# qts8n/water-sandbox

Measured on AMD Instinct MI355X. Metric: simulation steps/sec @ N particles, higher is better.
Workload: dtype f32

## Files before the change

water-sandbox_amd/csrc/ws_api.cpp:

```cpp
#include <math.h>
#include <stdio.h>
#include <stdlib.h>
#include <string.h>

#include <algorithm>
#include <new>

#include "ws_internal.h"

namespace {

constexpr int kGridPad = 2;
constexpr uint64_t kMaxCells = 1ull << 29;

thread_local std::string g_create_error;

void slab_free(ws_handle *h);
void slab_drop_graphs(WsSlab *S);
ws_status slab_step(ws_handle *h);
ws_status slab_settle(ws_handle *h);
ws_status slab_read_by_id(ws_handle *h, int kind, void *out);
ws_status slab_gather_by_id(ws_handle *h, int kind);
ws_status slab_reset(ws_handle *h, const float *pos_xyz);
ws_status slab_write_particles(ws_handle *h, const ws_particle80 *in);
// ... 49 lines not shown
template <class T>
ws_status scratch_zeroed(ws_handle *h, WsScratch<T> &buf, size_t bytes, const char *what)
{
    const ws_status st = buf.grow(h, bytes, what);
    if (st) return st;
    HIP_TRY(h, hipMemsetAsync(buf.p, 0, bytes, h->stream));
    return WS_OK;
}

float powi_f32(float a, int b)
{
    float r = 1.0f;
    for (;;) {
        if (b & 1) r *= a;
        b /= 2;
        if (b == 0) break;
        a *= a;
    }
    return r;
}

float accept_threshold(float h)
{
    float t = h * h;
    while (sqrtf(t) > h) t = nextafterf(t, 0.0f);
    for (;;) {
        const float up = nextafterf(t, INFINITY);
        if (sqrtf(up) <= h)
            t = up;
        else
            break;
    }
    return t;
}

}

ws_status ws_alloc_failed(ws_handle *h, const char *what, hipError_t e)
{
    (void)hipGetLastError();
    return fail(h, e == hipErrorOutOfMemory ? WS_ERR_OUT_OF_MEMORY : WS_ERR_HIP, what, e);
}

namespace {

bool is_pow2(uint32_t n) { return n && !(n & (n - 1)); }

uint32_t ref_linear(int x, int y, int z)
{
    return (uint32_t)x * 15823u + (uint32_t)y * 9737333u + (uint32_t)z * 440817757u;
}

uint32_t ref_hash_delta(int x, int y, int z, uint32_t n) { return ref_linear(x, y, z) % n; }

ws_status validate_params(ws_handle *h, const ws_params *p)
{
    if (!p) return fail(h, WS_ERR_INVALID_ARG, "params is NULL");
    if (!(p->smoothing_radius > 0.0f) || !isfinite(p->smoothing_radius))
        return fail(h, WS_ERR_INVALID_ARG, "smoothing_radius must be finite and > 0");
    for (int c = 0; c < 3; c++) {
        if (!isfinite(p->ext_min[c]) || !isfinite(p->ext_max[c]) || p->ext_min[c] > p->ext_max[c])
            return fail(h, WS_ERR_INVALID_ARG, "container ext_min/ext_max must be finite with ext_min <= ext_max");
    }
    return WS_OK;
}

ws_status derive_dev(ws_handle *h, const ws_params &p, uint32_t n, WsDev *out)
{
    WsDev d{};
    d.dt = p.delta_time;
    d.damping = p.collision_damping;
    d.h = p.smoothing_radius;
    d.target_density = p.target_density;
    d.pressure_scalar = p.pressure_scalar;
    d.near_pressure_scalar = p.near_pressure_scalar;
    d.viscosity = p.viscosity_strength;
    ws_smoothing_kernel sk;
    ws_get_smoothing_kernel(&p, &sk);
    d.k_pow2 = sk.pow2;
    d.k_pow2_der = sk.pow2_der;
    d.k_pow3 = sk.pow3;
    d.k_pow3_der = sk.pow3_der;
    d.k_spikey = sk.spikey_pow3;
    for (int c = 0; c < 3; c++) {
        d.grav[c] = p.gravity[c];
        d.ext_min[c] = p.ext_min[c];
        d.ext_max[c] = p.ext_max[c];
    }
    d.d2_accept = accept_threshold(d.h);
    uint64_t cells = 1;
    for (int c = 0; c < 3; c++) {
        const double lo = floor((double)floorf(p.ext_min[c] / d.h)) - kGridPad;
        const double hi = floor((double)floorf(p.ext_max[c] / d.h)) + kGridPad;
        const double dim = hi - lo + 1.0;
        if (!(fabs(lo) < 8388608.0) || !(fabs(hi) < 8388608.0))
            return fail(h, WS_ERR_INVALID_ARG, "container / smoothing_radius out of range (more than 2^23 cells along an axis)");
        d.org[c] = (int32_t)lo;
        d.fdim[c] = d.dim[c] = (int32_t)dim;
        d.cm[c] = 1;
        cells *= (uint64_t)d.dim[c];
    }
    uint64_t budget = std::max<uint64_t>(16ull * n, 1ull << 24);
    if (const char *v = WS_DEV_ENV("WS_CELL_BUDGET")) budget = std::max<uint64_t>(strtoull(v, nullptr, 10), 64);
    budget = std::min<uint64_t>(budget, kMaxCells);
    for (int c = 2; c >= 0 && cells > budget; c--) {
        const uint64_t others = cells / (uint64_t)d.dim[c];
        uint64_t want = std::max<uint64_t>(budget / std::max<uint64_t>(others, 1), 1);
        uint64_t m = ((uint64_t)d.fdim[c] + want - 1) / want;
        const uint64_t m_max = c == 0 ? (uint64_t)d.fdim[c] : (uint64_t)d.fdim[c] / 3;
        m = std::min<uint64_t>(std::max<uint64_t>(m, 1), std::max<uint64_t>(m_max, 1));
        d.cm[c] = (int32_t)m;
        d.dim[c] = (int32_t)(((uint64_t)d.fdim[c] + m - 1) / m);
        cells = others * (uint64_t)d.dim[c];
    }
    d.coarse = (d.cm[0] != 1 || d.cm[1] != 1 || d.cm[2] != 1) ? 1u : 0u;
    if (cells > kMaxCells) return fail(h, WS_ERR_OUT_OF_MEMORY, "cell grid too large even with merged cells");
    d.ncells = (uint32_t)cells;
    d.guard = d.dim[1] * d.dim[2] + d.dim[2] + 1;
    d.n = n;
    d.base = 0;
    d.gdim_x = d.dim[0];
    d.xoff = 0;
    d.hash_n = n;
    h->sk = sk;
    *out = d;
    return WS_OK;
}

void free_grid(ws_handle *h)
{
    h->cells.release();
    h->starts.release();
    h->start = nullptr;
    h->grid_alloc_cells = 0;
}

ws_status alloc_grid(ws_handle *h)
{
    const WsDev &d = h->dev;
    if (h->steps > 0 && WS_DEV_ENV("WS_FAIL_REGRID")) return fail(h, WS_ERR_OUT_OF_MEMORY, "cell tables: allocation failure forced by WS_FAIL_REGRID");
    ws_status st = WS_OK;
    if (h->grid_alloc_cells < d.ncells) {
        free_grid(h);
        if ((st = h->cells.alloc(h, &h->count, (size_t)d.ncells * 4, "cell counts"))) return st;
        if ((st = h->cells.alloc(h, &h->cursor, (size_t)d.ncells * 4, "cell cursors"))) return st;
        h->grid_alloc_cells = d.ncells;
    }
    h->starts.release();
    h->start = nullptr;
    const size_t nstart = (size_t)d.ncells + 2 * (size_t)d.guard + 2;
    if ((st = h->starts.alloc(h, &h->start_alloc, (nstart + 4) * 4, "cell starts"))) return st;
    h->start = h->start_alloc + (4u - (uint32_t)d.guard % 4u) % 4u;
    if ((st = h->starts.alloc(h, &h->bsum, (size_t)wsk_scan_state_words(d.ncells) * 4, "cell scan state", true))) return st;
    HIP_TRY(h, hipMemsetAsync(h->start, 0, (size_t)d.guard * 4, h->stream));
    std::vector<uint32_t> tail((size_t)d.guard + 2, d.n);
    HIP_TRY(h, hipMemcpyAsync(h->start + d.guard + d.ncells, tail.data(), tail.size() * 4, hipMemcpyHostToDevice,
                              h->stream));
    HIP_TRY(h, hipStreamSynchronize(h->stream));
    HIP_TRY(h, hipMemsetAsync(h->count, 0, (size_t)d.ncells * 4, h->stream));
    return WS_OK;
}

ws_status upload_mult(ws_handle *h)
{
    uint8_t m[27];
    bool alias = false;
    const uint32_t n = h->dev.hash_n;
    for (int dx = -1; dx <= 1; dx++)
        for (int dy = -1; dy <= 1; dy++)
            for (int dz = -1; dz <= 1; dz++) {
                uint32_t cnt = 0;
                for (int ox = -1; ox <= 1; ox++)
                    for (int oy = -1; oy <= 1; oy++)
                        for (int oz = -1; oz <= 1; oz++) {
                            if (is_pow2(n)) {
                                if (ref_hash_delta(ox, oy, oz, n) == ref_hash_delta(dx, dy, dz, n)) cnt++;
                                continue;
                            }
                            if (ox == dx && oy == dy && oz == dz) {
                                cnt++;
                                continue;
                            }
                            const int64_t delta = (int64_t)ref_linear(ox, oy, oz) - (int64_t)ref_linear(dx, dy, dz);
                            for (int64_t k = -1; k <= 1; k++)
                                if ((delta + k * ((int64_t)1 << 32)) % (int64_t)n == 0) alias = true;
                        }
                if (cnt > 1) alias = true;
                m[(dx + 1) * 9 + (dy + 1) * 3 + (dz + 1)] = (uint8_t)(cnt ? cnt : 1);
            }
    h->alias = alias;
    if (!h->mult) {
        const ws_status st = h->fixed.alloc(h, &h->mult, 32, "stencil multiplicities");
        if (st) return st;
    }
    HIP_TRY(h, copy_now(h, h->mult, m, 27, hipMemcpyHostToDevice));
    return WS_OK;
}

void configure_kernels(ws_handle *h)
{
    if (const char *v = WS_DEV_ENV("WS_VARIANT")) h->variant = strcmp(v, "simple") == 0 ? WS_VARIANT_SIMPLE : WS_VARIANT_LISTED;
    h->ieee = (h->flags & WS_FLAG_IEEE_DIVISION) != 0;
}

ws_status ensure_stage(ws_handle *h, size_t bytes)
{
    const ws_status st = h->stage_mem.grow(h, bytes, "staging buffer");
    h->stage = h->stage_mem.p;
    return st;
}

#define WS_DEAD_CHECK(h)                                               \
    do {                                                               \
        if ((h)->dead) return fail((h), WS_ERR_HIP, (h)->err.c_str()); \
    } while (0)

#ifdef WS_WITH_REFCHECK
#include "ws_refcheck_host.inc"
#define WS_REF_DISPATCH(h, call)       \
    do {                               \
        if ((h)->refmode) return call; \
    } while (0)
#else
#define WS_REF_DISPATCH(h, call) ((void)0)
#endif

hipEvent_t get_event(ws_handle *h)
{
    if (!h->pool.empty()) {
        hipEvent_t e = h->pool.back();
        h->pool.pop_back();
        return e;
    }
    hipEvent_t e = nullptr;
    if (hipEventCreate(&e) != hipSuccess) return nullptr;
    return e;
}

struct Prof {
    ws_handle *h;
    bool on;
    WsEventPair p{};
    Prof(ws_handle *h_, uint32_t k) : h(h_), on((h_->flags & WS_FLAG_PROFILE) != 0 && ((h_->prof_mask >> k) & 1u))
    {
        if (!on) return;
        p.kernel = k;
        p.a = get_event(h);
        p.b = get_event(h);
        if (!p.a || !p.b || hipEventRecord(p.a, h->stream) != hipSuccess) {
            if (p.a) h->pool.push_back(p.a);
            if (p.b) h->pool.push_back(p.b);
            on = false;
        }
    }
    ~Prof()
    {
        if (!on) return;
        if (hipEventRecord(p.b, h->stream) == hipSuccess) {
            h->pending.push_back(p);
        } else {
            h->pool.push_back(p.a);
            h->pool.push_back(p.b);
        }
    }
};

struct ProfLaunch {
    ws_handle *h;
    bool on, taken = false;
    WsEventPair p{};
    ProfLaunch(ws_handle *h_, uint32_t k, bool counts = true)
        : h(h_), on((h_->flags & WS_FLAG_PROFILE) != 0 && ((h_->prof_mask >> k) & 1u))
    {
        if (!on) return;
        p.kernel = k;
        p.counts = counts;
        p.a = get_event(h);
        p.b = get_event(h);
        if (!p.a || !p.b) {
            if (p.a) h->pool.push_back(p.a);
            if (p.b) h->pool.push_back(p.b);
            on = false;
        }
    }
    const WsEventPair *events()
    {
        if (!on) return nullptr;
        taken = true;
        return &p;
    }
    ~ProfLaunch()
    {
        if (!on) return;
        if (taken) {
            h->pending.push_back(p);
        } else {
            h->pool.push_back(p.a);
            h->pool.push_back(p.b);
        }
    }
};

void drain_profile(ws_handle *h)
{
    for (auto &p : h->pending) {
        float ms = 0.f;
        if (hipEventElapsedTime(&ms, p.a, p.b) == hipSuccess) {
            h->prof_ms[p.kernel] += ms;
            h->prof_cnt[p.kernel] += p.counts ? 1 : 0;
        }
        h->pool.push_back(p.a);
        h->pool.push_back(p.b);
    }
    h->pending.clear();
}

void bound_pending(ws_handle *h)
{
    if (h->pending.size() < 4096) return;
    if (hipStreamSynchronize(h->stream) == hipSuccess) drain_profile(h);
}

#define WS_SCHED_MIN_PARTICLES (1u << 18)
#define WS_SCHED_END_PARTICLES (1u << 20)

void free_schedule(ws_handle *h)
{
    if (h->sched_stream) {
        hipStreamSynchronize(h->sched_stream);
        hipStreamDestroy(h->sched_stream);
    }
    if (h->ev_sched_in) hipEventDestroy(h->ev_sched_in);
    if (h->ev_sched_out) hipEventDestroy(h->ev_sched_out);
    h->sched.release();
    h->sched4[1].cost = nullptr;
    h->sched_stream = nullptr;
    h->ev_sched_in = h->ev_sched_out = nullptr;
    h->sched_on = false;
}

ws_status alloc_schedule(ws_handle *h)
{
    if (h->variant != WS_VARIANT_LISTED || h->slab) return WS_OK;
    uint32_t min_n = WS_SCHED_MIN_PARTICLES, max_n = WS_SCHED_END_PARTICLES - 1u;
    if (const char *v = WS_DEV_ENV("WS_TILE_SCHEDULE")) {
        min_n = 0;
        max_n = atoi(v) ? 0xFFFFFFFFu : 0u;
    }
    if (h->n > max_n || h->n < min_n) return WS_OK;
    if (const char *v = WS_DEV_ENV("WS_SCHED_CLASSES")) h->sched_classes = (uint32_t)atoi(v);
    if (const char *v = WS_DEV_ENV("WS_SCHED_GROUP")) h->sched_group = (uint32_t)atoi(v);
    h->sched_tiles4 = (h->n + wsk_density_tile() - 1u) / wsk_density_tile();
    h->sched_tiles5 = (h->n + wsk_force_tile(h->n) - 1u) / wsk_force_tile(h->n);
    const size_t t4 = (size_t)h->sched_tiles4 * 4, t5 = (size_t)h->sched_tiles5 * 4;
    WsGroup &G = h->sched;
    ws_status st = G.alloc(h, &h->sched4[0].cost, t4, "tile costs", true);
    h->sched4[1].cost = h->sched4[0].cost;
    for (int k = 0; k < 2 && !st; k++) {
        st = G.alloc(h, &h->sched4[k].split, 16 * 4, "tile schedule");
        if (!st) st = G.alloc(h, &h->sched4[k].perm, t4, "tile schedule");
        if (!st) st = G.alloc(h, &h->sched5[k].split, 16 * 4, "tile schedule");
        if (!st) st = G.alloc(h, &h->sched5[k].perm, t5, "tile schedule");
        if (!st) st = G.alloc(h, &h->sched5[k].cost, t5, "tile costs", true);
    }
    if (st) return st;
    HIP_TRY(h, hipStreamCreateWithFlags(&h->sched_stream, hipStreamNonBlocking));
    HIP_TRY(h, hipEventCreateWithFlags(&h->ev_sched_in, hipEventDisableTiming));
    HIP_TRY(h, hipEventCreateWithFlags(&h->ev_sched_out, hipEventDisableTiming));
    for (int k = 0; k < 2; k++)
        wsk_schedule(h->stream, h->sched4[k], h->sched_tiles4, h->sched5[k], h->sched5[k], h->sched_tiles5, h->sched_classes, h->sched_group,
                     wsk_force_tile(h->n));
    HIP_TRY(h, hipGetLastError());
    HIP_TRY(h, hipStreamSynchronize(h->stream));
    h->sched_parity = 0;
    h->sched_on = true;
    return WS_OK;
}

void enqueue_step(ws_handle *h)
{
    const WsDev &d = h->dev;
    hipStream_t s = h->stream;
    const bool sched = h->sched_on && !h->alias && h->variant == WS_VARIANT_LISTED && !(h->flags & WS_FLAG_GRAPH);
    const uint32_t par = h->sched_parity;
    {
        Prof p(h, WS_K_SCAN);
        wsk_scan(s, h->count, h->start + d.guard, nullptr, h->bsum, d.ncells, true, 0);
    }
    {
        Prof p(h, WS_K_SCATTER);
        wsk_place(s, d, h->cid_cur, h->cur.rank, h->start, h->slot_tmp);
    }
    {
        Prof p(h, WS_K_REORDER);
        wsk_reorder(s, d, h->slot_tmp, h->cid_cur, h->start, h->cur, h->srt, h->cid_srt, h->sxyz, h->pred_stale);
    }
    if (sched) hipStreamWaitEvent(s, h->ev_sched_out, 0);
    {
        ProfLaunch p(h, WS_K_DENSITY);
        wsk_density(s, d, h->start, h->cid_srt, h->srt, h->mult, h->alias, h->variant, h->ieee, h->stats, h->mask, h->sxyz,
                    p.events(), sched ? h->sched4[par] : WsSched{});
    }
    if (sched) {
        hipEventRecord(h->ev_sched_in, s);
        hipStreamWaitEvent(h->sched_stream, h->ev_sched_in, 0);
        wsk_schedule(h->sched_stream, h->sched4[par ^ 1u], h->sched_tiles4, h->sched5[par ^ 1u], h->sched5[par ^ 1u], h->sched_tiles5,
                     h->sched_classes, h->sched_group, wsk_force_tile(h->n));
        hipEventRecord(h->ev_sched_out, h->sched_stream);
        h->sched_parity = par ^ 1u;
    }
    {
        ProfLaunch p(h, WS_K_FORCE);
        wsk_force(s, d, h->start, h->cid_srt, h->srt, h->cur, h->accel, h->cid_cur, h->count, h->mult, h->alias,
                  h->variant, h->ieee, h->mask, false, p.events(), sched ? h->sched5[par] : WsSched{});
    }
    h->pred_stale = true;
    h->accel_stale = true;
}

void note_step_params(ws_handle *h)
{
    h->last_pressure = {h->dev.pressure_scalar, h->dev.target_density, h->dev.near_pressure_scalar};
}

void refresh_pred(ws_handle *h, const WsDev &d)
{
    if (!h->pred_stale) return;
    wsk_refresh_pred(h->stream, d, h->cur);
    h->pred_stale = false;
}

ws_status refresh_accel(ws_handle *h)
{
    if (!h->accel_stale) return WS_OK;
    WsDev d = h->dev;
    auto pass = [&](const WsDev &dd) {
        if (dd.n)
            wsk_force(h->stream, dd, h->start, h->cid_srt, h->srt, h->cur, h->accel, h->cid_cur, h->count, h->mult, h->alias,
                      h->variant, h->ieee, h->mask, true);
    };
    if (h->slab) {
        const WsSlab *S = h->slab;
        d.dyn = S->dyn;
        d.n = S->cap;
        if (S->last_split) {
            d.range_sel = WS_RANGE_EARLY;
            pass(d);
            d.range_sel = d.has_left && d.has_right ? WS_RANGE_LATE_BOTH : d.has_left ? WS_RANGE_LATE_LEFT : WS_RANGE_LATE_RIGHT;
            d.n = (uint32_t)std::min<uint64_t>(S->cap, 2ull * S->halo_cap);
            pass(d);
        } else {
            d.range_sel = WS_RANGE_ALL;
            pass(d);
        }
    } else {
        pass(d);
    }
    HIP_TRY(h, hipGetLastError());
    h->accel_stale = false;
    return WS_OK;
}

ws_status bin_current(ws_handle *h)
{
    refresh_pred(h, h->dev);
    HIP_TRY(h, hipMemsetAsync(h->count, 0, (size_t)h->dev.ncells * 4, h->stream));
    {
        Prof pr(h, WS_K_BIN);
        wsk_bin(h->stream, h->dev, h->cur, h->cid_cur, h->count);
    }
    HIP_TRY(h, hipGetLastError());
    return WS_OK;
}

ws_status upload_positions(ws_handle *h, const float *pos_xyz)
{
    const size_t bytes = (size_t)h->n * 12;
    ws_status st = ensure_stage(h, bytes);
    if (st) return st;
    HIP_TRY(h, hipMemcpyAsync(h->stage, pos_xyz, bytes, hipMemcpyHostToDevice, h->stream));
    wsk_upload_positions(h->stream, (const float *)h->stage, h->cur, h->n);
    HIP_TRY(h, hipGetLastError());
    h->pred_stale = false;
    h->accel_stale = false;
    st = bin_current(h);
    if (st) return st;
    HIP_TRY(h, hipStreamSynchronize(h->stream));
    h->steps = 0;
    h->last_pressure = {};
    return WS_OK;
}

void drop_graphs(ws_handle *h)
{
    if (h->graph_exec) hipGraphExecDestroy(h->graph_exec);
    h->graph_exec = nullptr;
    if (h->slab) slab_drop_graphs(h->slab);
}

ws_status alloc_particle_arrays(ws_handle *h, size_t slots, uint32_t mask_particles)
{
    const size_t n16 = (slots + 16) * 16, n4 = slots * 4;
    WsGroup &G = h->particles;
    ws_status st = G.alloc(h, &h->cur.pv, 2 * n16, "particle records");
    if (!st) st = G.alloc(h, &h->cur.pred, n16, "predicted positions");
    if (!st) st = G.alloc(h, &h->cur.rank, n4, "cell ranks");
    if (!st) st = G.alloc(h, &h->srt.pos, n16, "sorted positions");
    if (!st) st = G.alloc(h, &h->srt.pv, 2 * n16, "sorted records");
    for (float **plane : {&h->sxyz.x, &h->sxyz.y, &h->sxyz.z})
        if (!st) st = G.alloc(h, plane, n16 / 4, "sorted position planes", true);
    if (!st) st = G.alloc(h, &h->cid_cur, n4, "cell ids");
    if (!st) st = G.alloc(h, &h->cid_srt, n4, "sorted cell ids");
    if (!st) st = G.alloc(h, &h->accel, n16, "accelerations");
    if (!st) st = G.alloc(h, &h->slot_tmp, n4, "sort slots");
    if (!st && h->variant == WS_VARIANT_LISTED) {
        h->mask.stride = mask_particles;
        st = G.alloc(h, &h->mask.words, (size_t)wsk_mask_words() * mask_particles * 4, "accept masks");
    }
    return st;
}

void free_particle_arrays(ws_handle *h)
{
    drop_graphs(h);
    h->particles.release();
    h->mask.stride = 0;
}

void free_all(ws_handle *h)
{
    if (h->stream) hipStreamSynchronize(h->stream);
    if (h->copy_stream) {
        hipStreamSynchronize(h->copy_stream);
        hipStreamDestroy(h->copy_stream);
    }
    free_schedule(h);
    if (h->rb_gathered) hipEventDestroy(h->rb_gathered);
    if (h->rb_done) hipEventDestroy(h->rb_done);
    release_all(h->rb_stage, h->rb_host[0], h->rb_host[1]);
    drain_profile(h);
    for (auto e : h->pool) hipEventDestroy(e);
    free_grid(h);
    free_particle_arrays(h);
    release_all(h->fixed, h->stage_mem, h->force_cnt, h->solid_sums, h->v_keys, h->v_perm, h->v_tmp, h->v_count, h->v_cursor, h->v_start, h->v_bsum,
                h->v_off);
    for (auto &volume : h->volume) release_all(volume);
    release_all(h->attr);
    free_field(h);
#ifdef WS_WITH_REFCHECK
    ref_free(h);
#endif
    slab_free(h);
    if (h->done) hipEventDestroy(h->done);
    if (h->stream && h->own_stream) hipStreamDestroy(h->stream);
}

}

extern "C" {

uint32_t ws_abi_version(void) { return WS_ABI_VERSION; }

const char *ws_status_string(ws_status s)
{
    switch (s) {
        case WS_OK: return "ok";
        case WS_ERR_INVALID_ARG: return "invalid argument";
        case WS_ERR_NO_DEVICE: return "no usable gfx950 device";
        case WS_ERR_OUT_OF_MEMORY: return "out of device memory";
        case WS_ERR_HIP: return "HIP runtime error";
        case WS_ERR_COMM: return "RCCL communication error";
        case WS_ERR_UNSUPPORTED: return "unsupported";
        case WS_ERR_NOT_READY: return "not ready";
    }
    return "unknown status";
}

const char *ws_kernel_name(uint32_t k)
{
    static const char *names[WS_K_COUNT] = {"cell_scan", "cell_scatter", "reorder", "density", "force_integrate_bin",
                                            "bin"};
    return k < WS_K_COUNT ? names[k] : "?";
}

ws_status ws_default_params(ws_params *out)
{
    if (!out) return WS_ERR_INVALID_ARG;
    memset(out, 0, sizeof *out);
    out->delta_time = 1.0f / 60.0f;
    out->collision_damping = 0.95f;
    out->smoothing_radius = 0.25f;
    out->target_density = 10.0f;
    out->pressure_scalar = 22.0f;
    out->near_pressure_scalar = 2.0f;
    out->viscosity_strength = 0.1f;
    out->gravity[1] = -9.8f;
    const float position[3] = {0.f, 0.f, 0.f}, size[3] = {16.f, 9.f, 9.f};
    return ws_get_ext(position, size, 0.1f, out->ext_min, out->ext_max);
}

ws_status ws_get_smoothing_kernel(const ws_params *p, ws_smoothing_kernel *out)
{
    if (!p || !out) return WS_ERR_INVALID_ARG;
    const float PI = 3.14159265358979323846f;
    const float h = p->smoothing_radius;
    out->pow2 = 15.0f / (2.0f * PI * powi_f32(h, 5));
    out->pow2_der = 15.0f / (PI * powi_f32(h, 5));
    out->pow3 = 15.0f / (PI * powi_f32(h, 6));
    out->pow3_der = 45.0f / (PI * powi_f32(h, 6));
    out->spikey_pow3 = 315.0f / (64.0f * PI * powi_f32(h, 9));
    return WS_OK;
}

ws_status ws_cube_fluid(uint32_t ni, uint32_t nj, uint32_t nk, float r, float *out)
{
    if (!out) return WS_ERR_INVALID_ARG;
    const float ox = r - (float)ni * r, oy = r - (float)nj * r, oz = r - (float)nk * r;
    const float diam = r * 2.0f;
    size_t o = 0;
    for (uint32_t i = 0; i < ni; i++)
        for (uint32_t j = 0; j < nj; j++)
            for (uint32_t k = 0; k < nk; k++) {
                out[o++] = (float)i * diam + ox;
                out[o++] = (float)j * diam + oy;
                out[o++] = (float)k * diam + oz;
            }
    return WS_OK;
}

ws_status ws_get_ext(const float position[3], const float size[3], float padding, float ext_min[4], float ext_max[4])
{
    if (!position || !size || !ext_min || !ext_max) return WS_ERR_INVALID_ARG;
    for (int c = 0; c < 3; c++) {
        const float half = size[c] / 2.0f;
        ext_min[c] = (position[c] - half) + padding;
        ext_max[c] = (position[c] + half) - padding;
    }
    ext_min[3] = ext_max[3] = 0.0f;
    return WS_OK;
}

uint32_t ws_bit_sorter_stage_count(uint32_t data_length)
{
    uint32_t k = 0;
    uint64_t p = 1;
    while (p < data_length) {
        p <<= 1;
        k++;
    }
    return k * (k + 1) / 2;
}

ws_status ws_create(const ws_params *params, const float *pos_xyz, uint32_t n, const ws_device_cfg *cfg,
                    ws_handle **out)
{
    if (!out) return WS_ERR_INVALID_ARG;
    *out = nullptr;
    if (!pos_xyz || n == 0) return fail(nullptr, WS_ERR_INVALID_ARG, "pos_xyz is NULL or n == 0");
    if (n > WS_MAX_SLOTS - 16u) return fail(nullptr, WS_ERR_INVALID_ARG, "more than 2^27 particles on one device");
    ws_status st = validate_params(nullptr, params);
    if (st) return st;
    if (cfg && cfg->world_size > 1) return fail(nullptr, WS_ERR_UNSUPPORTED, "multi-GPU slabs are created with ws_slab_create");
#ifndef WS_WITH_REFCHECK
    if (cfg && (cfg->flags & WS_FLAG_REFERENCE_ORDER))
        return fail(nullptr, WS_ERR_UNSUPPORTED,
                    "WS_FLAG_REFERENCE_ORDER is a validation mode of the test-only build (tests/libwsfluid_refcheck.so)");
#endif

    int ndev = 0;
    if (hipGetDeviceCount(&ndev) != hipSuccess || ndev <= 0)
        return fail(nullptr, WS_ERR_NO_DEVICE, "no HIP device visible (this library has no CPU fallback)");
    const int device = cfg ? cfg->device : 0;
    if (device < 0 || device >= ndev) return fail(nullptr, WS_ERR_NO_DEVICE, "device index out of range");
    hipDeviceProp_t prop;
    if (hipGetDeviceProperties(&prop, device) != hipSuccess) return fail(nullptr, WS_ERR_NO_DEVICE, "hipGetDeviceProperties failed");
    if (strncmp(prop.gcnArchName, "gfx950", 6) != 0)
        return fail(nullptr, WS_ERR_NO_DEVICE, "device is not gfx950 (kernels are built for MI355X only)");

    ws_handle *h = new (std::nothrow) ws_handle();
    if (!h) return fail(nullptr, WS_ERR_OUT_OF_MEMORY, "host allocation failed");
    h->device = device;
    h->flags = cfg ? cfg->flags : 0;
    h->n = n;
    h->params = *params;
    configure_kernels(h);
    if (h->flags & WS_FLAG_GRAPH) h->flags &= ~(uint32_t)WS_FLAG_PROFILE;

    auto bail = [&](ws_status s) {
        g_create_error = h->err;
        free_all(h);
        delete h;
        return s;
    };

    CREATE_HIP(hipSetDevice(device));
    CREATE_HIP(hipStreamCreateWithFlags(&h->stream, hipStreamNonBlocking));
    CREATE_HIP(hipEventCreateWithFlags(&h->done, hipEventDisableTiming));
    CREATE_TRY(derive_dev(h, *params, n, &h->dev));
#ifdef WS_WITH_REFCHECK
    if (h->flags & WS_FLAG_REFERENCE_ORDER) {
        CREATE_TRY(ref_alloc(h));
        CREATE_TRY(ref_upload_positions(h, pos_xyz));
        *out = h;
        return WS_OK;
    }
#endif
    CREATE_TRY(alloc_particle_arrays(h, n, n));
    CREATE_TRY(h->fixed.alloc(h, &h->stats, 64, "device counters", true));
    CREATE_TRY(alloc_grid(h));
    CREATE_TRY(upload_mult(h));
    CREATE_TRY(upload_positions(h, pos_xyz));
    CREATE_TRY(alloc_schedule(h));
    *out = h;
    return WS_OK;
}

ws_status ws_destroy(ws_handle *h)
{
    if (!h) return WS_OK;
    hipSetDevice(h->device);
    free_all(h);
    delete h;
    return WS_OK;
}

const char *ws_last_error(ws_handle *h) { return h ? h->err.c_str() : g_create_error.c_str(); }
uint32_t ws_num_particles(ws_handle *h) { return h ? h->n : 0; }
uint64_t ws_steps_done(ws_handle *h) { return h ? h->steps : 0; }

ws_status ws_step(ws_handle *h)
{
    if (!h) return WS_ERR_INVALID_ARG;
    HIP_TRY(h, hipSetDevice(h->device));
    if (h->slab) return slab_step(h);
    WS_REF_DISPATCH(h, ref_step(h));
    if (h->dead) return fail(h, WS_ERR_HIP, h->err.c_str());
    hipStream_t s = h->stream;
    bound_pending(h);
    note_step_params(h);
    if ((h->flags & WS_FLAG_GRAPH) && !h->graph_failed && h->pred_stale) {
        if (!h->graph_exec) {
            hipGraph_t gr = nullptr;
            hipError_t e = hipStreamBeginCapture(s, hipStreamCaptureModeRelaxed);
            if (e == hipSuccess) {
                enqueue_step(h);
                e = hipStreamEndCapture(s, &gr);
                if (e == hipSuccess) e = hipGraphInstantiate(&h->graph_exec, gr, nullptr, nullptr, 0);
                if (gr) hipGraphDestroy(gr);
            }
            if (e != hipSuccess || !h->graph_exec) {
                (void)hipGetLastError();
                h->graph_failed = true;
                h->graph_exec = nullptr;
                h->err = std::string("WS_FLAG_GRAPH: capture failed (") + hipGetErrorName(e) + "), using direct launches";
            }
        }
        if (h->graph_exec) {
            HIP_TRY(h, hipGraphLaunch(h->graph_exec, s));
            h->pred_stale = true;
            h->accel_stale = true;
            h->graph_steps++;
            HIP_TRY(h, hipEventRecord(h->done, s));
            h->done_recorded = true;
            h->steps++;
            return WS_OK;
        }
    }
    enqueue_step(h);
    HIP_TRY(h, hipGetLastError());
    HIP_TRY(h, hipEventRecord(h->done, s));
    h->done_recorded = true;
    h->steps++;
    return WS_OK;
}

ws_status ws_ready(ws_handle *h, int *ready)
{
    if (!h || !ready) return WS_ERR_INVALID_ARG;
    if (!h->done_recorded) {
        *ready = 1;
        return WS_OK;
    }
    const hipError_t e = hipEventQuery(h->done);
    if (e == hipSuccess)
        *ready = 1;
    else if (e == hipErrorNotReady)
        *ready = 0;
    else
        return fail(h, WS_ERR_HIP, "hipEventQuery", e);
    return WS_OK;
}

ws_status ws_sync(ws_handle *h)
{
    if (!h) return WS_ERR_INVALID_ARG;
    WS_DEAD_CHECK(h);
    HIP_TRY(h, hipSetDevice(h->device));
    if (h->slab) {
        const ws_status st = slab_settle(h);
        drain_profile(h);
        return st;
    }
    HIP_TRY(h, hipStreamSynchronize(h->stream));
    drain_profile(h);
    return WS_OK;
}

ws_status ws_set_params(ws_handle *h, const ws_params *params)
{
    if (!h) return WS_ERR_INVALID_ARG;
    WS_DEAD_CHECK(h);
    ws_status st = validate_params(h, params);
    if (st) return st;
    HIP_TRY(h, hipSetDevice(h->device));
    WsDev nd;
    st = derive_dev(h, *params, h->slab ? h->slab->n_global : h->n, &nd);
    if (st) return st;
    const WsDev &od = h->dev;
    bool regrid = memcmp(nd.org, od.org, sizeof nd.org) || memcmp(nd.dim, od.dim, sizeof nd.dim) || nd.h != od.h;
    if (h->slab) {
        regrid = nd.h != od.h || nd.dim[1] != od.dim[1] || nd.dim[2] != od.dim[2] || nd.dim[0] != od.gdim_x ||
                 memcmp(nd.org, od.org, sizeof nd.org);
        nd.dim[0] = od.dim[0]; nd.gdim_x = od.gdim_x; nd.xoff = od.xoff; nd.ncells = od.ncells; nd.guard = od.guard;
        nd.base = od.base; nd.n = od.n; nd.hash_n = od.hash_n;
        nd.has_left = od.has_left; nd.has_right = od.has_right; nd.mig = od.mig;
        memcpy(nd.lidx, od.lidx, sizeof nd.lidx);
    }
    WS_REF_DISPATCH(h, ref_set_params(h, params, nd));
    if (h->slab && regrid) return slab_regrid(h, params, false);
    const bool accel_params_changed =
        nd.h != od.h || nd.target_density != od.target_density || nd.pressure_scalar != od.pressure_scalar ||
        nd.near_pressure_scalar != od.near_pressure_scalar || nd.viscosity != od.viscosity || nd.k_pow2_der != od.k_pow2_der ||
        nd.k_pow3_der != od.k_pow3_der || nd.k_spikey != od.k_spikey || nd.d2_accept != od.d2_accept;
    if (regrid || accel_params_changed) {
        st = refresh_accel(h);
        if (st) return st;
    }
    h->params = *params;
    if (!regrid) {
        if (memcmp(&h->dev, &nd, sizeof nd) != 0) {
            drop_graphs(h);
            if (h->slab) h->slab->limit_hold = 8;
        }
        h->dev = nd;
        return WS_OK;
    }
    drop_graphs(h);
    HIP_TRY(h, hipStreamSynchronize(h->stream));
    h->dev = nd;
    st = alloc_grid(h);
    if (!st) st = bin_current(h);
    if (st) {
        h->dead = true;
        h->err = "re-grid failed after the old cell tables were given up (" + h->err + "); the handle is unusable";
    }
    return st;
}

ws_status ws_read_positions(ws_handle *h, float *out_xyz)
{
    if (!h || (!out_xyz && !h->slab)) return WS_ERR_INVALID_ARG;
    WS_DEAD_CHECK(h);
    HIP_TRY(h, hipSetDevice(h->device));
    if (h->slab) return slab_read_by_id(h, WS_PACK_POS_H, out_xyz);
    WS_REF_DISPATCH(h, ref_read_positions(h, out_xyz));
    const size_t bytes = (size_t)h->n * 12;
    ws_status st = ensure_stage(h, bytes);
    if (st) return st;
    wsk_gather_positions(h->stream, h->cur, (float *)h->stage, h->n);
    HIP_TRY(h, hipGetLastError());
    HIP_TRY(h, hipMemcpyAsync(out_xyz, h->stage, bytes, hipMemcpyDeviceToHost, h->stream));
    HIP_TRY(h, hipStreamSynchronize(h->stream));
    drain_profile(h);
    return WS_OK;
}

ws_status ws_read_positions_begin(ws_handle *h, float *out_xyz)
{
    if (!h) return WS_ERR_INVALID_ARG;
    WS_DEAD_CHECK(h);
    WS_REF_DISPATCH(h, fail(h, WS_ERR_UNSUPPORTED, "no asynchronous readback in the reference-order validation mode"));
    if (h->rb_inflight) return fail(h, WS_ERR_INVALID_ARG, "a readback is already in flight (call ws_read_positions_end)");
    HIP_TRY(h, hipSetDevice(h->device));
    const size_t bytes = (size_t)(h->slab ? h->slab->n_global : h->n) * 12;
    if (!h->copy_stream) {
        int lo = 0, hi = 0;
        const char *pr = WS_DEV_ENV("WS_COPY_STREAM_PRIORITY");
        if (pr && strcmp(pr, "default") == 0) {
            HIP_TRY(h, hipStreamCreateWithFlags(&h->copy_stream, hipStreamNonBlocking));
        } else {
            HIP_TRY(h, hipDeviceGetStreamPriorityRange(&lo, &hi));
            HIP_TRY(h, hipStreamCreateWithPriority(&h->copy_stream, hipStreamNonBlocking, hi));
        }
        HIP_TRY(h, hipEventCreateWithFlags(&h->rb_gathered, hipEventDisableTiming));
        HIP_TRY(h, hipEventCreateWithFlags(&h->rb_done, hipEventDisableTiming));
    }
    const bool owned = out_xyz == nullptr;
    if (owned) {
        if (h->rb_host[1].bytes < bytes) {
            release_all(h->rb_host[0], h->rb_host[1]);
            h->rb_last = -1;
            for (auto &b : h->rb_host) {
                const ws_status st = b.alloc(h, bytes, "page-locked readback buffer");
                if (st) return st;
            }
        }
        h->rb_fill = h->rb_last == 0 ? 1 : 0;
        out_xyz = h->rb_host[h->rb_fill].p;
    }
    const float *src;
    if (h->slab) {
// ... 22 lines not shown
    if (!h->rb_inflight) return fail(h, WS_ERR_INVALID_ARG, "no readback in flight");
    HIP_TRY(h, hipSetDevice(h->device));
    HIP_TRY(h, hipEventSynchronize(h->rb_done));
    h->rb_inflight = false;
    if (h->rb_owned) h->rb_last = h->rb_fill;
    return WS_OK;
}

ws_status ws_read_positions_view(ws_handle *h, const float **out_xyz)
{
    if (!h || !out_xyz) return WS_ERR_INVALID_ARG;
    *out_xyz = nullptr;
    if (h->rb_last < 0) return fail(h, WS_ERR_INVALID_ARG, "no finished readback into the library's buffers (ws_read_positions_begin(h, NULL) / _end)");
    *out_xyz = h->rb_host[h->rb_last].p;
    return WS_OK;
}

ws_status ws_read_speeds(ws_handle *h, float *out_speed)
{
    if (!h || (!out_speed && !h->slab)) return WS_ERR_INVALID_ARG;
    WS_DEAD_CHECK(h);
    HIP_TRY(h, hipSetDevice(h->device));
    if (h->slab) return slab_read_by_id(h, WS_PACK_SPEED_H, out_speed);
    WS_REF_DISPATCH(h, ref_read_speeds(h, out_speed));
    const size_t bytes = (size_t)h->n * 4;
    ws_status st = ensure_stage(h, bytes);
    if (st) return st;
    wsk_gather_speeds(h->stream, h->cur, (float *)h->stage, h->n);
    HIP_TRY(h, hipGetLastError());
    HIP_TRY(h, hipMemcpyAsync(out_speed, h->stage, bytes, hipMemcpyDeviceToHost, h->stream));
    HIP_TRY(h, hipStreamSynchronize(h->stream));
    drain_profile(h);
    return WS_OK;
}

ws_status ws_read_velocities(ws_handle *h, float *out_xyz)
{
    if (!h || (!out_xyz && !h->slab)) return WS_ERR_INVALID_ARG;
    WS_DEAD_CHECK(h);
    if (h->flags & WS_FLAG_REFERENCE_ORDER) return fail(h, WS_ERR_UNSUPPORTED, "velocities: not in the reference-order validation mode");
    HIP_TRY(h, hipSetDevice(h->device));
    const uint32_t n = h->slab ? h->slab->n_global : h->n;
    const size_t bytes = (size_t)n * 12;
    if (h->slab) {
        ws_status st = slab_gather_by_id(h, WS_PACK_POSVEL_H);
        if (st) return st;
        if (out_xyz) {
            if ((st = ensure_stage(h, bytes))) return st;
            wsk_field_split(h->stream, reinterpret_cast<const float *>(h->slab->g_out.p), nullptr, (float *)h->stage, n);
            HIP_TRY(h, hipGetLastError());
            HIP_TRY(h, hipMemcpyAsync(out_xyz, h->stage, bytes, hipMemcpyDeviceToHost, h->stream));
        }
        HIP_TRY(h, hipStreamSynchronize(h->stream));
        return WS_OK;
    }
    ws_status st = ensure_stage(h, bytes);
    if (st) return st;
    wsk_gather_velocities(h->stream, h->cur, (float *)h->stage, n);
    HIP_TRY(h, hipGetLastError());
    HIP_TRY(h, hipMemcpyAsync(out_xyz, h->stage, bytes, hipMemcpyDeviceToHost, h->stream));
    HIP_TRY(h, hipStreamSynchronize(h->stream));
    drain_profile(h);
    return WS_OK;
}

ws_status ws_pin_host_buffer(ws_handle *h, void *ptr, uint64_t bytes)
{
    if (!h || !ptr || !bytes) return WS_ERR_INVALID_ARG;
    HIP_TRY(h, hipSetDevice(h->device));
    HIP_TRY(h, hipHostRegister(ptr, (size_t)bytes, hipHostRegisterDefault));
    return WS_OK;
}

ws_status ws_unpin_host_buffer(ws_handle *h, void *ptr)
{
    if (!h || !ptr) return WS_ERR_INVALID_ARG;
    HIP_TRY(h, hipSetDevice(h->device));
    HIP_TRY(h, hipHostUnregister(ptr));
    return WS_OK;
}

ws_status ws_read_particles(ws_handle *h, ws_particle80 *out)
{
    if (!h || (!out && !h->slab)) return WS_ERR_INVALID_ARG;
    WS_DEAD_CHECK(h);
    HIP_TRY(h, hipSetDevice(h->device));
    if (h->slab) return slab_read_by_id(h, WS_PACK_RECORD_H, out);
    WS_REF_DISPATCH(h, ref_read_particles(h, out));
    const size_t bytes = (size_t)h->n * sizeof(ws_particle80);
    ws_status st = ensure_stage(h, bytes);
    if (st) return st;
    refresh_pred(h, h->dev);
    st = refresh_accel(h);
    if (st) return st;
    wsk_gather_particles(h->stream, h->cur, h->srt, h->accel, h->steps > 0, h->last_pressure, (ws_particle80 *)h->stage, h->n);
    HIP_TRY(h, hipGetLastError());
    HIP_TRY(h, hipMemcpyAsync(out, h->stage, bytes, hipMemcpyDeviceToHost, h->stream));
    HIP_TRY(h, hipStreamSynchronize(h->stream));
    drain_profile(h);
    return WS_OK;
}

ws_status ws_reset(ws_handle *h, const float *pos_xyz)
{
    if (!h || !pos_xyz) return WS_ERR_INVALID_ARG;
    WS_DEAD_CHECK(h);
    HIP_TRY(h, hipSetDevice(h->device));
    if (h->attr.p) HIP_TRY(h, hipMemsetAsync(h->attr.p, 0, h->attr.bytes, h->stream));
    if (h->slab) return slab_reset(h, pos_xyz);
    WS_REF_DISPATCH(h, ref_upload_positions(h, pos_xyz));
    return upload_positions(h, pos_xyz);
}

ws_status ws_write_particles(ws_handle *h, const ws_particle80 *in)
{
    if (!h || !in) return WS_ERR_INVALID_ARG;
    WS_DEAD_CHECK(h);
    HIP_TRY(h, hipSetDevice(h->device));
    if (h->slab) return slab_write_particles(h, in);
    WS_REF_DISPATCH(h, ref_load(h, in, false));
    const size_t bytes = (size_t)h->n * sizeof(ws_particle80);
    ws_status st = ensure_stage(h, bytes);
    if (st) return st;
    HIP_TRY(h, hipMemcpyAsync(h->stage, in, bytes, hipMemcpyHostToDevice, h->stream));
    wsk_upload_particles(h->stream, (const ws_particle80 *)h->stage, h->cur, h->n);
    HIP_TRY(h, hipGetLastError());
    h->pred_stale = false;
    h->accel_stale = false;
    st = bin_current(h);
    if (st) return st;
    HIP_TRY(h, hipStreamSynchronize(h->stream));
    h->steps = 0;
    h->last_pressure = {};
    return WS_OK;
}

}

namespace {

template <class Call>
ws_status edit_fluid(ws_handle *h, Call &call)
{
    if (!h) return WS_ERR_INVALID_ARG;
    WS_DEAD_CHECK(h);
    if (h->flags & WS_FLAG_REFERENCE_ORDER)
        return fail(h, WS_ERR_UNSUPPORTED, (std::string(call.tag) + ": not in the reference-order validation mode").c_str());
    HIP_TRY(h, hipSetDevice(h->device));
    if (h->slab) return slab_edit_gathered(h, call);
    if (const char *why = call.refuse()) return fail(h, WS_ERR_INVALID_ARG, why);
    const ws_status st = call.prepare(h, nullptr);
    if (st) return st;
    HIP_TRY(h, hipMemsetAsync(h->count, 0, (size_t)h->dev.ncells * 4, h->stream));
    wsk_edit_current(h->stream, h->dev, h->cur, h->cid_cur, h->count, call.args);
    HIP_TRY(h, hipGetLastError());
    h->pred_stale = true;
    HIP_TRY(h, call.fetch(h));
    return WS_OK;
}

const char *forces_refusal(const ws_force *f, uint32_t k, float dt)
{
    if (!f) return "forces: f is NULL";
    if (k < 1u || k > WS_MAX_FORCES) return "forces: k outside 1 .. WS_MAX_FORCES";
    if (ws_bad_float(dt) || !(dt > 0.f)) return "forces: dt must be finite, > 0 and at most 1e15";
    for (uint32_t e = 0; e < k; e++) {
        if (f[e].kind > WS_FORCE_VORTEX) return "forces: unknown kind";
        if (f[e].reserved[0] || f[e].reserved[1]) return "forces: reserved words must be 0";
        for (int c = 0; c < 3; c++)
            if (ws_bad_float(f[e].centre[c]) || ws_bad_float(f[e].axis[c])) return "forces: centre and axis must be finite and at most 1e15 in magnitude";
        if (ws_bad_float(f[e].strength) || ws_bad_float(f[e].damping)) return "forces: strength and damping must be finite and at most 1e15 in magnitude";
        if (f[e].damping < 0.f) return "forces: damping must be >= 0";
        if (ws_bad_float(f[e].radius) || !(f[e].radius > 0.f)) return "forces: radius must be finite, > 0 and at most 1e15";
    }
    return nullptr;
}

struct ForcesCall {
    const ws_force *f;
    uint32_t k;
    float dt;
    uint32_t *out_affected;
    const char *tag = "forces", *things = "emitters";
    WsForceArgs args{};
    const char *refuse() const { return forces_refusal(f, k, dt); }
    ws_status prepare(ws_handle *h, const WsGathered *)
    {
        memcpy(args.fs.e, f, (size_t)k * sizeof(ws_force));
        args.k = k;
        args.dt = dt;
        if (!out_affected) return WS_OK;
        const ws_status st = scratch_zeroed(h, h->force_cnt, WS_MAX_FORCES * 4, "force counters");
        args.affected = h->force_cnt.p;
        return st;
    }
    template <class M>
    void mix(M m, bool valid) const
    {
        m(&k, 4);
        m(&dt, 4);
        if (valid) m(f, (size_t)k * sizeof(ws_force));
    }
    hipError_t fetch(ws_handle *h) const
    {
        return out_affected ? copy_now(h, out_affected, h->force_cnt.p, (size_t)k * 4, hipMemcpyDeviceToHost) : hipSuccess;
    }
};

}

extern "C" {

ws_status ws_apply_forces(ws_handle *h, const ws_force *f, uint32_t k, float dt, uint32_t *out_affected)
{
    ForcesCall call{f, k, dt, out_affected};
    return edit_fluid(h, call);
}

}

namespace {

struct CohesionCall {
    const ws_cohesion_params *p;
    float dt;
    uint32_t *out_affected;
    const char *tag = "cohesion", *things = "parameters";
    WsCohesionArgs args{};
    const char *refuse() const { return cohesion_refusal(p, dt); }
    uint32_t partial[WS_COHESION_SLOTS * WS_COHESION_SLOT_WORDS];
    ws_status prepare(ws_handle *h, const WsGathered *g)
    {
        ws_status st = cohesion_prepare(h, g, p, dt, &args);
        if (st || !out_affected) return st;
        st = scratch_zeroed(h, h->force_cnt, sizeof partial, "cohesion counters");
        args.affected = h->force_cnt.p;
        return st;
    }
    template <class M>
    void mix(M m, bool valid) const
    {
        m(&dt, 4);
        if (valid) m(p, sizeof *p);
    }
    hipError_t fetch(ws_handle *h)
    {
        if (!out_affected) return hipSuccess;
        const hipError_t e = copy_now(h, partial, h->force_cnt.p, sizeof partial, hipMemcpyDeviceToHost);
        if (e != hipSuccess) return e;
        uint32_t total = 0;
        for (uint32_t s = 0; s < WS_COHESION_SLOTS; s++) total += partial[s * WS_COHESION_SLOT_WORDS];
        *out_affected = total;
        return hipSuccess;
    }
};

}

extern "C" {

ws_status ws_apply_cohesion(ws_handle *h, const ws_cohesion_params *p, float dt, uint32_t *out_affected)
{
    CohesionCall call{p, dt, out_affected};
    return edit_fluid(h, call);
}

}

namespace {

const char *solids_refusal(const ws_solid *s, uint32_t k)
{
    if (!s) return "solids: s is NULL";
    if (k < 1u || k > WS_MAX_SOLIDS) return "solids: k outside 1 .. WS_MAX_SOLIDS";
    for (uint32_t e = 0; e < k; e++) {
        const ws_solid &o = s[e];
        if (o.kind > WS_SOLID_CAPSULE) return "solids: unknown kind";
        if (o.flags & ~WS_SOLID_HOLLOW) return "solids: unknown flag bits";
        if (o.reserved[0] || o.reserved[1]) return "solids: reserved words must be 0";
        for (int c = 0; c < 9; c++)
            if (ws_bad_float(o.rot[c])) return "solids: rot must be finite and at most 1e15 in magnitude";
        for (int c = 0; c < 3; c++)
            if (ws_bad_float(o.centre[c]) || ws_bad_float(o.size[c]) || ws_bad_float(o.velocity[c]) || ws_bad_float(o.angular_velocity[c]))
                return "solids: centre, size, velocity and angular_velocity must be finite and at most 1e15 in magnitude";
        if (ws_bad_float(o.restitution) || ws_bad_float(o.friction) || ws_bad_float(o.margin)) return "solids: restitution, friction and margin must be finite";
        const int used = o.kind == WS_SOLID_BOX ? 3 : 1;
        for (int c = 0; c < used; c++)
            if (!(o.size[c] > 0.f)) return "solids: a radius or half extent must be > 0";
        if (o.kind == WS_SOLID_CAPSULE && o.size[1] < 0.f) return "solids: a capsule's half length must be >= 0";
        if (o.restitution < 0.f || o.restitution > 1.f || o.friction < 0.f || o.friction > 1.f) return "solids: restitution and friction must lie in [0, 1]";
        if (o.margin < 0.f) return "solids: margin must be >= 0";
    }
    return nullptr;
}

double rot_sigma_min2(const float *rot)
{
    double G[3][3];
    for (int i = 0; i < 3; i++)
        for (int j = 0; j < 3; j++)
            G[i][j] = (double)rot[3 * i] * rot[3 * j] + (double)rot[3 * i + 1] * rot[3 * j + 1] + (double)rot[3 * i + 2] * rot[3 * j + 2];
    const double tr = G[0][0] + G[1][1] + G[2][2], mean = tr / 3.0;
    const double off = G[0][1] * G[0][1] + G[0][2] * G[0][2] + G[1][2] * G[1][2];
    double dev = 2.0 * off;
    for (int i = 0; i < 3; i++) dev += (G[i][i] - mean) * (G[i][i] - mean);
    const double pp = sqrt(dev / 6.0);
// ... 335 lines not shown
ws_status ws_read_stats(ws_handle *h, uint32_t out[16])
{
    if (!h || !out) return WS_ERR_INVALID_ARG;
    ws_status st = ws_sync(h);
    if (st) return st;
    HIP_TRY(h, copy_now(h, out, h->stats, 64, hipMemcpyDeviceToHost));
    for (int c = 0; c < 3; c++) out[1 + c] = (uint32_t)h->dev.cm[c];
    out[4] = (uint32_t)(h->slab ? h->slab->graph_steps : h->graph_steps);
    out[15] = (h->sched_on && !h->alias && !(h->flags & WS_FLAG_GRAPH)) ? 1u : 0u;
    if (h->slab) {
        uint32_t dyn[WS_DYN_WORDS];
        HIP_TRY(h, copy_now(h, dyn, h->slab->dyn, sizeof dyn, hipMemcpyDeviceToHost));
        out[5] = dyn[DY_PEAK_HALO];
        out[6] = h->slab->halo_cap;
        out[7] = dyn[DY_PEAK_MIG];
        out[8] = h->slab->mig_cap;
        out[9] = dyn[DY_PEAK_FAR];
        out[10] = h->slab->far_cap;
        out[11] = h->slab->mig_limit_next;
        out[12] = h->slab->halo_limit_next;
        out[13] = h->slab->far_limit_next;
        out[14] = h->slab->size_waits;
        if (h->slab->world == 1) {
            out[11] = out[12] = out[13] = 0;
        } else if (h->slab->exact_messages) {
            out[11] = h->slab->exact_now[0];
            out[12] = h->slab->exact_now[1];
            out[13] = h->slab->exact_now[2];
        }
    }
    return WS_OK;
}

ws_status ws_grid_dims(ws_handle *h, uint32_t dims[3])
{
    if (!h || !dims) return WS_ERR_INVALID_ARG;
    for (int c = 0; c < 3; c++) dims[c] = (uint32_t)h->dev.dim[c];
    return WS_OK;
}

}

#ifdef WS_DEV_HOOKS
namespace {

struct DevSchedArrays {
    WsScratch<uint32_t> cost4, cost5, split4, split5, perm4, perm5;
    void release() { release_all(cost4, cost5, split4, split5, perm4, perm5); }
};

ws_status dev_upload_costs(ws_handle *h, WsScratch<uint32_t> &buf, const uint32_t *cost, uint32_t nt)
{
    const ws_status st = buf.alloc(h, (size_t)nt * 4, "planted tile costs");
    if (st) return st;
    if (nt) HIP_TRY(h, hipMemcpyAsync(buf.p, cost, (size_t)nt * 4, hipMemcpyHostToDevice, h->stream));
    return WS_OK;
}

ws_status dev_schedule_outputs(ws_handle *h, WsScratch<uint32_t> &split, WsScratch<uint32_t> &perm, uint32_t nt)
{
    ws_status st = split.alloc(h, 16 * 4, "tile schedule");
    if (!st) st = perm.alloc(h, (size_t)nt * 4, "tile schedule");
    if (st) return st;
    HIP_TRY(h, hipMemsetAsync(split.p, 0xFF, 16 * 4, h->stream));
    if (nt) HIP_TRY(h, hipMemsetAsync(perm.p, 0xFF, (size_t)nt * 4, h->stream));
    return WS_OK;
}

ws_status dev_drain(ws_handle *h)
{
    HIP_TRY(h, hipStreamSynchronize(h->stream));
    if (h->sched_stream) HIP_TRY(h, hipStreamSynchronize(h->sched_stream));
    return WS_OK;
}

}

extern "C" {

ws_status ws_dev_schedule(ws_handle *h, const uint32_t *cost4, uint32_t nt4, const uint32_t *cost5, uint32_t nt5, uint32_t nclasses,
                          uint32_t group_particles, uint32_t tile5, uint32_t *split4, uint32_t *perm4, uint32_t *split5, uint32_t *perm5)
{
    if (!h || !split4 || !split5 || (nt4 && (!cost4 || !perm4)) || (nt5 && (!cost5 || !perm5)) || !tile5) return WS_ERR_INVALID_ARG;
    WS_DEAD_CHECK(h);
    HIP_TRY(h, hipSetDevice(h->device));
    DevSchedArrays a;
    const ws_status st = [&]() -> ws_status {
        ws_status s = dev_upload_costs(h, a.cost4, cost4, nt4);
        if (!s) s = dev_upload_costs(h, a.cost5, cost5, nt5);
        if (!s) s = dev_schedule_outputs(h, a.split4, a.perm4, nt4);
        if (!s) s = dev_schedule_outputs(h, a.split5, a.perm5, nt5);
        if (s) return s;
        WsSched s4, s5;
        s4.split = a.split4.p, s4.perm = a.perm4.p, s4.cost = a.cost4.p;
        s5.split = a.split5.p, s5.perm = a.perm5.p, s5.cost = a.cost5.p;
        wsk_schedule(h->stream, s4, nt4, s5, s5, nt5, nclasses, group_particles, tile5);
        HIP_TRY(h, hipGetLastError());
        HIP_TRY(h, hipMemcpyAsync(split4, a.split4.p, 9 * 4, hipMemcpyDeviceToHost, h->stream));
        HIP_TRY(h, hipMemcpyAsync(split5, a.split5.p, 9 * 4, hipMemcpyDeviceToHost, h->stream));
        if (nt4) HIP_TRY(h, hipMemcpyAsync(perm4, a.perm4.p, (size_t)nt4 * 4, hipMemcpyDeviceToHost, h->stream));
        if (nt5) HIP_TRY(h, hipMemcpyAsync(perm5, a.perm5.p, (size_t)nt5 * 4, hipMemcpyDeviceToHost, h->stream));
        HIP_TRY(h, hipStreamSynchronize(h->stream));
        return WS_OK;
    }();
    (void)hipStreamSynchronize(h->stream);
    a.release();
    return st;
}

ws_status ws_dev_plant_schedule(ws_handle *h, const uint32_t *cost4, const uint32_t *cost5)
{
    if (!h || !cost4 || !cost5) return WS_ERR_INVALID_ARG;
    WS_DEAD_CHECK(h);
    HIP_TRY(h, hipSetDevice(h->device));
    if (!h->sched_on) return fail(h, WS_ERR_INVALID_ARG, "ws_dev_plant_schedule: the handle has no tile schedule");
    DevSchedArrays a;
    const ws_status st = [&]() -> ws_status {
        ws_status s = dev_drain(h);
        if (!s) s = dev_upload_costs(h, a.cost4, cost4, h->sched_tiles4);
        if (!s) s = dev_upload_costs(h, a.cost5, cost5, h->sched_tiles5);
        if (s) return s;
        const uint32_t par = h->sched_parity;
        WsSched s4 = h->sched4[par], from5;
        s4.cost = a.cost4.p;
        from5.cost = a.cost5.p;
        wsk_schedule(h->stream, s4, h->sched_tiles4, h->sched5[par], from5, h->sched_tiles5, h->sched_classes, h->sched_group,
                     wsk_force_tile(h->n));
        HIP_TRY(h, hipGetLastError());
        HIP_TRY(h, hipMemsetAsync(h->sched4[par].cost, 0, (size_t)h->sched_tiles4 * 4, h->stream));
        HIP_TRY(h, hipMemsetAsync(h->sched5[par].cost, 0, (size_t)h->sched_tiles5 * 4, h->stream));
        HIP_TRY(h, hipStreamSynchronize(h->stream));
        return WS_OK;
    }();
    (void)hipStreamSynchronize(h->stream);
    a.release();
    return st;
}

ws_status ws_dev_read_tile_costs(ws_handle *h, uint32_t *cost4, uint32_t *cost5, uint32_t *ntiles)
{
    if (!h) return WS_ERR_INVALID_ARG;
    WS_DEAD_CHECK(h);
    HIP_TRY(h, hipSetDevice(h->device));
    if (!h->sched_on) return fail(h, WS_ERR_INVALID_ARG, "ws_dev_read_tile_costs: the handle has no tile schedule");
    const ws_status st = dev_drain(h);
    if (st) return st;
    if (ntiles) ntiles[0] = h->sched_tiles4, ntiles[1] = h->sched_tiles5;
    const uint32_t ran = h->sched_parity ^ 1u;
    if (cost4) HIP_TRY(h, copy_now(h, cost4, h->sched4[ran].cost, (size_t)h->sched_tiles4 * 4, hipMemcpyDeviceToHost));
    if (cost5) HIP_TRY(h, copy_now(h, cost5, h->sched5[ran].cost, (size_t)h->sched_tiles5 * 4, hipMemcpyDeviceToHost));
    return WS_OK;
}

}
#endif

#include "ws_field.inc"
#include "ws_slab.inc"
```

water-sandbox_amd/csrc/ws_internal.h:

```cpp
#pragma once

#include <hip/hip_runtime.h>
#include <math.h>
#include <stdint.h>

#include <string>
#include <vector>

#include "wsfluid.h"

#include "ws_devhooks.h"

struct WsMig {
    const uint32_t *cuts;
    uint32_t world, me;
    uint32_t *dyn;
    uint32_t *hole;
    uint32_t hole_cap;
    uint32_t *sendL, *sendR;
    uint32_t mig_cap;
    uint32_t *far;
    uint32_t far_cap;
};

// ... 95 lines not shown

struct WsSched {
    uint32_t *split = nullptr;
    uint32_t *perm = nullptr;
    uint32_t *cost = nullptr;
};

struct WsEventPair {
    uint32_t kernel;
    hipEvent_t a, b;
    bool counts = true;
};

inline bool ws_bad_float(float x) { return !isfinite(x) || fabsf(x) > 1e15f; }

ws_status ws_alloc_failed(ws_handle *h, const char *what, hipError_t e);

struct WsParked {
    std::vector<void *> list;
    void release()
    {
        for (void *q : list) (void)hipFree(q);
        list.clear();
    }
};

template <class... Owner>
void release_all(Owner &...o)
{
    (o.release(), ...);
}

template <class T, bool PINNED = false>
struct WsScratch {
    T *p = nullptr;
    size_t bytes = 0;
    ws_status alloc(ws_handle *h, size_t need, const char *what)
    {
        release();
        return fresh(h, need, what);
    }
    ws_status grow(ws_handle *h, size_t need, const char *what) { return bytes >= need ? WS_OK : alloc(h, need, what); }
    ws_status grow_parked(ws_handle *h, size_t need, size_t slack_div, WsParked *parked, const char *what)
    {
        if (bytes >= need) return WS_OK;
        T *const old = p;
        const size_t geometric = bytes + bytes / slack_div;
        const ws_status st = fresh(h, need > geometric ? need : geometric, what);
        if (!st && old) parked->list.push_back(old);
        return st;
    }
    void release()
    {
        if (p) (void)(PINNED ? hipHostFree(p) : hipFree(p));
        p = nullptr;
        bytes = 0;
    }

private:
    ws_status fresh(ws_handle *h, size_t want, const char *what)
    {
        void *q = nullptr;
        const size_t real = want > 4 ? want : 4;
        const hipError_t e = PINNED ? hipHostMalloc(&q, real, hipHostMallocDefault) : hipMalloc(&q, real);
        if (e != hipSuccess) return ws_alloc_failed(h, what, e);
        p = static_cast<T *>(q);
        bytes = want;
        return WS_OK;
    }
};

struct WsGroup {
    std::vector<void **> fields;
    template <class T>
    ws_status alloc(ws_handle *h, T **field, size_t bytes, const char *what, bool zero = false);
    void release()
    {
        for (void **f : fields) {
            (void)hipFree(*f);
            *f = nullptr;
        }
        fields.clear();
    }
};

struct WsField {
    uint32_t n = 0;
    WsScratch<float> xyz;
    WsScratch<uint32_t> keys, tmp, perm;
    WsScratch<float4> spos;
    uint32_t cells = 0;
    WsScratch<uint32_t> count, cursor, start, bsum;
    WsScratch<float> q, rho;
    WsScratch<float> grad;
    WsScratch<uint8_t> code;
    WsScratch<uint32_t> vbase, bcnt, bstart, bstate, tri;
    WsScratch<float> mxyz, mnrm;
    WsScratch<float> vxyz, vpos;
    WsScratch<float4> svel;
    WsScratch<float4> wnrm;
    WsScratch<float> wst, wout, wpt;
    WsScratch<uint32_t> wnb, wcnt, woff, wstate;
    WsScratch<float4> cnd, crec;
    WsScratch<float> cst;
    WsScratch<uint32_t> cnb;
    WsScratch<float4> sattr[2];
    WsScratch<float> srho;
    WsScratch<float4> aval;
    WsScratch<float> body;
    WsScratch<float> cxyz;
    WsScratch<float4> amf, smf;
    WsScratch<uint32_t> anb;
    WsScratch<float> rays, ray_t, ray_n;
};

struct WsVolumeDesc {
    const float *sdf;
    uint32_t dims[3];
    float origin[3];
    float spacing[3];
};

struct WsPressureParams {
    float pressure_scalar, target_density, near_pressure_scalar;
};

struct ws_handle {
    int device = 0;
    uint32_t flags = 0;
    uint32_t prof_mask = 0xFFFFFFFFu;
    uint32_t n = 0;
    uint64_t steps = 0;
    ws_params params{};
    ws_smoothing_kernel sk{};
    WsDev dev{};
    WsPressureParams last_pressure{};
    hipStream_t stream = nullptr;
    hipEvent_t done = nullptr;
    bool done_recorded = false;

    WsSoA cur{};
    WsSorted srt{};
    WsXYZ sxyz;
    uint32_t *cid_cur = nullptr;
    uint32_t *cid_srt = nullptr;
    int variant = WS_VARIANT_LISTED;
    float4 *accel = nullptr;
    uint32_t *slot_tmp = nullptr;
    uint32_t *count = nullptr;
    uint32_t *cursor = nullptr;
    uint32_t *start = nullptr;
    uint32_t *start_alloc = nullptr;
    uint32_t *bsum = nullptr;
    WsMask mask = {nullptr, 0};
    bool ieee = false;
    uint32_t *stats = nullptr;
    uint8_t *mult = nullptr;
    WsScratch<uint32_t> force_cnt;
    WsScratch<unsigned long long> solid_sums;
    WsScratch<float> volume[WS_MAX_VOLUMES];
    WsVolumeDesc volume_desc[WS_MAX_VOLUMES] = {};
    uint64_t volume_hash[WS_MAX_VOLUMES] = {};
    WsScratch<float4> attr;
    bool alias = false;
    size_t grid_alloc_cells = 0;
    WsGroup particles;
    WsGroup cells;
    WsGroup starts;
    WsGroup sched;
    WsGroup fixed;

    WsScratch<char> stage_mem;
    void *stage = nullptr;
    hipStream_t copy_stream = nullptr;
    hipEvent_t rb_gathered = nullptr, rb_done = nullptr;
    WsScratch<float> rb_stage;
    bool rb_inflight = false;
    WsScratch<float, true> rb_host[2];
    int rb_fill = 0, rb_last = -1;
    bool rb_owned = false;

    WsScratch<uint32_t> v_keys, v_perm, v_tmp, v_count, v_cursor, v_start, v_bsum, v_off;

    WsField field;

    std::vector<WsEventPair> pending;
    std::vector<hipEvent_t> pool;
    double prof_ms[WS_K_COUNT] = {0};
    uint64_t prof_cnt[WS_K_COUNT] = {0};

#ifdef WS_WITH_REFCHECK
    bool refmode = false;
    WsRef ref;
#endif

    WsSched sched4[2], sched5[2];
    uint32_t sched_tiles4 = 0, sched_tiles5 = 0;
    bool sched_on = false;
    uint32_t sched_classes = 8, sched_group = 64;
    uint32_t sched_parity = 0;
    hipStream_t sched_stream = nullptr;
    hipEvent_t ev_sched_in = nullptr, ev_sched_out = nullptr;

    hipGraphExec_t graph_exec = nullptr;
    bool graph_failed = false;
    uint64_t graph_steps = 0;

    bool accel_stale = false;
    bool pred_stale = false;
    struct WsSlab *slab = nullptr;
    bool own_stream = true;
    bool dead = false;

    std::string err;
};

template <class T>
ws_status WsGroup::alloc(ws_handle *h, T **field, size_t bytes, const char *what, bool zero)
{
    void *q = nullptr;
    hipError_t e = hipMalloc(&q, bytes);
    if (e != hipSuccess) return ws_alloc_failed(h, what, e);
    *field = static_cast<T *>(q);
    fields.push_back(reinterpret_cast<void **>(field));
    if (zero && (e = hipMemsetAsync(q, 0, bytes, h->stream)) != hipSuccess) return ws_alloc_failed(h, what, e);
    return WS_OK;
}

struct WsGraphEntry {
    uint32_t n_bound = 0, mig_cur = 0, mig_next = 0, halo = 0, far_cur = 0, far_next = 0;
    hipGraphExec_t exec = nullptr;
};
struct WsSlab {
    ws_transport tr{};
    uint32_t rank = 0, world = 1;
    uint32_t n_global = 0;
    uint32_t cap = 0;
    uint32_t halo_cap = 0;
    uint32_t mig_cap = 0;
    uint32_t far_cap = 0;
    uint32_t hole_cap = 0;
    uint32_t max_arrivals = 0;
    uint32_t mig_limit_cur = 0;
    uint32_t mig_limit_next = 0;
    uint32_t far_limit_cur = 0, far_limit_next = 0, want_far = 0;
    uint32_t halo_limit = 0, halo_limit_next = 0;
    uint32_t want_mig = 0, want_halo = 0;
    uint32_t want_ring[3][8] = {};
    uint64_t arrivals_hist[4] = {0, 0, 0, 0};
    uint32_t floor_mig = 4096, floor_far = 256, floor_halo = 8192;
    bool exact_messages = false;
    uint32_t *xs_send[2] = {nullptr, nullptr}, *xs_all[2] = {nullptr, nullptr};
    WsScratch<uint32_t, true> xs_host[2];
    hipEvent_t ev_sizes[2] = {nullptr, nullptr};
    uint32_t *far_pack = nullptr;
    uint32_t exact_now[3] = {0, 0, 0};
    uint32_t size_waits = 0;
    uint32_t limit_hold = 0;
    bool fixed_messages = false;
    uint32_t mode_word = 0;
    std::vector<uint32_t> cuts;
    uint32_t *cuts_dev = nullptr;
    uint32_t *dyn = nullptr;
    WsMig *mig_dev = nullptr;
    uint32_t *hole = nullptr, *tgt = nullptr, *src = nullptr;
    uint32_t *mig_sendL = nullptr, *mig_sendR = nullptr, *mig_recvL = nullptr, *mig_recvR = nullptr;
    uint32_t *far_send = nullptr, *far_all = nullptr;
    uint32_t *halo_sendL = nullptr, *halo_sendR = nullptr, *halo_recvL = nullptr, *halo_recvR = nullptr;
    bool binned = false;
    uint32_t *status_dev = nullptr;
    WsScratch<uint32_t, true> status_host;
    hipEvent_t ev_status[4] = {nullptr, nullptr, nullptr, nullptr};
    uint32_t n_known = 0;
    uint64_t n_known_step = 0;
    uint64_t t0 = 0;
    uint32_t cfg_ghost_capacity = 0;
    WsScratch<uint32_t> cnt_send, cnt_all;
    WsScratch<uint32_t> g_send, g_all, g_out;
    WsScratch<uint32_t> hist;
    WsScratch<uint32_t> agree_send, agree_all;
    WsParked retired;
    WsGroup fixed;
    WsGroup geometry;
    std::vector<uint32_t> counts;
    std::vector<uint32_t> caps;
    uint64_t left_base = 0, arrived_base = 0, far_base = 0;
    bool balanced = false;
    uint32_t failed = 0;
    bool comm_failed = false;
    hipStream_t comm = nullptr, copy = nullptr;
    hipEvent_t ev_sorted = nullptr, ev_halo_a = nullptr, ev_k4_late = nullptr, ev_halo_b = nullptr, ev_filled = nullptr;
    bool overlap = true;
    bool last_split = false;
    std::vector<struct WsGraphEntry> graphs;
    bool graph_failed = false;
    bool capturing = false;
    uint64_t graph_steps = 0;
    hipEvent_t ev_copied = nullptr;
    uint64_t migrated_out = 0;
};

extern "C" void ws_rccl_transport_bind_stream(const ws_transport *t, void *stream);

void wsk_upload_positions(hipStream_t s, const float *xyz_dev, WsSoA cur, uint32_t n);
void wsk_upload_particles(hipStream_t s, const ws_particle80 *in_dev, WsSoA cur, uint32_t n);
void wsk_bin(hipStream_t s, const WsDev &d, WsSoA cur, uint32_t *cid, uint32_t *count);
void wsk_place(hipStream_t s, const WsDev &d, const uint32_t *cid, const uint32_t *rank, const uint32_t *start, uint32_t *slot_tmp);
void wsk_scan(hipStream_t s, uint32_t *count, uint32_t *start_body, uint32_t *cursor, uint32_t *state, uint32_t nitems,
              bool zero_count, uint32_t base);
uint32_t wsk_scan_state_words(uint32_t nitems);
void wsk_scatter(hipStream_t s, const uint32_t *keys, uint32_t *cursor, uint32_t *slot_tmp, uint32_t n, const uint32_t *n_dev);
void wsk_reorder(hipStream_t s, const WsDev &d, const uint32_t *slot_tmp, const uint32_t *cid_cur, const uint32_t *start, WsSoA cur,
                 WsSorted srt, uint32_t *cid_srt, WsXYZ sxyz, bool recompute_pred);
void wsk_refresh_pred(hipStream_t s, const WsDev &d, WsSoA cur);
struct WsForceSet {
    ws_force e[WS_MAX_FORCES];
};
struct WsForceArgs {
    WsForceSet fs;
    uint32_t k;
    float dt;
    uint32_t *affected;
    bool outputs() const { return affected != nullptr; }
};
#define WS_SOLID_WORDS 7u
struct WsSolidSet {
    ws_solid e[WS_MAX_SOLIDS];
    float reach2[WS_MAX_SOLIDS];
};
struct WsSolidArgs {
    WsSolidSet ss;
    uint32_t k;
    unsigned long long *sums;
    bool outputs() const { return sums != nullptr; }
};
struct WsVolumeSet {
    WsVolumeDesc vol[WS_MAX_VOLUMES];
    ws_volume_pose e[WS_MAX_VOLUME_POSES];
    float reach2[WS_MAX_VOLUME_POSES];
};
struct WsVolumeArgs {
    WsVolumeSet vs;
    uint32_t k;
    unsigned long long *sums;
    bool outputs() const { return sums != nullptr; }
};
static_assert(WS_MAX_VOLUME_POSES == WS_MAX_SOLIDS, "the poses' sums are the solids' accumulator rows");
#define WS_COHESION_SLOTS 64u
#define WS_COHESION_SLOT_WORDS 16u
struct WsCohesionArgs {
    const float4 *dvc;
    uint32_t *affected;
    uint32_t n;
    bool outputs() const { return affected != nullptr; }
};
struct WsGathered {
    const uint32_t *recs, *cnt;
    uint32_t world, max_n;
    size_t stride_words;
};
template <class Args>
void wsk_edit_current(hipStream_t s, const WsDev &d, WsSoA cur, uint32_t *cid, uint32_t *count, const Args &a);
template <class Args>
void wsk_edit_records(hipStream_t s, const WsDev &d, uint32_t *all, const uint32_t *cnt, uint32_t world, uint32_t max_n,
                      size_t stride_words, const Args &a);
void wsk_density(hipStream_t s, const WsDev &d, const uint32_t *start, const uint32_t *cid_srt, WsSorted srt,
                 const uint8_t *mult, bool alias, int variant, bool ieee, uint32_t *stats, WsMask mask, WsXYZ sxyz,
                 const WsEventPair *ev = nullptr, WsSched sched = WsSched{});
uint32_t wsk_density_tile(void);
uint32_t wsk_force_tile(uint32_t n);
uint32_t wsk_sched_grid(uint32_t ntiles);
void wsk_schedule(hipStream_t s, WsSched s4, uint32_t ntiles4, WsSched s5, WsSched s5_costs, uint32_t ntiles5, uint32_t nclasses,
                  uint32_t group_particles, uint32_t tile5);
uint32_t wsk_mask_words(void);
void wsk_force(hipStream_t s, const WsDev &d, const uint32_t *start, const uint32_t *cid_srt, WsSorted srt, WsSoA out,
               float4 *accel, uint32_t *cid_out, uint32_t *count, const uint8_t *mult, bool alias, int variant, bool ieee,
               WsMask mask, bool accel_only, const WsEventPair *ev = nullptr, WsSched sched = WsSched{});
void wsk_gather_positions(hipStream_t s, WsSoA cur, float *out_xyz, uint32_t n);
void wsk_gather_speeds(hipStream_t s, WsSoA cur, float *out, uint32_t n);
void wsk_gather_velocities(hipStream_t s, WsSoA cur, float *out_xyz, uint32_t n);
void wsk_gather_particles(hipStream_t s, WsSoA cur, WsSorted srt, const float4 *accel, bool have_step,
                          const WsPressureParams &pp, ws_particle80 *out, uint32_t n);
void wsk_view_keys(hipStream_t s, const WsDev &d, WsSorted srt, uint32_t *keys_by_id, uint32_t *count);
void wsk_view_count(hipStream_t s, const uint32_t *keys, uint32_t *count, uint32_t n);
void wsk_view_fix(hipStream_t s, const uint32_t *tmp, const uint32_t *keys, const uint32_t *start,
                  uint32_t *perm, uint32_t n);
void wsk_view_offsets(hipStream_t s, const uint32_t *start, uint32_t *off, uint32_t n);
void wsk_iota(hipStream_t s, uint32_t *p, uint32_t n);
void wsk_set_words4(hipStream_t s, uint32_t *p, uint32_t a, uint32_t b, uint32_t c, uint32_t d);
void wsk_field_keys(hipStream_t s, const WsDev &d, const float *xyz, uint32_t *keys, uint32_t n);
void wsk_field_gather(hipStream_t s, const uint32_t *perm, const float *xyz, float4 *spos, uint32_t n);
void wsk_field_sample(hipStream_t s, const WsDev &d, const uint32_t *start, const float4 *spos, const float4 *smf, bool ieee,
                      bool grad_on, const float *xyz, uint32_t m, const float *grid6, const uint32_t *dims, bool bricks,
                      float *rho, float *grad);
void wsk_field_split(hipStream_t s, const float *pv, float *pos, float *vel, uint32_t n);
void wsk_field_gather_vel(hipStream_t s, const uint32_t *perm, const float *vxyz, float4 *svel, uint32_t n);
void wsk_velocity_sample(hipStream_t s, const WsDev &d, const uint32_t *start, const float4 *spos, const float4 *svel, bool ieee,
                         const float *xyz, uint32_t m, const float *grid6, const uint32_t *dims, bool bricks, float *vel,
                         float *rho);
void wsk_advect(hipStream_t s, const WsDev &d, const uint32_t *start, const float4 *spos, const float4 *svel, bool ieee,
                float *pts, uint32_t m, float dt, uint32_t substeps, float *vel, float *rho);
struct WsWhiteEmit {
    float tt0, tt1, tc0, tc1, te0, te1, kt, kc, align, dt, radius, l0, l1;
    uint32_t maxpp, seed;
};
struct WsWhiteStep {
    float dt;
    uint32_t spray_max, bubble_min;
    float buoyancy, drag;
};
void wsk_whitewater_stage(hipStream_t s, const WsDev &d, const uint32_t *start, const float4 *spos, const float4 *svel,
                          float4 *snrm, float *trapped, float *crest, float *align, float *energy, float *normal, uint32_t *nb,
                          uint32_t n);
void wsk_whitewater_count(hipStream_t s, const WsWhiteEmit &e, const float *vxyz, const float *trapped, const float *crest,
                          const float *align, const float *energy, uint32_t *cnt, uint32_t n);
void wsk_whitewater_spawn(hipStream_t s, const WsWhiteEmit &e, const float *pxyz, const float *vxyz, const uint32_t *cnt,
                          const uint32_t *off, float *out_xyz, float *out_vel, float *out_life, uint32_t *out_src, uint32_t n);
void wsk_whitewater_step(hipStream_t s, const WsDev &d, const uint32_t *start, const float4 *spos, const float4 *svel, bool ieee,
                         const WsWhiteStep &sp, float *pts, float *vel, float *life, uint8_t *cls, uint32_t m);
struct WsCohesion {
    float cohesion, curvature, xsph, rho0, dt, kc, h664;
};
void wsk_cohesion_stage(hipStream_t s, const WsDev &d, const uint32_t *start, const float4 *spos, const float4 *svel,
                        float4 *snd, const WsCohesion &k, float4 *dvc, float4 *nrho, uint32_t n);
void wsk_cohesion_unpack(hipStream_t s, const float4 *dvc, const float4 *nrho, float *normal, float *rho, float *dv, uint32_t *nb,
                         uint32_t n);
void wsk_state_split(hipStream_t s, const uint32_t *all, const uint32_t *cnt, uint32_t world, uint32_t max_n, size_t stride_words,
                     uint32_t n_global, float *pos, float *vel);
struct WsBrushSet {
    ws_brush e[WS_MAX_BRUSHES];
};
struct WsBrushArgs {
    WsBrushSet bs;
    uint32_t k;
    uint32_t *painted;
};
void wsk_attr_paint(hipStream_t s, const WsBrushArgs &a, const float *xyz, float4 *attr, uint32_t n);
void wsk_attr_gather(hipStream_t s, const float4 *spos, const float4 *attr, float4 *sa, uint32_t n);
void wsk_attr_scatter(hipStream_t s, const float4 *spos, const float4 *sa, float4 *attr, uint32_t n);
void wsk_attr_density(hipStream_t s, const WsDev &d, const uint32_t *start, const float4 *spos, float *srho, uint32_t n);
void wsk_attr_diffuse(hipStream_t s, const WsDev &d, const uint32_t *start, const float4 *spos, const float *srho, const float4 *sa,
                      const float *r4, float4 *out, uint32_t *affected, uint32_t n);
void wsk_attr_sample(hipStream_t s, const WsDev &d, const uint32_t *start, const float4 *spos, const float4 *sa, bool ieee,
                     const float *xyz, uint32_t m, const float *grid6, const uint32_t *dims, bool bricks, float4 *value, float *rho);
struct WsBodyParams {
    float fluid_density, drag, rho0;
};
uint32_t wsk_body_chunk(void);
void wsk_body_forces(hipStream_t s, const WsDev &d, const uint32_t *start, const float4 *spos, const float4 *svel, bool ieee,
                     const WsBodyParams &bp, const uint32_t *chunks, uint32_t nchunks, const uint32_t *cstart, uint32_t nb,
                     const float *xyz, const float *vel, const float *vol, const float *centre, float *part, float *sforce,
                     float *sfrac, float *force, float *torque, float *volume, uint32_t *wet);
struct WsAnisoParams {
    float lambda, kr, kn;
    uint32_t neps;
};
void wsk_aniso(hipStream_t s, const WsDev &d, const uint32_t *start, const float4 *spos, WsAnisoParams ap, float *cxyz,
               float4 *mf, uint32_t *nb, uint32_t n);
void wsk_aniso_gather(hipStream_t s, const uint32_t *perm, const float *cxyz, const float4 *mf, float4 *srec, float4 *smf,
                      uint32_t n);
void wsk_ray_cast(hipStream_t s, const WsDev &d, const uint32_t *start, const float4 *spos, const float4 *smf,
                  bool ieee, const ws_ray_params &r, const float *origin, const float *dir, uint32_t m,
                  const ws_camera *cam, const uint32_t *size, float *out_t, float *out_n);
uint32_t wsk_iso_blocks(const uint32_t *dims);
void wsk_iso_totals(hipStream_t s, const uint32_t *v_total, const uint32_t *t_total, uint32_t *out);
void wsk_iso_count(hipStream_t s, const float *rho, const float *grid6, const uint32_t *dims, float iso, uint8_t *code,
                   uint32_t *vcnt, uint32_t *tcnt);
void wsk_iso_mesh(hipStream_t s, const float *rho, const float *grad, const float *grid6, const uint32_t *dims, float iso,
                  const uint8_t *code, const uint32_t *vstart, const uint32_t *tstart, uint32_t *vbase, float *xyz,
                  float *nrm, uint32_t *tri);
void wsk_migrate_mark(hipStream_t s, const WsDev &d, WsSoA cur, uint32_t *cid_cur, uint32_t *count);
void wsk_migrate_fill(hipStream_t s, const WsDev &d, uint32_t world, uint32_t me, uint32_t cap, uint32_t *dyn,
                      const uint32_t *hole, const uint32_t *recvL, const uint32_t *recvR, uint32_t mig_cap,
                      const uint32_t *far_all, uint32_t far_cap, uint32_t *tgt, uint32_t *src, WsSoA cur, uint32_t *cid_cur,
                      uint32_t *count, uint32_t *status_ring, uint32_t status_slots, uint32_t hole_cap, uint32_t *sendL,
                      uint32_t *sendR, uint32_t *far_send, uint32_t far_next, uint64_t leave_bound);
void wsk_far_seal(hipStream_t s, uint32_t world, uint32_t far_cur, uint32_t *far_send, uint32_t *dyn);
void wsk_sizes(hipStream_t s, const uint32_t *a, const uint32_t *b, const uint32_t *c, const uint32_t *dyn, uint32_t *out);
void wsk_far_pack(hipStream_t s, uint32_t world, uint32_t far_cap, uint32_t far_n, const uint32_t *src, uint32_t *dst);
void wsk_halo_pack(hipStream_t s, const WsDev &d, const uint32_t *start, WsSorted srt, uint32_t *dyn, uint32_t rowy,
                   uint32_t halo_cap, uint32_t *sendL, uint32_t *sendR, bool densities);
void wsk_halo_unpack(hipStream_t s, const WsDev &d, uint32_t *start, WsSorted srt, WsXYZ sxyz, uint32_t *dyn, uint32_t rowy,
                     uint32_t nxl, uint32_t ghost_cap, const uint32_t *recvL, const uint32_t *recvR, bool densities);
void wsk_gather_slab(hipStream_t s, const WsDev &d, WsSoA cur, WsSorted srt, const float4 *accel, bool have_step,
                     const WsPressureParams &pp, ws_particle80 *out, uint32_t *ids);
void wsk_upload_positions_ids(hipStream_t s, const float *xyz_dev, const uint32_t *ids_dev, WsSoA cur, uint32_t n);
enum { WS_PACK_POS_H = 0, WS_PACK_SPEED_H = 1, WS_PACK_RECORD_H = 2, WS_PACK_STATE_H = 3, WS_PACK_KEY_H = 4, WS_PACK_POSVEL_H = 5 };
uint32_t wsk_pack_words(int kind);
void wsk_slab_pack(hipStream_t s, const WsDev &d, int kind, WsSoA cur, WsSorted srt, const float4 *accel, bool have_step,
                   const WsPressureParams &pp, uint32_t *out);
void wsk_slab_unpack_by_id(hipStream_t s, const uint32_t *all, const uint32_t *cnt, uint32_t world, uint32_t max_n,
                           size_t stride_words, uint32_t pw, uint32_t n_global, uint32_t *out);
void wsk_slab_layer_hist(hipStream_t s, const WsDev &d, const uint32_t *all, const uint32_t *cnt, uint32_t world, uint32_t max_n,
                         size_t stride_words, uint32_t *hist);
void wsk_slab_select(hipStream_t s, const WsDev &d, int src, const uint32_t *cuts, uint32_t world, uint32_t me,
                     const void *chunk, uint32_t id0, uint32_t m, const uint32_t *cnt, size_t stride_words, WsSoA cur,
                     uint32_t cap, uint32_t *dyn);
```

water-sandbox_amd/csrc/ws_kernels.hip:

```cpp
#include <stdlib.h>

#include <algorithm>
#include <type_traits>

#include "ws_internal.h"

#include <hip/hip_ext.h>


#pragma clang fp contract(off)

#define WS_BLOCK 256
#define WS_SCAN_ITEMS_SMALL 32
#define WS_SCAN_ITEMS_LARGE 64
#define WS_SCAN_LARGE_FROM (1u << 21)
#define WS_SCAN_TILE_MIN (WS_BLOCK * WS_SCAN_ITEMS_SMALL)

static inline uint32_t cdiv(uint32_t a, uint32_t b) { return (a + b - 1) / b; }

__device__ __forceinline__ uint32_t xcd_tile(uint32_t b, uint32_t nt, bool reverse = false)
{
    const uint32_t xcd = b & 7u, q = nt >> 3, r = nt & 7u;
    const uint32_t first = xcd < r ? xcd * (q + 1u) : r * (q + 1u) + (xcd - r) * q, mine = q + (xcd < r ? 1u : 0u);
    const uint32_t j = b >> 3;
    return first + (reverse ? mine - 1u - j : j);
}


__device__ __forceinline__ int grid_layer_x(const WsDev &d, float x)
{
    const float fx = floorf(x / d.h) - (float)d.org[0];
    int gxg = (int)fminf(fmaxf(fx, 0.0f), (float)(d.fdim[0] - 1));
    if (d.coarse) gxg /= d.cm[0];
    return gxg;
}

__device__ __forceinline__ uint32_t grid_cell(const WsDev &d, float x, float y, float z)
{
    const float fy = floorf(y / d.h) - (float)d.org[1];
    const float fz = floorf(z / d.h) - (float)d.org[2];
    const int gxg = grid_layer_x(d, x);
    int gy = (int)fminf(fmaxf(fy, 0.0f), (float)(d.fdim[1] - 1));
    int gz = (int)fminf(fmaxf(fz, 0.0f), (float)(d.fdim[2] - 1));
    if (d.coarse) {
        gy /= d.cm[1];
        gz /= d.cm[2];
    }
    const int gx = min(max(gxg - d.xoff, 0), d.dim[0] - 1);
    return (uint32_t)((gx * d.dim[1] + gy) * d.dim[2] + gz);
}

__device__ __forceinline__ uint32_t ref_hash_key(const WsDev &d, float x, float y, float z)
{
    const uint32_t cx = (uint32_t)(int32_t)floorf(x / d.h);
    const uint32_t cy = (uint32_t)(int32_t)floorf(y / d.h);
    const uint32_t cz = (uint32_t)(int32_t)floorf(z / d.h);
    return (cx * 15823u + cy * 9737333u + cz * 440817757u) % d.hash_n;
}

__device__ __forceinline__ uint32_t ws_n(const WsDev &d) { return d.dyn ? d.dyn[DY_N] : d.n; }

struct WsSpan {
    uint32_t lo, len, split, jump;
};
__device__ __forceinline__ WsSpan ws_span(const WsDev &d, const uint32_t *__restrict__ start)
{
    WsSpan sp = {d.base, d.n, 0xFFFFFFFFu, 0u};
    if (!d.dyn) return sp;
    const uint32_t n = d.dyn[DY_N], end = d.base + n;
    sp.len = n;
    if (d.range_sel == WS_RANGE_ALL) return sp;
    const uint32_t a = d.has_left ? start[d.lidx[1]] : d.base;
    const uint32_t b = d.has_right ? start[d.lidx[2]] : end;
    if (d.range_sel == WS_RANGE_EARLY) {
        sp.lo = a;
        sp.len = b - a;
    } else if (d.range_sel == WS_RANGE_LATE_LEFT) {
        sp.len = a - d.base;
    } else if (d.range_sel == WS_RANGE_LATE_RIGHT) {
        sp.lo = b;
        sp.len = end - b;
    } else {
        sp.split = a - d.base;
        sp.jump = b - a;
        sp.len = (a - d.base) + (end - b);
    }
    return sp;
}
__device__ __forceinline__ uint32_t span_at(const WsSpan &sp, uint32_t v) { return sp.lo + v + (v >= sp.split ? sp.jump : 0u); }

struct WsCut {
    uint32_t lo, hi;
    bool on;
};
__device__ __forceinline__ WsCut ws_cut(const WsDev &d)
{
    WsCut c = {0u, 0xFFFFFFFFu, false};
    if (d.dyn && d.range_sel == WS_RANGE_EARLY) {
        c.lo = d.base;
        c.hi = d.base + d.dyn[DY_N];
        c.on = true;
    }
    return c;
}
template <bool CUT>
__device__ __forceinline__ void cut_run_t(const WsDev &d, uint32_t &b, uint32_t &e)
{
    if constexpr (CUT) {
        const uint32_t lo = d.base, hi = d.base + d.dyn[DY_N];
        b = min(max(b, lo), hi);
        e = min(max(e, lo), hi);
    }
}
__device__ __forceinline__ void cut_run(const WsCut &c, uint32_t &b, uint32_t &e)
{
    if (c.on) {
        b = min(max(b, c.lo), c.hi);
        e = min(max(e, c.lo), c.hi);
    }
}


__global__ void __launch_bounds__(WS_BLOCK) k_upload_positions(const float *__restrict__ xyz, WsSoA cur,
                                                               uint32_t n)
{
    const uint32_t i = blockIdx.x * WS_BLOCK + threadIdx.x;
    if (i >= n) return;
    const float x = xyz[3 * (size_t)i], y = xyz[3 * (size_t)i + 1], z = xyz[3 * (size_t)i + 2];
    cur.pos(i) = make_float4(x, y, z, __uint_as_float(i));
    cur.vel(i) = make_float4(0.f, 0.f, 0.f, 0.f);
    cur.pred[i] = make_float4(x, y, z, 0.f);
}

__global__ void __launch_bounds__(WS_BLOCK) k_upload_particles(const ws_particle80 *__restrict__ in, WsSoA cur,
                                                               uint32_t n)
{
    const uint32_t i = blockIdx.x * WS_BLOCK + threadIdx.x;
    if (i >= n) return;
    const float4 *rec = reinterpret_cast<const float4 *>(in + i);
    const float4 p = rec[0], v = rec[2], q = rec[4];
    cur.pos(i) = make_float4(p.x, p.y, p.z, __uint_as_float(i));
    cur.vel(i) = make_float4(v.x, v.y, v.z, 0.f);
    cur.pred[i] = make_float4(q.x, q.y, q.z, 0.f);
}

void wsk_upload_positions(hipStream_t s, const float *xyz_dev, WsSoA cur, uint32_t n)
{
    hipLaunchKernelGGL(k_upload_positions, dim3(cdiv(n, WS_BLOCK)), dim3(WS_BLOCK), 0, s, xyz_dev, cur, n);
}
void wsk_upload_particles(hipStream_t s, const ws_particle80 *in_dev, WsSoA cur, uint32_t n)
{
    hipLaunchKernelGGL(k_upload_particles, dim3(cdiv(n, WS_BLOCK)), dim3(WS_BLOCK), 0, s, in_dev, cur, n);
}

#define WS_DEAD 0xFFFFFFFFu

__global__ void __launch_bounds__(WS_BLOCK) k_bin(WsDev d, WsSoA cur, uint32_t *__restrict__ cid, uint32_t *__restrict__ count)
{
    const uint32_t i = blockIdx.x * WS_BLOCK + threadIdx.x;
    if (i >= ws_n(d)) return;
    const float4 p = cur.pred[i];
    const uint32_t c = grid_cell(d, p.x, p.y, p.z);
    cid[i] = c;
    cur.vel(i).w = __uint_as_float(c);
    const uint32_t r = atomicAdd(&count[c], 1u);
    if (cur.rank) cur.rank[i] = r;
}

void wsk_bin(hipStream_t s, const WsDev &d, WsSoA cur, uint32_t *cid, uint32_t *count)
{
    hipLaunchKernelGGL(k_bin, dim3(cdiv(d.n, WS_BLOCK)), dim3(WS_BLOCK), 0, s, d, cur, cid, count);
}

__device__ __forceinline__ uint32_t wave_incl_scan(uint32_t v)
{
    const int lane = threadIdx.x & 63;
#pragma unroll
    for (int o = 1; o < 64; o <<= 1) {
        const uint32_t t = __shfl_up(v, o, 64);
        if (lane >= o) v += t;
    }
    return v;
}

__device__ __forceinline__ uint32_t wave_run_atomic_inc(uint32_t *__restrict__ table, uint32_t key, bool active)
{
    const int lane = threadIdx.x & 63;
    const unsigned long long act = __ballot(active);
    const uint32_t prev = __shfl_up(key, 1, 64);
    const bool prev_active = lane > 0 && ((act >> (lane - 1)) & 1ull);
    const bool head = active && (!prev_active || key != prev);
    const unsigned long long heads = __ballot(head);
    if (!active) return 0u;
    const unsigned long long upto = heads & ((lane == 63) ? ~0ull : ((2ull << lane) - 1ull));
    const int hl = 63 - __builtin_clzll(upto);
    const unsigned long long above = (hl == 63) ? 0ull : (~((2ull << hl) - 1ull));
    const unsigned long long stop = (heads | ~act) & above;
    const int end = stop ? __builtin_ctzll(stop) : 64;
    uint32_t base = 0;
    if (lane == hl) base = atomicAdd(&table[key], (uint32_t)(end - hl));
    base = __shfl(base, hl, 64);
    return base + (uint32_t)(lane - hl);
}

template <bool ZERO, int WS_SCAN_ITEMS>
__global__ void __launch_bounds__(WS_BLOCK) k_scan(uint32_t *__restrict__ count, uint32_t nitems,
                                                   uint32_t *__restrict__ state, uint32_t *__restrict__ start,
                                                   uint32_t *__restrict__ cursor, uint32_t start_offset, uint32_t ntiles)
{
    __shared__ uint32_t s_tile, s_epoch, s_prefix;
    if (threadIdx.x == 0) {
        const unsigned long long ticket = atomicAdd(reinterpret_cast<unsigned long long *>(state), 1ull);
        s_tile = (uint32_t)(ticket % ntiles);
        s_epoch = (uint32_t)(ticket / ntiles) + 1u;
    }
    __syncthreads();
    const uint32_t tile = s_tile, epoch = s_epoch;
    constexpr int Q = WS_SCAN_ITEMS / 4;
    constexpr uint32_t WS_SCAN_TILE = WS_BLOCK * WS_SCAN_ITEMS;
    const uint32_t tbase = tile * WS_SCAN_TILE;
    uint4 v[Q];
    uint32_t excl[Q], total = 0;
#pragma unroll
    for (int q = 0; q < Q; q++) {
        const uint32_t at = tbase + (q * WS_BLOCK + threadIdx.x) * 4u;
        if (at + 4u <= nitems) {
            v[q] = *reinterpret_cast<const uint4 *>(count + at);
        } else {
            v[q].x = at < nitems ? count[at] : 0u;
            v[q].y = at + 1u < nitems ? count[at + 1u] : 0u;
            v[q].z = at + 2u < nitems ? count[at + 2u] : 0u;
            v[q].w = 0u;
        }
    }
    {
        __shared__ uint32_t wsum[Q][WS_BLOCK / 64];
        const int lane = threadIdx.x & 63, wave = threadIdx.x >> 6;
#pragma unroll
        for (int q = 0; q < Q; q++) {
            excl[q] = wave_incl_scan(v[q].x + v[q].y + v[q].z + v[q].w);
            if (lane == 63) wsum[q][wave] = excl[q];
        }
        __syncthreads();
#pragma unroll
        for (int q = 0; q < Q; q++) {
            uint32_t base = 0, tot = 0;
#pragma unroll
            for (int w = 0; w < WS_BLOCK / 64; w++) {
                const uint32_t sw = wsum[q][w];
                if (w < wave) base += sw;
                tot += sw;
            }
            excl[q] = total + base + excl[q] - (v[q].x + v[q].y + v[q].z + v[q].w);
            total += tot;
        }
    }
    if (threadIdx.x < 64) {
        unsigned long long *desc = reinterpret_cast<unsigned long long *>(state + 2);
        const uint32_t e30 = epoch & 0x3FFFFFFFu;
        const unsigned long long tag = (unsigned long long)(e30 << 2) << 32;
        const int lane = (int)threadIdx.x;
        uint32_t prefix = 0;
        if (tile != 0u) {
            if (lane == 0)
                __hip_atomic_store(&desc[tile], tag | (1ull << 32) | total, __ATOMIC_RELAXED, __HIP_MEMORY_SCOPE_AGENT);
            for (int32_t newest = (int32_t)tile - 1;;) {
                const int32_t p = newest - lane;
                const unsigned long long dsc =
                    p >= 0 ? __hip_atomic_load(&desc[p], __ATOMIC_RELAXED, __HIP_MEMORY_SCOPE_AGENT) : (tag | (2ull << 32));
                const uint32_t hi = (uint32_t)(dsc >> 32);
                const bool ready = (hi >> 2) == e30 && (hi & 3u) != 0u;
                const unsigned long long inclusive = __ballot(ready && (hi & 3u) == 2u);
                const int stop = inclusive ? __ffsll((long long)inclusive) - 1 : 63;
                const unsigned long long needed = stop == 63 ? ~0ull : (2ull << stop) - 1ull;
                if (__ballot(!ready) & needed) {
                    __builtin_amdgcn_s_sleep(1);
                    continue;
                }
                uint32_t v = lane <= stop ? (uint32_t)dsc : 0u;
#pragma unroll
                for (int sh = 32; sh >= 1; sh >>= 1) v += __shfl_xor(v, sh, 64);
                prefix += v;
                if (inclusive) break;
                newest -= 64;
            }
        }
        if (lane == 0) {
            __hip_atomic_store(&desc[tile], tag | (2ull << 32) | (prefix + total), __ATOMIC_RELAXED, __HIP_MEMORY_SCOPE_AGENT);
            s_prefix = prefix;
        }
    }
    __syncthreads();
    const uint32_t carry = s_prefix + start_offset;
#pragma unroll
    for (int q = 0; q < Q; q++) {
        const uint32_t at = tbase + (q * WS_BLOCK + threadIdx.x) * 4u;
        uint4 r;
        r.x = carry + excl[q];
        r.y = r.x + v[q].x;
        r.z = r.y + v[q].y;
        r.w = r.z + v[q].z;
        if (at + 4u <= nitems) {
            *reinterpret_cast<uint4 *>(start + at) = r;
            if (cursor) *reinterpret_cast<uint4 *>(cursor + at) = r;
            if (ZERO) *reinterpret_cast<uint4 *>(count + at) = make_uint4(0u, 0u, 0u, 0u);
        } else {
            const uint32_t rr[3] = {r.x, r.y, r.z};
            for (uint32_t k = 0; k < 3u && at + k < nitems; k++) {
                start[at + k] = rr[k];
                if (cursor) cursor[at + k] = rr[k];
                if (ZERO) count[at + k] = 0u;
            }
        }
    }
}

uint32_t wsk_scan_state_words(uint32_t nitems) { return 2u + 2u * cdiv(nitems, WS_SCAN_TILE_MIN); }

void wsk_scan(hipStream_t s, uint32_t *count, uint32_t *start_body, uint32_t *cursor, uint32_t *state, uint32_t nitems,
              bool zero_count, uint32_t base)
{
    const bool large = nitems >= WS_SCAN_LARGE_FROM;
    const uint32_t ntiles = cdiv(nitems, WS_BLOCK * (large ? WS_SCAN_ITEMS_LARGE : WS_SCAN_ITEMS_SMALL));
#define WS_SCAN_LAUNCH(Z, I) \
    hipLaunchKernelGGL((k_scan<Z, I>), dim3(ntiles), dim3(WS_BLOCK), 0, s, count, nitems, state, start_body, cursor, base, ntiles)
    if (zero_count) {
        if (large) WS_SCAN_LAUNCH(true, WS_SCAN_ITEMS_LARGE);
        else WS_SCAN_LAUNCH(true, WS_SCAN_ITEMS_SMALL);
    } else {
        if (large) WS_SCAN_LAUNCH(false, WS_SCAN_ITEMS_LARGE);
        else WS_SCAN_LAUNCH(false, WS_SCAN_ITEMS_SMALL);
    }
#undef WS_SCAN_LAUNCH
}

__global__ void __launch_bounds__(WS_BLOCK) k_scatter(const uint32_t *__restrict__ keys, uint32_t *__restrict__ cursor,
                                                      uint32_t *__restrict__ slot_tmp, uint32_t n,
                                                      const uint32_t *__restrict__ n_dev)
{
    const uint32_t i = blockIdx.x * WS_BLOCK + threadIdx.x;
    bool active = i < (n_dev ? *n_dev : n);
    if (active && keys[i] == WS_DEAD) active = false;
    const uint32_t slot = wave_run_atomic_inc(cursor, active ? keys[i] : 0u, active);
    if (active) slot_tmp[slot] = i;
}

__global__ void __launch_bounds__(WS_BLOCK) k_place(WsDev d, const uint32_t *__restrict__ cid,
                                                    const uint32_t *__restrict__ rank,
                                                    const uint32_t *__restrict__ start, uint32_t *__restrict__ slot_tmp)
{
    const uint32_t i = blockIdx.x * WS_BLOCK + threadIdx.x;
    if (i >= ws_n(d)) return;
    const uint32_t c = cid[i];
    if (c == WS_DEAD) return;
    slot_tmp[start[d.guard + c] + rank[i]] = i;
}

void wsk_place(hipStream_t s, const WsDev &d, const uint32_t *cid, const uint32_t *rank, const uint32_t *start, uint32_t *slot_tmp)
{
    hipLaunchKernelGGL(k_place, dim3(cdiv(d.n, WS_BLOCK)), dim3(WS_BLOCK), 0, s, d, cid, rank, start, slot_tmp);
}

void wsk_scatter(hipStream_t s, const uint32_t *keys, uint32_t *cursor, uint32_t *slot_tmp, uint32_t n, const uint32_t *n_dev)
{
    hipLaunchKernelGGL(k_scatter, dim3(cdiv(n, WS_BLOCK)), dim3(WS_BLOCK), 0, s, keys, cursor, slot_tmp, n, n_dev);
}

#define WS_LOOKAHEAD 0.02f
typedef uint32_t nd_u4u __attribute__((ext_vector_type(4), aligned(4)));
#ifndef WS_REORDER_BLOCK
#define WS_REORDER_BLOCK 512
#endif
template <bool RECOMPUTE_PRED>
__global__ void __launch_bounds__(WS_REORDER_BLOCK) k_reorder(WsDev d, const uint32_t *__restrict__ slot_tmp,
                                                      const uint32_t *__restrict__ cid_cur,
                                                      const uint32_t *__restrict__ start, WsSoA cur, WsSorted srt,
                                                      uint32_t *__restrict__ cid_srt, WsXYZ sxyz)
{
    __shared__ uint32_t s_id[WS_REORDER_BLOCK];
    const uint32_t blk = d.dyn ? blockIdx.x : xcd_tile(blockIdx.x, gridDim.x);
    const uint32_t k = blk * WS_REORDER_BLOCK + threadIdx.x;
    const uint32_t s = d.base + k, s0 = d.base + blk * WS_REORDER_BLOCK;
    bool active = k < ws_n(d);
    uint32_t i = 0, c = WS_DEAD;
    float4 p = make_float4(0.f, 0.f, 0.f, __uint_as_float(0xFFFFFFFFu)), v = p;
    if (active) {
        i = slot_tmp[s];
        p = cur.pos(i);
        v = cur.vel(i);
        c = __float_as_uint(v.w);
        v.w = 0.f;
        active = c != WS_DEAD;
        if (!active) p.w = __uint_as_float(0xFFFFFFFFu);
    }
    const uint32_t id = __float_as_uint(p.w);
    s_id[threadIdx.x] = id;
    __syncthreads();
    if (!active) return;
    const uint32_t b = start[d.guard + c], e = start[d.guard + c + 1];
    uint32_t rank = 0;
    for (uint32_t t = b; t < e; t++) {
        const uint32_t o = t - s0;
        const uint32_t other = o < (uint32_t)WS_REORDER_BLOCK ? s_id[o] : __float_as_uint(cur.pos(slot_tmp[t]).w);
        rank += other < id ? 1u : 0u;
    }
    const uint32_t dst = b + rank;
    float4 q;
    if constexpr (RECOMPUTE_PRED)
        q = make_float4(p.x + v.x * WS_LOOKAHEAD, p.y + v.y * WS_LOOKAHEAD, p.z + v.z * WS_LOOKAHEAD, 0.f);
    else
        q = cur.pred[i];
    srt.pos[dst] = p;
    srt.vel(dst) = v;
    srt.pred(dst) = q;
    sxyz.x[dst] = q.x;
    sxyz.y[dst] = q.y;
    sxyz.z[dst] = q.z;
    cid_srt[dst] = c;
}

void wsk_reorder(hipStream_t s, const WsDev &d, const uint32_t *slot_tmp, const uint32_t *cid_cur, const uint32_t *start, WsSoA cur,
                 WsSorted srt, uint32_t *cid_srt, WsXYZ sxyz, bool recompute_pred)
{
    if (recompute_pred)
        hipLaunchKernelGGL(k_reorder<true>, dim3(cdiv(d.n, WS_REORDER_BLOCK)), dim3(WS_REORDER_BLOCK), 0, s, d, slot_tmp, cid_cur, start, cur, srt,
                           cid_srt, sxyz);
    else
        hipLaunchKernelGGL(k_reorder<false>, dim3(cdiv(d.n, WS_REORDER_BLOCK)), dim3(WS_REORDER_BLOCK), 0, s, d, slot_tmp, cid_cur, start, cur, srt,
                           cid_srt, sxyz);
}

__global__ void __launch_bounds__(WS_BLOCK) k_refresh_pred(WsDev d, WsSoA cur)
{
    const uint32_t k = blockIdx.x * WS_BLOCK + threadIdx.x;
    if (k >= ws_n(d)) return;
    const uint32_t i = d.base + k;
    const float4 p = cur.pos(i), v = cur.vel(i);
    cur.pred[i] = make_float4(p.x + v.x * WS_LOOKAHEAD, p.y + v.y * WS_LOOKAHEAD, p.z + v.z * WS_LOOKAHEAD, 0.f);
}

void wsk_refresh_pred(hipStream_t s, const WsDev &d, WsSoA cur)
{
    if (d.n) hipLaunchKernelGGL(k_refresh_pred, dim3(cdiv(d.n, WS_BLOCK)), dim3(WS_BLOCK), 0, s, d, cur);
}

template <bool COUNTS>
__device__ __forceinline__ bool forces_eval(const WsForceSet &fs, uint32_t k, float dt, bool active, const float4 &p, float4 &v,
                                            uint32_t *__restrict__ affected)
{
    float ax = 0.f, ay = 0.f, az = 0.f;
    bool hit = false;
    for (uint32_t e = 0; e < k; e++) {
        const ws_force &f = fs.e[e];
        const float qx = p.x - f.centre[0], qy = p.y - f.centre[1], qz = p.z - f.centre[2];
        const float dst = sqrtf(qx * qx + qy * qy + qz * qz);
        const bool in = active && dst < f.radius;
        if constexpr (COUNTS) {
            const uint32_t c = (uint32_t)__popcll(__ballot(in));
            if (c && (threadIdx.x & 63u) == 0u) atomicAdd(&affected[e], c);
        }
        if (!in) continue;
        hit = true;
        const float w = 1.f - dst / f.radius, s = f.strength * w;
        if (f.kind == WS_FORCE_RADIAL) {
            if (dst > 0.f) {
                ax = ax - (qx / dst) * s;
                ay = ay - (qy / dst) * s;
                az = az - (qz / dst) * s;
            }
        } else if (f.kind == WS_FORCE_JET) {
            ax = ax + f.axis[0] * s;
            ay = ay + f.axis[1] * s;
            az = az + f.axis[2] * s;
        } else {
            const float tx = f.axis[1] * qz - f.axis[2] * qy;
            const float ty = f.axis[2] * qx - f.axis[0] * qz;
            const float tz = f.axis[0] * qy - f.axis[1] * qx;
            ax = ax + tx * s;
            ay = ay + ty * s;
            az = az + tz * s;
        }
        const float g = f.damping * w;
        ax = ax - v.x * g;
        ay = ay - v.y * g;
        az = az - v.z * g;
    }
    if (hit) {
        v.x = v.x + dt * ax;
        v.y = v.y + dt * ay;
        v.z = v.z + dt * az;
    }
    return hit;
}

__device__ __forceinline__ long long solids_fixed(float x)
{
    return llrintf(fminf(fmaxf(x, -2147483648.f), 2147483648.f) * 16777216.f);
}

__device__ __forceinline__ long long wave_sum_i64(long long x)
{
#pragma unroll
    for (int o = 32; o > 0; o >>= 1) x += __shfl_xor(x, o, 64);
    return x;
}

template <bool REACT>
__device__ __forceinline__ bool contact_respond(bool hit, float s, float nx, float ny, float nz, float margin, const float *centre,
                                                const float *V, const float *W, float restitution, float friction, float4 &p,
                                                float4 &v, unsigned long long *a)
{
    bool kicked = false;
    float dvx = 0.f, dvy = 0.f, dvz = 0.f, rx = 0.f, ry = 0.f, rz = 0.f;
// ... 405 lines not shown
            }
    return cnt;
}


template <bool IEEE>
__device__ __forceinline__ float ws_sqrt(float x)
{
    if constexpr (IEEE) return sqrtf(x);
    else return __builtin_amdgcn_sqrtf(x);
}

template <bool IEEE>
struct WsDivisor {
    float v;
    __device__ __forceinline__ explicit WsDivisor(float den) : v(IEEE ? den : __builtin_amdgcn_rcpf(den)) {}
    __device__ __forceinline__ float operator()(float num) const { return IEEE ? num / v : num * v; }
};

template <bool IEEE>
__device__ __forceinline__ void density_pair(const WsDev &d, float d2, float &density, float &near_density,
                                             uint32_t mult)
{
    const float dst = ws_sqrt<IEEE>(d2);
    const float w = sk_density(d, dst), wn = sk_near(d, dst);
    for (uint32_t r = 0; r < mult; r++) {
        density += w;
        near_density += wn;
    }
}

struct ForceAcc {
    float pfx, pfy, pfz, vfx, vfy, vfz;
};

template <bool IEEE>
__device__ __forceinline__ void force_pair(const WsDev &d, float ex, float ey, float ez, float d2, float nrho_x,
                                           float nrho_y, float4 nvel, float4 vel, float pressure, float near_pressure,
                                           ForceAcc &a, uint32_t mult)
{
    const float dst = ws_sqrt<IEEE>(d2);
    const float npress = d.pressure_scalar * (nrho_x - d.target_density);
    const float nnear = d.near_pressure_scalar * nrho_y;
    const float slope = sk_der(d, dst);
    const float shared = (pressure + npress) / 2.f;
    const float slope_near = sk_der_near(d, dst);
    const float shared_near = (near_pressure + nnear) / 2.f;
    if constexpr (IEEE) {
        const WsDivisor<IEEE> by_dst(dst), by_rho(nrho_x), by_near_rho(nrho_y);
        if (dst > 0.f) {
            ex = by_dst(ex);
            ey = by_dst(ey);
            ez = by_dst(ez);
        } else {
            ex = 0.f;
            ey = 1.f;
            ez = 0.f;
        }
        const float ax = by_rho(ex * shared * slope), ay = by_rho(ey * shared * slope), az = by_rho(ez * shared * slope);
        const float bx = by_near_rho(ex * shared_near * slope_near), by = by_near_rho(ey * shared_near * slope_near),
                    bz = by_near_rho(ez * shared_near * slope_near);
        const float visc = sk_visc(d, dst);
        const float wx = (nvel.x - vel.x) * visc, wy = (nvel.y - vel.y) * visc, wz = (nvel.z - vel.z) * visc;
        for (uint32_t r = 0; r < mult; r++) {
            a.pfx += ax; a.pfy += ay; a.pfz += az;
            a.pfx += bx; a.pfy += by; a.pfz += bz;
            a.vfx += wx; a.vfy += wy; a.vfz += wz;
        }
    } else {
        const float sa = shared * slope * __builtin_amdgcn_rcpf(nrho_x);
        const float sb = shared_near * slope_near * __builtin_amdgcn_rcpf(nrho_y);
        const float f = sa + sb;
        const float g = f * __builtin_amdgcn_rcpf(dst);
        const bool apart = dst > 0.f;
        const float fx = apart ? ex * g : 0.f, fy = apart ? ey * g : f, fz = apart ? ez * g : 0.f;
        const float hv = d.h * d.h - d2;
        const float visc = hv * hv * hv * d.k_spikey;
        const float wx = (nvel.x - vel.x) * visc, wy = (nvel.y - vel.y) * visc, wz = (nvel.z - vel.z) * visc;
        for (uint32_t r = 0; r < mult; r++) {
            a.pfx += fx; a.pfy += fy; a.pfz += fz;
            a.vfx += wx; a.vfy += wy; a.vfz += wz;
        }
    }
}

__device__ __forceinline__ void density_store(float density, float near_density, uint32_t i, WsSorted srt)
{
    density = density + 0.00001f;
    near_density = near_density + 0.00001f;
    srt.pred(i).w = density;
    srt.vel(i).w = near_density;
}


#define WS_HDR_WORDS 8u
#define WS_MIG_REC_WORDS 8u

__device__ __forceinline__ void migrate_out(const WsDev &d, const WsMig &m, uint32_t i, float4 pos, float4 vel, float4 pred)
{
    const uint32_t gxg = (uint32_t)grid_layer_x(d, pred.x);
    uint32_t dest = 0;
    while (dest + 1 < m.world && gxg >= m.cuts[dest + 1]) dest++;
    const uint32_t hs = atomicAdd(&m.dyn[DY_NHOLE], 1u);
    if (hs < m.hole_cap) m.hole[hs] = i;
    uint32_t *msg;
    uint32_t cap;
    const uint32_t mig_cap = d.mig_limit ? min(d.mig_limit, m.mig_cap) : m.mig_cap;
    if (dest + 1u == m.me) {
        msg = m.sendL; cap = mig_cap;
    } else if (dest == m.me + 1u) {
        msg = m.sendR; cap = mig_cap;
    } else {
        cap = d.far_limit ? min(d.far_limit, m.far_cap) : m.far_cap;
        msg = m.far + (size_t)min(dest, m.world - 1u) * (WS_HDR_WORDS + (size_t)cap * WS_MIG_REC_WORDS);
        atomicAdd(&m.dyn[DY_FAR], 1u);
    }
    const uint32_t slot = atomicAdd(&msg[0], 1u);
    if (slot >= cap || dest == m.me) {
        atomicOr(&m.dyn[DY_ERR], WS_DYN_ERR_MIGRATION);
        return;
    }
    float4 *rec = reinterpret_cast<float4 *>(msg + WS_HDR_WORDS) + 2 * (size_t)slot;
    rec[0] = pos;
    rec[1] = vel;
}

struct WsNewRecord {
    float px, py, pz, pw, vx, vy, vz, vw;
    int have;
};

__device__ __forceinline__ void store_records(const WsDev &d, WsSoA out, uint32_t i, const WsNewRecord &r)
{
    const int lane = threadIdx.x & 63;
    const bool odd = (lane & 1) != 0;
    const int nhave = __popcll(__ballot(r.have != 0));
    const uint32_t i0 = (uint32_t)__builtin_amdgcn_readfirstlane((int)i);
    auto from = [](int byte_addr, float v) { return __int_as_float(__builtin_amdgcn_ds_bpermute(byte_addr, __float_as_int(v))); };
#pragma unroll
    for (int h = 0; h < 2; h++) {
        const int src = 32 * h + (lane >> 1), a = src << 2;
        const uint32_t si = d.dyn ? (uint32_t)__builtin_amdgcn_ds_bpermute(a, (int)i) : i0 + (uint32_t)src;
        const float px = from(a, r.px), py = from(a, r.py), pz = from(a, r.pz), pw = from(a, r.pw);
        const float vx = from(a, r.vx), vy = from(a, r.vy), vz = from(a, r.vz), vw = from(a, r.vw);
        const float4 w = make_float4(odd ? vx : px, odd ? vy : py, odd ? vz : pz, odd ? vw : pw);
        if (src < nhave) out.pv[2 * (size_t)si + (odd ? 1u : 0u)] = w;
    }
}

template <bool ACCEL_ONLY>
__device__ __forceinline__ void force_integrate_bin(const WsDev &d, const ForceAcc &a, float rho_x, float4 vel, uint32_t i,
                                                    const float4 *__restrict__ pos, WsSoA out, float4 *__restrict__ accel,
                                                    uint32_t *__restrict__ cid_out, uint32_t *__restrict__ count,
                                                    WsNewRecord &rec)
{
    const float accx = a.pfx / rho_x + a.vfx * d.viscosity;
    const float accy = a.pfy / rho_x + a.vfy * d.viscosity;
    const float accz = a.pfz / rho_x + a.vfz * d.viscosity;
    if constexpr (ACCEL_ONLY) {
        accel[i] = make_float4(accx, accy, accz, 0.f);
        return;
    }

    const float4 p0 = pos[i];
    float vx = vel.x + (d.grav[0] + accx) * d.dt;
    float vy = vel.y + (d.grav[1] + accy) * d.dt;
    float vz = vel.z + (d.grav[2] + accz) * d.dt;
    float px = p0.x + vx * d.dt;
    float py = p0.y + vy * d.dt;
    float pz = p0.z + vz * d.dt;
    const float nd = -1.f * d.damping;
    if (px < d.ext_min[0]) { vx *= nd; px = d.ext_min[0]; } else if (px > d.ext_max[0]) { vx *= nd; px = d.ext_max[0]; }
    if (py < d.ext_min[1]) { vy *= nd; py = d.ext_min[1]; } else if (py > d.ext_max[1]) { vy *= nd; py = d.ext_max[1]; }
    if (pz < d.ext_min[2]) { vz *= nd; pz = d.ext_min[2]; } else if (pz > d.ext_max[2]) { vz *= nd; pz = d.ext_max[2]; }
    const float qx = px + vx * WS_LOOKAHEAD, qy = py + vy * WS_LOOKAHEAD, qz = pz + vz * WS_LOOKAHEAD;

    const uint32_t nc = grid_cell(d, qx, qy, qz);
    bool stays = true;
    if (d.mig) {
        const uint32_t rowy = (uint32_t)(d.dim[1] * d.dim[2]);
        stays = nc >= rowy && nc < (uint32_t)(d.dim[0] - 1) * rowy;
    }
    const uint32_t cell = stays ? nc : WS_DEAD;
    cid_out[i] = cell;
    rec.px = px; rec.py = py; rec.pz = pz; rec.pw = p0.w;
    rec.vx = vx; rec.vy = vy; rec.vz = vz; rec.vw = __uint_as_float(cell);
    rec.have = 1;
    const uint32_t r = wave_run_atomic_inc(count, nc, stays);
    if (out.rank) out.rank[i] = r;
    if (!stays) migrate_out(d, *d.mig, i, make_float4(px, py, pz, p0.w), make_float4(vx, vy, vz, 0.f), make_float4(qx, qy, qz, 0.f));
}

template <bool ALIAS, bool IEEE, int CUTMODE = 2>
__device__ __forceinline__ void density_sweep_simple(const WsDev &d, const uint32_t *__restrict__ start, WsSorted srt,
                                                     const uint8_t *__restrict__ mult, float4 o, int c, float &density,
                                                     float &near_density)
{
    const int rowz = d.dim[2], rowy = d.dim[1] * d.dim[2];
    WsCut cut = {0u, 0xFFFFFFFFu, false};
    if constexpr (CUTMODE == 2) cut = ws_cut(d);
    for (int dx = -1; dx <= 1; dx++) {
        for (int dy = -1; dy <= 1; dy++) {
            const int cc = d.guard + c + dx * rowy + dy * rowz;
            uint32_t b = start[cc - 1], e = start[cc + 2];
            if constexpr (CUTMODE == 2) cut_run(cut, b, e);
            else cut_run_t<CUTMODE == 1>(d, b, e);
            for (uint32_t j = b; j < e; j++) {
                const float4 q = srt.pred(j);
                const float ex = q.x - o.x, ey = q.y - o.y, ez = q.z - o.z;
                const float d2 = ex * ex + ey * ey + ez * ez;
                if (d2 > d.d2_accept) continue;
                density_pair<IEEE>(d, d2, density, near_density, ALIAS ? alias_mult(d, mult, o, q) : 1u);
            }
        }
    }
}

template <bool ALIAS, bool IEEE, int CUTMODE = 2>
__device__ __forceinline__ void force_sweep_simple(const WsDev &d, const uint32_t *__restrict__ start, WsSorted srt,
                                                   const uint8_t *__restrict__ mult, uint32_t i, float4 o, float4 vel, int c,
                                                   float pressure, float near_pressure, ForceAcc &acc)
{
    const int rowz = d.dim[2], rowy = d.dim[1] * d.dim[2];
    WsCut cut = {0u, 0xFFFFFFFFu, false};
    if constexpr (CUTMODE == 2) cut = ws_cut(d);
    for (int dx = -1; dx <= 1; dx++) {
        for (int dy = -1; dy <= 1; dy++) {
            const int cc = d.guard + c + dx * rowy + dy * rowz;
            uint32_t b = start[cc - 1], e = start[cc + 2];
            if constexpr (CUTMODE == 2) cut_run(cut, b, e);
            else cut_run_t<CUTMODE == 1>(d, b, e);
            for (uint32_t j = b; j < e; j++) {
                if (j == i) continue;
                const float4 q = srt.pred(j);
                const float ex = q.x - o.x, ey = q.y - o.y, ez = q.z - o.z;
                const float d2 = ex * ex + ey * ey + ez * ez;
                if (d2 > d.d2_accept) continue;
                const float4 nvel = srt.vel(j);
                force_pair<IEEE>(d, ex, ey, ez, d2, q.w, nvel.w, nvel, vel, pressure, near_pressure, acc,
                                 ALIAS ? alias_mult(d, mult, o, q) : 1u);
            }
        }
    }
}

template <bool ALIAS, bool IEEE>
__global__ void __launch_bounds__(WS_BLOCK) k_density_simple(WsDev d, const uint32_t *__restrict__ start,
                                                             const uint32_t *__restrict__ cid_srt, WsSorted srt,
                                                             const uint8_t *__restrict__ mult)
{
    const WsSpan sp = ws_span(d, start);
    const uint32_t v = blockIdx.x * WS_BLOCK + threadIdx.x;
    if (v >= sp.len) return;
    const uint32_t i = span_at(sp, v);
    float density = 0.f, near_density = 0.f;
    density_sweep_simple<ALIAS, IEEE>(d, start, srt, mult, srt.pred(i), (int)cid_srt[i], density, near_density);
    density_store(density, near_density, i, srt);
}

template <bool ALIAS, bool IEEE, bool ACCEL_ONLY>
__global__ void __launch_bounds__(WS_BLOCK) k_force_simple(WsDev d, const uint32_t *__restrict__ start,
                                                           const uint32_t *__restrict__ cid_srt, WsSorted srt, WsSoA out,
                                                           float4 *__restrict__ accel, uint32_t *__restrict__ cid_out,
                                                           uint32_t *__restrict__ count, const uint8_t *__restrict__ mult)
{
    const WsSpan sp = ws_span(d, start);
    const uint32_t v = blockIdx.x * WS_BLOCK + threadIdx.x;
    if (sp.len == 0u || (blockIdx.x * WS_BLOCK + (threadIdx.x & ~63u)) >= sp.len) return;
    const bool valid = v < sp.len;
    const uint32_t i = span_at(sp, valid ? v : sp.len - 1u);
    const float4 o = srt.pred(i);
    const float4 vel = srt.vel(i);
    WsNewRecord rec = {0.f, 0.f, 0.f, 0.f, 0.f, 0.f, 0.f, 0.f, 0};
    if (valid) {
        const float pressure = d.pressure_scalar * (o.w - d.target_density);
        const float near_pressure = d.near_pressure_scalar * vel.w;
        ForceAcc acc = {0.f, 0.f, 0.f, 0.f, 0.f, 0.f};
        force_sweep_simple<ALIAS, IEEE>(d, start, srt, mult, i, o, vel, (int)cid_srt[i], pressure, near_pressure, acc);
        force_integrate_bin<ACCEL_ONLY>(d, acc, o.w, vel, i, srt.pos, out, accel, cid_out, count, rec);
    }
    if constexpr (!ACCEL_ONLY) store_records(d, out, i, rec);
}

#ifndef ND_P
#define ND_P 64
#endif
#ifndef ND_K
#define ND_K 16
#endif
#define ND_ROWS (ND_K + 3)
#ifndef ND_MASK_WORDS
#define ND_MASK_WORDS 64
#endif


typedef float nd_f4 __attribute__((ext_vector_type(4)));
typedef float nd_f4u __attribute__((ext_vector_type(4), aligned(4)));

__device__ __forceinline__ void run_bounds(const uint32_t *__restrict__ start, int cc, uint32_t &b, uint32_t &e)
{
    const nd_u4u v = *reinterpret_cast<const nd_u4u *>(start + (cc - 1));
    b = v[0];
    e = v[3];
}

__device__ __forceinline__ uint64_t nd_lanes_lt(uint32_t a, uint32_t b) { return __ballot(a < b); }
__device__ __forceinline__ uint64_t nd_lanes_ge(uint32_t a, uint32_t b) { return __ballot(a >= b); }

template <int U, bool TEST>
__device__ __forceinline__ void nd_mark(float d2, float d2_accept, uint32_t left, uint32_t &at, uint32_t &bits)
{
    const bool acc = (!(TEST && U > 0) || left > 4u * U) && !(d2 > d2_accept);
    *reinterpret_cast<__attribute__((address_space(3))) float *>(at) = d2;
    at += acc ? 4u * ND_P : 0u;
    bits = (U ? bits : 0u) | (acc ? 1u : 0u) << U;
}

template <class Phase2, class Note>
__device__ __forceinline__ void nd_run_planar(const WsDev &d, float4 o, uint32_t j, uint32_t e, uint32_t &at, const uint32_t at0,
                                              WsXYZ p, Phase2 &&phase2, Note &&note)
{
    static_assert(4u * ND_P == 256u, "the fill level is read as (at - at0) >> 8");
    uint32_t off = j * 4u;
    const uint32_t end = e > j ? e * 4u : off;
    auto trip = [&]() {
        const nd_f4 X = *reinterpret_cast<const nd_f4u *>(reinterpret_cast<const char *>(p.x) + off);
        const nd_f4 Y = *reinterpret_cast<const nd_f4u *>(reinterpret_cast<const char *>(p.y) + off);
        const nd_f4 Z = *reinterpret_cast<const nd_f4u *>(reinterpret_cast<const char *>(p.z) + off);
        __builtin_amdgcn_sched_barrier(0);
        float d2[4];
#pragma unroll
        for (int u = 0; u < 4; u++) {
            const float ex = X[u] - o.x, ey = Y[u] - o.y, ez = Z[u] - o.z;
            d2[u] = ex * ex + ey * ey + ez * ez;
        }
        const uint32_t left = end - off;
        uint32_t bits;
        nd_mark<0, true>(d2[0], d.d2_accept, left, at, bits);
        nd_mark<1, true>(d2[1], d.d2_accept, left, at, bits);
        nd_mark<2, true>(d2[2], d.d2_accept, left, at, bits);
        nd_mark<3, true>(d2[3], d.d2_accept, left, at, bits);
        note(min(4u, left >> 2), bits);
        off += 16u;
    };
    if (!(nd_lanes_lt(off, end) & nd_lanes_lt((uint32_t)ND_K, ((at - at0) >> 8) + ((end - off) >> 2)))) {
        while (off < end) trip();
        return;
    }
    const uint32_t full = at0 + 4u * ND_P * ND_K;
    for (;;) {
        const uint64_t more = nd_lanes_lt(off, end);
        if (more & nd_lanes_ge(at, full)) {
            phase2((at - at0) >> 8);
            at = at0;
        }
        if (!more) break;
        if (off < end) {
            do trip();
            while (off < end && !nd_lanes_ge(at, full));
        }
    }
}

template <bool IEEE, bool CUT>
__device__ __forceinline__ void nd_tile(const WsDev &d, const uint32_t *__restrict__ start, const uint32_t *__restrict__ cid_srt,
                                        WsSorted srt, WsXYZ sxyz, WsMask mask, uint32_t *__restrict__ stats, float *list,
                                        const uint32_t iv, const bool valid, const uint32_t tid)
{
    const uint32_t i = iv;
    const float4 o = make_float4(sxyz.x[iv], sxyz.y[iv], sxyz.z[iv], 0.f);
    const int c = (int)cid_srt[iv];
    const int rowz = d.dim[2], rowy = d.dim[1] * d.dim[2];
    float density = 0.f, near_density = 0.f;
    uint32_t acc32 = 0;
    uint32_t posb = 0u - 32u, word = 0;
    uint32_t *mrow = mask.words + (iv - d.base);
    auto phase2 = [&](uint32_t cnt) {
        uint32_t k = 0;
        for (; k + 2u <= cnt; k += 2u) {
            const float a = list[k * ND_P + tid], b = list[(k + 1u) * ND_P + tid];
            density_pair<IEEE>(d, a, density, near_density, 1u);
            density_pair<IEEE>(d, b, density, near_density, 1u);
        }
        if (k < cnt) density_pair<IEEE>(d, list[k * ND_P + tid], density, near_density, 1u);
    };
    auto note = [&](uint32_t nvalid, uint32_t bits) {
        acc32 |= bits << (posb & 31u);
        uint32_t over;
        if (__builtin_expect(__builtin_add_overflow(posb, nvalid, &over), 0)) {
            if (word < ND_MASK_WORDS) {
                *mrow = acc32;
                mrow += mask.stride;
            }
            acc32 = bits >> (nvalid - over);
            word++;
            over -= 32u;
        }
        posb = over;
    };
    const uint32_t at0 = (uint32_t)(uintptr_t)(__attribute__((address_space(3))) float *)list + 4u * tid;
    uint32_t at = at0;
    for (int p = 0; p < 3; p++) {
        const int cc = d.guard + c + (p - 1) * rowy;
        uint32_t b0, b1, b2, e0, e1, e2;
        run_bounds(start, cc - rowz, b0, e0);
        run_bounds(start, cc, b1, e1);
        run_bounds(start, cc + rowz, b2, e2);
        cut_run_t<CUT>(d, b0, e0);
        cut_run_t<CUT>(d, b1, e1);
        cut_run_t<CUT>(d, b2, e2);
        if (!valid) {
            e0 = b0;
            e1 = b1;
            e2 = b2;
        }
        nd_run_planar(d, o, b0, e0, at, at0, sxyz, phase2, note);
        nd_run_planar(d, o, b1, e1, at, at0, sxyz, phase2, note);
        nd_run_planar(d, o, b2, e2, at, at0, sxyz, phase2, note);
    }
    phase2((at - at0) >> 8);
    if (valid) {
        const uint32_t pos = posb + 32u;
        if (pos && word < ND_MASK_WORDS) *mrow = acc32;
        if (32u * word + pos > 32u * ND_MASK_WORDS) atomicAdd(&stats[0], 1u);
        density_store(density, near_density, i, srt);
    }
}

template <bool IEEE, bool CUT, bool SCHED>
__global__ void __launch_bounds__(ND_P) k_density_listed(WsDev d, const uint32_t *__restrict__ start,
                                                         const uint32_t *__restrict__ cid_srt, WsSorted srt, WsXYZ sxyz,
                                                         WsMask mask, uint32_t *__restrict__ stats, WsSched sched)
{
    __shared__ float list[ND_ROWS * ND_P];
    if constexpr (SCHED) {
        const unsigned long long t0 = wall_clock64();
        const uint32_t x = blockIdx.x & 7u, j = blockIdx.x >> 3;
        const uint32_t s0 = sched.split[x], s1 = sched.split[x + 1];
        if (j >= s1 - s0) return;
        const uint32_t tile = sched.perm[s0 + j];
        const uint32_t v = tile * ND_P + threadIdx.x;
        const bool valid = v < d.n;
        nd_tile<IEEE, CUT>(d, start, cid_srt, srt, sxyz, mask, stats, list, d.base + (valid ? v : d.n - 1u), valid, threadIdx.x);
        if (threadIdx.x == 0) sched.cost[tile] = (uint32_t)min(wall_clock64() - t0, 0xFFFFFFull) + 1u;
    } else {
        const WsSpan sp = ws_span(d, start);
        const uint32_t ntiles = (sp.len + ND_P - 1u) / ND_P;
        if (blockIdx.x >= ntiles) return;
        const uint32_t v = xcd_tile(blockIdx.x, ntiles, true) * ND_P + threadIdx.x;
        const bool valid = v < sp.len;
        nd_tile<IEEE, CUT>(d, start, cid_srt, srt, sxyz, mask, stats, list, span_at(sp, valid ? v : sp.len - 1u), valid, threadIdx.x);
    }
}

#ifndef NF_WORDSYNC_MAX
#define NF_WORDSYNC_MAX 6
#endif
#ifndef NF_WORDSYNC_MAX_BIG
#define NF_WORDSYNC_MAX_BIG 12
#endif
#ifndef NF_WORDSYNC_BIG_TILES
#define NF_WORDSYNC_BIG_TILES 16384
#endif
#ifndef NF_WORDSYNC_MAX_TINY
#define NF_WORDSYNC_MAX_TINY 4
#endif
#ifndef NF_WORDSYNC_TINY_TILES
#define NF_WORDSYNC_TINY_TILES 2048
#endif
#ifndef NF_WORDSYNC_MAX_IEEE
#define NF_WORDSYNC_MAX_IEEE 4
#endif
#ifndef NF_P
#define NF_P 128
#endif
#ifndef NF_P_SMALL
#define NF_P_SMALL 64
#endif
#ifndef NF_SMALL_BELOW
#define NF_SMALL_BELOW (1u << 19)
#endif

template <bool IEEE, bool ACCEL_ONLY, bool CUT, int P>
__device__ __forceinline__ void nf_tile(const WsDev &d, const uint32_t *__restrict__ start, const uint32_t *__restrict__ cid_srt,
                                        WsSorted srt, WsSoA out, float4 *__restrict__ accel, uint32_t *__restrict__ cid_out,
                                        uint32_t *__restrict__ count, WsMask mask, uint32_t *t_end, uint32_t *t_delta,
                                        const uint32_t iv, const bool valid, const uint32_t tid, const uint32_t wordsync_max)
{
    const uint32_t i = iv;
    const float4 o = srt.pred(iv);
    const float4 vel = srt.vel(iv);
    const float pressure = d.pressure_scalar * (o.w - d.target_density);
    const float near_pressure = d.near_pressure_scalar * vel.w;
    ForceAcc acc = {0.f, 0.f, 0.f, 0.f, 0.f, 0.f};
    const int c = (int)cid_srt[iv];
    uint32_t total = 0;
    {
        const int rowz = d.dim[2], rowy = d.dim[1] * d.dim[2];
#pragma unroll
        for (int p = 0; p < 3; p++) {
            uint32_t b[3], e[3];
#pragma unroll
            for (int q = 0; q < 3; q++) {
                const int cc = d.guard + c + (p - 1) * rowy + (q - 1) * rowz;
                b[q] = start[cc - 1];
                e[q] = start[cc + 2];
                cut_run_t<CUT>(d, b[q], e[q]);
            }
#pragma unroll
            for (int q = 0; q < 3; q++) {
                const int r = 3 * p + q;
                t_delta[r * P + tid] = b[q] - total;
                total += e[q] - b[q];
                t_end[r * P + tid] = total;
            }
        }
        t_end[9 * P + tid] = 0xFFFFFFFFu;
        if (!valid) total = 0;
    }
    const bool over = total > 32u * ND_MASK_WORDS;
    const bool any_over = __ballot(over) != 0ull;
    if (!over) {
        const uint32_t *mrow = mask.words + (iv - d.base);
        const uint32_t nwords = (total + 31u) >> 5;
        uint32_t run = 0, end_r = t_end[tid], delta_r = t_delta[tid];
        const uint32_t self_s = i - t_delta[4 * P + tid];
      if (!any_over && !__ballot(nwords > wordsync_max)) {
        uint32_t wn0 = nwords ? mrow[0] : 0u, wn1 = nwords > 1u ? mrow[mask.stride] : 0u;
        bool pend = false;
        float4 q_p = o, nvel_p = vel;
        for (uint32_t w = 0; __ballot(w < nwords); w += 2u) {
            unsigned long long bits = (w < nwords ? (unsigned long long)wn0 : 0ull) | (w + 1u < nwords ? (unsigned long long)wn1 << 32 : 0ull);
            if ((w >> 1) == (self_s >> 6)) bits &= ~(1ull << (self_s & 63u));
            wn0 = w + 2u < nwords ? mrow[(size_t)(w + 2u) * mask.stride] : 0u;
            wn1 = w + 3u < nwords ? mrow[(size_t)(w + 3u) * mask.stride] : 0u;
            const uint32_t wbase = w << 5;
            while (__ballot(bits != 0ull)) {
                const bool has = bits != 0ull;
                float4 q_n = q_p, nvel_n = nvel_p;
                if (has) {
                    const uint32_t sc = wbase + (uint32_t)__ffsll((long long)bits) - 1u;
                    bits &= bits - 1ull;
                    while (sc >= end_r) {
                        run++;
                        end_r = t_end[run * P + tid];
                        delta_r = t_delta[min(run, 8u) * P + tid];
                    }
                    const uint32_t j = sc + delta_r;
                    q_n = srt.pred_near(j);
                    nvel_n = srt.vel_near(j);
                }
                if (pend) {
                    const float ex = q_p.x - o.x, ey = q_p.y - o.y, ez = q_p.z - o.z;
                    force_pair<IEEE>(d, ex, ey, ez, ex * ex + ey * ey + ez * ez, q_p.w, nvel_p.w, nvel_p, vel, pressure,
                                     near_pressure, acc, 1u);
                }
                pend = has;
                q_p = q_n;
                nvel_p = nvel_n;
            }
        }
        if (pend) {
            const float ex = q_p.x - o.x, ey = q_p.y - o.y, ez = q_p.z - o.z;
            force_pair<IEEE>(d, ex, ey, ez, ex * ex + ey * ey + ez * ez, q_p.w, nvel_p.w, nvel_p, vel, pressure, near_pressure,
                             acc, 1u);
        }
      } else {
        uint32_t rest = 0, wbase = 0, widx = 0;
        uint32_t wnext = nwords ? mrow[0] : 0u;
        const uint32_t *mnext = mrow;
        auto next = [&](uint32_t &j) -> bool {
            while (rest == 0u) {
                if (widx >= nwords) return false;
                rest = wnext;
                wbase = widx << 5;
                if (widx == (self_s >> 5)) rest &= ~(1u << (self_s & 31u));
                widx++;
                mnext += mask.stride;
                wnext = widx < nwords ? *mnext : 0u;
            }
            const uint32_t sc = wbase + (uint32_t)__ffs((int)rest) - 1u;
            rest &= rest - 1u;
            while (sc >= end_r) {
                run++;
                end_r = t_end[run * P + tid];
                delta_r = t_delta[min(run, 8u) * P + tid];
            }
            j = sc + delta_r;
            return true;
        };
        uint32_t j1 = iv, j2 = iv;
        bool have0 = next(j1);
        float4 q_next = srt.pred_near(j1), nvel_next = srt.vel_near(j1);
        bool have1 = have0 && next(j2);
        while (have0) {
            const float4 q = q_next, nvel = nvel_next;
            q_next = srt.pred_near(j2);
            nvel_next = srt.vel_near(j2);
            have0 = have1;
            have1 = have1 && next(j2);
            const float ex = q.x - o.x, ey = q.y - o.y, ez = q.z - o.z;
            force_pair<IEEE>(d, ex, ey, ez, ex * ex + ey * ey + ez * ez, q.w, nvel.w, nvel, vel, pressure, near_pressure,
                             acc, 1u);
        }
      }
    } else if (valid) {
        force_sweep_simple<false, IEEE, CUT ? 1 : 0>(d, start, srt, nullptr, i, o, vel, c, pressure, near_pressure, acc);
    }
    WsNewRecord rec = {0.f, 0.f, 0.f, 0.f, 0.f, 0.f, 0.f, 0.f, 0};
    if (valid) force_integrate_bin<ACCEL_ONLY>(d, acc, o.w, vel, i, srt.pos, out, accel, cid_out, count, rec);
    if constexpr (!ACCEL_ONLY) store_records(d, out, i, rec);
}

template <bool IEEE, bool ACCEL_ONLY, bool CUT, bool SCHED, int P>
__global__ void __launch_bounds__(P) k_force_listed(WsDev d, const uint32_t *__restrict__ start,
                                                       const uint32_t *__restrict__ cid_srt, WsSorted srt, WsSoA out,
                                                       float4 *__restrict__ accel, uint32_t *__restrict__ cid_out,
                                                       uint32_t *__restrict__ count, WsMask mask, WsSched sched)
{
    __shared__ uint32_t t_end[10 * P];
    __shared__ uint32_t t_delta[9 * P];
    if constexpr (SCHED) {
        const unsigned long long t0 = wall_clock64();
        const uint32_t x = blockIdx.x & 7u, j = blockIdx.x >> 3;
        const uint32_t s0 = sched.split[x], s1 = sched.split[x + 1];
        if (j >= s1 - s0) return;
        const uint32_t tile = sched.perm[s0 + j];
        const uint32_t v = tile * P + threadIdx.x;
        const bool valid = v < d.n;
        nf_tile<IEEE, ACCEL_ONLY, CUT, P>(d, start, cid_srt, srt, out, accel, cid_out, count, mask, t_end, t_delta,
                                       d.base + (valid ? v : d.n - 1u), valid, threadIdx.x, (uint32_t)(IEEE ? NF_WORDSYNC_MAX_IEEE : NF_WORDSYNC_MAX));
        __syncthreads();
        if (threadIdx.x == 0) sched.cost[tile] = (uint32_t)min(wall_clock64() - t0, 0xFFFFFFull) + 1u;
    } else {
        const WsSpan sp = ws_span(d, start);
        const uint32_t ntiles = (sp.len + P - 1u) / P;
        if (blockIdx.x >= ntiles) return;
        const uint32_t v = xcd_tile(blockIdx.x, ntiles) * P + threadIdx.x;
        const bool valid = v < sp.len;
        nf_tile<IEEE, ACCEL_ONLY, CUT, P>(d, start, cid_srt, srt, out, accel, cid_out, count, mask, t_end, t_delta,
                                       span_at(sp, valid ? v : sp.len - 1u), valid, threadIdx.x,
                                       IEEE ? (uint32_t)NF_WORDSYNC_MAX_IEEE : ntiles >= (uint32_t)NF_WORDSYNC_BIG_TILES ? (uint32_t)NF_WORDSYNC_MAX_BIG
                                                                     : ntiles >= (uint32_t)NF_WORDSYNC_TINY_TILES ? (uint32_t)NF_WORDSYNC_MAX : (uint32_t)NF_WORDSYNC_MAX_TINY);
    }
}

uint32_t wsk_mask_words(void) { return ND_MASK_WORDS; }

#define WS_LAUNCH(kernel, grid, block, s, ev, ...)                                                          \
    do {                                                                                                    \
        if (ev) hipExtLaunchKernelGGL(kernel, grid, block, 0, s, (ev)->a, (ev)->b, 0, __VA_ARGS__);         \
        else hipLaunchKernelGGL(kernel, grid, block, 0, s, __VA_ARGS__);                                    \
    } while (0)

uint32_t wsk_sched_grid(uint32_t ntiles) { return 8u * (ntiles / 8u + ntiles / 16u + 2u); }
uint32_t wsk_density_tile(void) { return ND_P; }
uint32_t wsk_force_tile(uint32_t n) { return n < (uint32_t)NF_SMALL_BELOW ? (uint32_t)NF_P_SMALL : (uint32_t)NF_P; }

template <bool IEEE>
static void launch_density(hipStream_t s, const WsDev &d, const uint32_t *start, const uint32_t *cid_srt, WsSorted srt,
                           const uint8_t *mult, bool alias, int variant, uint32_t *stats, WsMask mask, WsXYZ sxyz,
                           const WsEventPair *ev, WsSched sched)
{
    if (alias)
        WS_LAUNCH((k_density_simple<true, IEEE>), dim3(cdiv(d.n, WS_BLOCK)), dim3(WS_BLOCK), s, ev, d, start, cid_srt, srt, mult);
    else if (variant == WS_VARIANT_SIMPLE)
        WS_LAUNCH((k_density_simple<false, IEEE>), dim3(cdiv(d.n, WS_BLOCK)), dim3(WS_BLOCK), s, ev, d, start, cid_srt, srt, mult);
    else if (d.dyn && d.range_sel == WS_RANGE_EARLY)
        WS_LAUNCH((k_density_listed<IEEE, true, false>), dim3(cdiv(d.n, ND_P)), dim3(ND_P), s, ev, d, start, cid_srt, srt, sxyz, mask, stats, sched);
    else if (sched.perm && !d.dyn)
        WS_LAUNCH((k_density_listed<IEEE, false, true>), dim3(wsk_sched_grid(cdiv(d.n, ND_P))), dim3(ND_P), s, ev, d, start, cid_srt, srt, sxyz, mask, stats, sched);
    else
        WS_LAUNCH((k_density_listed<IEEE, false, false>), dim3(cdiv(d.n, ND_P)), dim3(ND_P), s, ev, d, start, cid_srt, srt, sxyz, mask, stats, sched);
}

template <bool IEEE, bool ACCEL_ONLY, int P>
static void launch_force_listed(hipStream_t s, const WsDev &d, const uint32_t *start, const uint32_t *cid_srt, WsSorted srt, WsSoA out,
                                float4 *accel, uint32_t *cid_out, uint32_t *count, WsMask mask, const WsEventPair *ev, WsSched sched)
{
    if (d.dyn && d.range_sel == WS_RANGE_EARLY)
        WS_LAUNCH((k_force_listed<IEEE, ACCEL_ONLY, true, false, P>), dim3(cdiv(d.n, P)), dim3(P), s, ev, d, start, cid_srt, srt, out,
                  accel, cid_out, count, mask, sched);
    else if (sched.perm && !d.dyn)
        WS_LAUNCH((k_force_listed<IEEE, ACCEL_ONLY, false, true, P>), dim3(wsk_sched_grid(cdiv(d.n, P))), dim3(P), s, ev, d, start, cid_srt, srt, out,
                  accel, cid_out, count, mask, sched);
    else
        WS_LAUNCH((k_force_listed<IEEE, ACCEL_ONLY, false, false, P>), dim3(cdiv(d.n, P)), dim3(P), s, ev, d, start, cid_srt, srt, out,
                  accel, cid_out, count, mask, sched);
}

template <bool IEEE, bool ACCEL_ONLY>
static void launch_force(hipStream_t s, const WsDev &d, const uint32_t *start, const uint32_t *cid_srt, WsSorted srt,
                         WsSoA out, float4 *accel, uint32_t *cid_out, uint32_t *count, const uint8_t *mult, bool alias,
                         int variant, WsMask mask, const WsEventPair *ev, WsSched sched)
{
    if (alias)
        WS_LAUNCH((k_force_simple<true, IEEE, ACCEL_ONLY>), dim3(cdiv(d.n, WS_BLOCK)), dim3(WS_BLOCK), s, ev, d, start, cid_srt,
                  srt, out, accel, cid_out, count, mult);
    else if (variant == WS_VARIANT_SIMPLE)
        WS_LAUNCH((k_force_simple<false, IEEE, ACCEL_ONLY>), dim3(cdiv(d.n, WS_BLOCK)), dim3(WS_BLOCK), s, ev, d, start, cid_srt,
                  srt, out, accel, cid_out, count, mult);
    else if (wsk_force_tile(d.n) == (uint32_t)NF_P_SMALL)
        launch_force_listed<IEEE, ACCEL_ONLY, NF_P_SMALL>(s, d, start, cid_srt, srt, out, accel, cid_out, count, mask, ev, sched);
    else
        launch_force_listed<IEEE, ACCEL_ONLY, NF_P>(s, d, start, cid_srt, srt, out, accel, cid_out, count, mask, ev, sched);
}

void wsk_density(hipStream_t s, const WsDev &d, const uint32_t *start, const uint32_t *cid_srt, WsSorted srt,
                 const uint8_t *mult, bool alias, int variant, bool ieee, uint32_t *stats, WsMask mask, WsXYZ sxyz,
                 const WsEventPair *ev, WsSched sched)
{
    if (ieee) launch_density<true>(s, d, start, cid_srt, srt, mult, alias, variant, stats, mask, sxyz, ev, sched);
    else launch_density<false>(s, d, start, cid_srt, srt, mult, alias, variant, stats, mask, sxyz, ev, sched);
}

void wsk_force(hipStream_t s, const WsDev &d, const uint32_t *start, const uint32_t *cid_srt, WsSorted srt, WsSoA out,
               float4 *accel, uint32_t *cid_out, uint32_t *count, const uint8_t *mult, bool alias, int variant, bool ieee,
               WsMask mask, bool accel_only, const WsEventPair *ev, WsSched sched)
{
    if (accel_only) {
        if (ieee) launch_force<true, true>(s, d, start, cid_srt, srt, out, accel, cid_out, count, mult, alias, variant, mask, ev, sched);
        else launch_force<false, true>(s, d, start, cid_srt, srt, out, accel, cid_out, count, mult, alias, variant, mask, ev, sched);
    } else {
        if (ieee) launch_force<true, false>(s, d, start, cid_srt, srt, out, accel, cid_out, count, mult, alias, variant, mask, ev, sched);
        else launch_force<false, false>(s, d, start, cid_srt, srt, out, accel, cid_out, count, mult, alias, variant, mask, ev, sched);
    }
}

#define WS_SCHED_BLOCK 1024
#define WS_SCHED_CLASSES 8

__device__ __forceinline__ uint32_t block_excl_scan_1024(uint32_t v, uint32_t *s_w, uint32_t &total)
{
    const int lane = threadIdx.x & 63, wave = threadIdx.x >> 6;
    const uint32_t incl = wave_incl_scan(v);
    __syncthreads();
    if (lane == 63) s_w[wave] = incl;
    __syncthreads();
    uint32_t base = 0, tot = 0;
#pragma unroll
    for (int w = 0; w < WS_SCHED_BLOCK / 64; w++) {
        const uint32_t x = s_w[w];
        if (w < wave) base += x;
        tot += x;
    }
    total = tot;
    return base + incl - v;
}

__global__ void __launch_bounds__(WS_SCHED_BLOCK) k_schedule(WsSched s4, uint32_t nt4, WsSched s5, uint32_t nt5, uint32_t nclasses,
                                                             uint32_t group_particles, uint32_t tile5)
{
    __shared__ uint32_t s_w[WS_SCHED_BLOCK / 64];
    __shared__ uint32_t s_cut[9];
    __shared__ uint32_t s_max;
    const bool second = blockIdx.x >= 8u;
    const WsSched sc = second ? s5 : s4;
    const uint32_t T = second ? nt5 : nt4, x = blockIdx.x & 7u, tid = threadIdx.x;
    if (T == 0u) return;
    const uint32_t G = max(group_particles / (second ? tile5 : (uint32_t)ND_P), 1u);
    const uint32_t per = (T + WS_SCHED_BLOCK - 1u) / WS_SCHED_BLOCK;
    const uint32_t a = min(tid * per, T), b = min(a + per, T);
    uint32_t known = 0, sum = 0;
    for (uint32_t t = a; t < b; t++) {
        const uint32_t c = sc.cost[t];
        known += c ? 1u : 0u;
        sum += c;
    }
    uint32_t tot_known, tot_sum;
    block_excl_scan_1024(known, s_w, tot_known);
    block_excl_scan_1024(sum >> 10, s_w, tot_sum);
    const uint32_t fill = tot_known ? (uint32_t)min(max(((unsigned long long)tot_sum << 10) / tot_known, 1ull), 0xFFFFFFull) : 1u;
    unsigned long long mine = 0;
    for (uint32_t t = a; t < b; t++) {
        const uint32_t c = sc.cost[t];
        mine += c ? c : fill;
    }
    const uint32_t shift = 10u;
    const uint32_t mine_s = (uint32_t)(mine >> shift);
    uint32_t total_s;
    const uint32_t before_s = block_excl_scan_1024(mine_s, s_w, total_s);
    if (tid < 9u) s_cut[tid] = tid == 8u ? T : 0u;
    __syncthreads();
    if (total_s >= 8u) {
        for (uint32_t k = 1; k < 8u; k++) {
            const unsigned long long target = (unsigned long long)total_s * k / 8u;
            if (target >= before_s && target < (unsigned long long)before_s + mine_s) {
                unsigned long long run = (unsigned long long)before_s << shift;
                const unsigned long long want = target << shift;
                uint32_t t = a;
                for (; t < b; t++) {
                    const uint32_t c = sc.cost[t];
                    run += c ? c : fill;
                    if (run > want) break;
                }
                s_cut[k] = min(t + 1u, T);
            }
        }
    } else if (tid == 0u) {
        for (uint32_t k = 1; k < 8u; k++) s_cut[k] = (uint32_t)((unsigned long long)T * k / 8u);
    }
    __syncthreads();
    if (tid == 0u) {
        const uint32_t nmax = T / 8u + T / 16u + 1u, nmin = T / 16u;
        uint32_t prev = 0;
        for (uint32_t k = 1; k < 8u; k++) {
            const uint32_t left = 8u - k;
            uint32_t lo = prev + nmin, hi = prev + nmax;
            lo = max(lo, T > left * nmax ? T - left * nmax : 0u);
            hi = min(hi, T - min(T, left * nmin));
            uint32_t c = s_cut[k];
            c = min(max(c, lo), max(hi, lo));
            c = min(c, T);
            s_cut[k] = c;
            prev = c;
        }
        s_cut[0] = 0u;
        s_cut[8] = T;
        s_max = 0u;
    }
    __syncthreads();
    if (x == 0u && tid < 9u) sc.split[tid] = s_cut[tid];
    const uint32_t r0 = s_cut[x], r1 = s_cut[x + 1u], n = r1 - r0;
    if (n == 0u) return;
    const uint32_t g0 = r0 / G, g1 = (r1 + G - 1u) / G, ng = g1 - g0;
    const uint32_t gper = (ng + WS_SCHED_BLOCK - 1u) / WS_SCHED_BLOCK;
    const uint32_t ga = g0 + min(tid * gper, ng), gb = min(ga + gper, g1);
    auto group_cost = [&](uint32_t g) {
        const uint32_t ta = max(g * G, r0), tb = min((g + 1u) * G, r1);
        unsigned long long sumc = 0;
        for (uint32_t t = ta; t < tb; t++) {
            const uint32_t c = sc.cost[t];
            sumc += c ? c : fill;
        }
        return tb > ta ? (uint32_t)(sumc / (tb - ta)) : 0u;
    };
    uint32_t mx = 0;
    for (uint32_t g = ga; g < gb; g++) mx = max(mx, group_cost(g));
#pragma unroll
    for (int sh = 32; sh >= 1; sh >>= 1) mx = max(mx, (uint32_t)__shfl_xor((int)mx, sh, 64));
    if ((tid & 63u) == 0u) atomicMax(&s_max, mx);
    __syncthreads();
    const uint32_t cmax = s_max + 1u;
    auto cls_of = [&](uint32_t v) {
        return (uint32_t)(((unsigned long long)(cmax - 1u - min(v, cmax - 1u)) * nclasses) / cmax);
    };
    uint32_t cnt[WS_SCHED_CLASSES];
#pragma unroll
    for (int k = 0; k < WS_SCHED_CLASSES; k++) cnt[k] = 0u;
    for (uint32_t g = ga; g < gb; g++) {
        const uint32_t k = cls_of(group_cost(g));
        const uint32_t m = min((g + 1u) * G, r1) - max(g * G, r0);
#pragma unroll
        for (int q = 0; q < WS_SCHED_CLASSES; q++) cnt[q] += (k == (uint32_t)q) ? m : 0u;
    }
    uint32_t off[WS_SCHED_CLASSES], cbase = 0;
#pragma unroll
    for (int k = 0; k < WS_SCHED_CLASSES; k++) {
        uint32_t tot;
        off[k] = cbase + block_excl_scan_1024(cnt[k], s_w, tot);
        cbase += tot;
    }
    for (uint32_t g = ga; g < gb; g++) {
        const uint32_t k = cls_of(group_cost(g));
        const uint32_t ta = max(g * G, r0), tb = min((g + 1u) * G, r1);
        uint32_t dst = 0;
#pragma unroll
        for (int q = 0; q < WS_SCHED_CLASSES; q++)
            if (k == (uint32_t)q) {
                dst = off[q];
                off[q] += tb - ta;
            }
        for (uint32_t t = ta; t < tb; t++) sc.perm[r0 + dst + (t - ta)] = t;
    }
}

void wsk_schedule(hipStream_t s, WsSched s4, uint32_t ntiles4, WsSched s5, WsSched s5_costs, uint32_t ntiles5, uint32_t nclasses,
                  uint32_t group_particles, uint32_t tile5)
// ... 2549 lines not shown
```

Before: 793.2.

## Accumulate per-tile cell-count sums during binning to skip scan lookback

The binning and force kernels now add per-tile particle counts into a small tile-sum table with wave-aggregated atomics. The next step's cell-count scan can then build each tile's prefix from these precomputed sums instead of running the decoupled lookback chain. The place kernel takes the table, presumably to reset or consume it. This removes the serial lookback latency from the scan. In exchange it adds atomics to the bin and force kernels, extra validity bookkeeping, and a second graph instance.

```diff
diff --git a/water-sandbox_amd/csrc/ws_api.cpp b/water-sandbox_amd/csrc/ws_api.cpp
--- a/water-sandbox_amd/csrc/ws_api.cpp
+++ b/water-sandbox_amd/csrc/ws_api.cpp
@@ -225,6 +225,13 @@
     if ((st = h->starts.alloc(h, &h->start_alloc, (nstart + 4) * 4, "cell starts"))) return st;
     h->start = h->start_alloc + (4u - (uint32_t)d.guard % 4u) % 4u;
     if ((st = h->starts.alloc(h, &h->bsum, (size_t)wsk_scan_state_words(d.ncells) * 4, "cell scan state", true))) return st;
+    h->tile_sums_valid = false;
+    h->tile_count = 0;
+    if (!h->slab && wsk_scan_sums_pays(d.ncells)) {
+        h->tile_count = wsk_scan_tiles(d.ncells);
+        h->tile_shift = wsk_scan_tile_shift(d.ncells);
+        if ((st = h->starts.alloc(h, &h->tile_sum, (size_t)h->tile_count * 4, "scan tile sums", true))) return st;
+    }
     HIP_TRY(h, hipMemsetAsync(h->start, 0, (size_t)d.guard * 4, h->stream));
     std::vector<uint32_t> tail((size_t)d.guard + 2, d.n);
     HIP_TRY(h, hipMemcpyAsync(h->start + d.guard + d.ncells, tail.data(), tail.size() * 4, hipMemcpyHostToDevice,
@@ -450,20 +457,32 @@
     return WS_OK;
 }
 
+bool scan_with_tile_sums(const ws_handle *h) { return h->tile_sum && h->tile_sums_valid && !h->scan_lookback_only; }
+
 void enqueue_step(ws_handle *h)
 {
     const WsDev &d = h->dev;
     hipStream_t s = h->stream;
     const bool sched = h->sched_on && !h->alias && h->variant == WS_VARIANT_LISTED && !(h->flags & WS_FLAG_GRAPH);
     const uint32_t par = h->sched_parity;
+    const WsTileSums ts = {h->tile_sum, h->tile_shift};
     {
         Prof p(h, WS_K_SCAN);
-        wsk_scan(s, h->count, h->start + d.guard, nullptr, h->bsum, d.ncells, true, 0);
+        if (scan_with_tile_sums(h)) {
+            wsk_scan_sums(s, h->count, h->start + d.guard, h->tile_sum, d.ncells, 0);
+            h->last_scan = 2;
+        } else {
+            wsk_scan(s, h->count, h->start + d.guard, nullptr, h->bsum, d.ncells, true, 0);
+            h->last_scan = 1;
+        }
     }
     {
         Prof p(h, WS_K_SCATTER);
-        wsk_place(s, d, h->cid_cur, h->cur.rank, h->start, h->slot_tmp);
-    }
+        wsk_place(s, d, h->cid_cur, h->cur.rank, h->start, h->slot_tmp, h->tile_sum, h->tile_count);
+    }
+#ifdef WS_DEV_HOOKS
+    if (h->tile_snap.p && h->tile_snap.bytes >= (size_t)h->tile_count * 4) hipMemcpyAsync(h->tile_snap.p, h->tile_sum, (size_t)h->tile_count * 4, hipMemcpyDeviceToDevice, s);
+#endif
     {
         Prof p(h, WS_K_REORDER);
         wsk_reorder(s, d, h->slot_tmp, h->cid_cur, h->start, h->cur, h->srt, h->cid_srt, h->sxyz, h->pred_stale);
@@ -485,8 +504,9 @@
     {
         ProfLaunch p(h, WS_K_FORCE);
         wsk_force(s, d, h->start, h->cid_srt, h->srt, h->cur, h->accel, h->cid_cur, h->count, h->mult, h->alias,
-                  h->variant, h->ieee, h->mask, false, p.events(), sched ? h->sched5[par] : WsSched{});
-    }
+                  h->variant, h->ieee, h->mask, false, p.events(), sched ? h->sched5[par] : WsSched{}, ts);
+    }
+    h->tile_sums_valid = true;
     h->pred_stale = true;
     h->accel_stale = true;
 }
@@ -538,11 +558,13 @@
 {
     refresh_pred(h, h->dev);
     HIP_TRY(h, hipMemsetAsync(h->count, 0, (size_t)h->dev.ncells * 4, h->stream));
+    if (h->tile_sum) HIP_TRY(h, hipMemsetAsync(h->tile_sum, 0, (size_t)h->tile_count * 4, h->stream));
     {
         Prof pr(h, WS_K_BIN);
-        wsk_bin(h->stream, h->dev, h->cur, h->cid_cur, h->count);
+        wsk_bin(h->stream, h->dev, h->cur, h->cid_cur, h->count, WsTileSums{h->tile_sum, h->tile_shift});
     }
     HIP_TRY(h, hipGetLastError());
+    h->tile_sums_valid = h->tile_sum != nullptr;
     return WS_OK;
 }
 
@@ -566,8 +588,10 @@
 
 void drop_graphs(ws_handle *h)
 {
-    if (h->graph_exec) hipGraphExecDestroy(h->graph_exec);
-    h->graph_exec = nullptr;
+    for (hipGraphExec_t &g : h->graph_exec) {
+        if (g) hipGraphExecDestroy(g);
+        g = nullptr;
+    }
     if (h->slab) slab_drop_graphs(h->slab);
 }
 
@@ -615,7 +639,7 @@
     for (auto e : h->pool) hipEventDestroy(e);
     free_grid(h);
     free_particle_arrays(h);
-    release_all(h->fixed, h->stage_mem, h->force_cnt, h->solid_sums, h->v_keys, h->v_perm, h->v_tmp, h->v_count, h->v_cursor, h->v_start, h->v_bsum,
+    release_all(h->fixed, h->stage_mem, h->tile_snap, h->force_cnt, h->solid_sums, h->v_keys, h->v_perm, h->v_tmp, h->v_count, h->v_cursor, h->v_start, h->v_bsum,
                 h->v_off);
     for (auto &volume : h->volume) release_all(volume);
     release_all(h->attr);
@@ -812,24 +836,28 @@
     bound_pending(h);
     note_step_params(h);
     if ((h->flags & WS_FLAG_GRAPH) && !h->graph_failed && h->pred_stale) {
-        if (!h->graph_exec) {
+        const bool sums = scan_with_tile_sums(h);
+        hipGraphExec_t &exec = h->graph_exec[sums ? 1 : 0];
+        if (!exec) {
             hipGraph_t gr = nullptr;
             hipError_t e = hipStreamBeginCapture(s, hipStreamCaptureModeRelaxed);
             if (e == hipSuccess) {
                 enqueue_step(h);
                 e = hipStreamEndCapture(s, &gr);
-                if (e == hipSuccess) e = hipGraphInstantiate(&h->graph_exec, gr, nullptr, nullptr, 0);
+                if (e == hipSuccess) e = hipGraphInstantiate(&exec, gr, nullptr, nullptr, 0);
                 if (gr) hipGraphDestroy(gr);
             }
-            if (e != hipSuccess || !h->graph_exec) {
+            if (e != hipSuccess || !exec) {
                 (void)hipGetLastError();
                 h->graph_failed = true;
-                h->graph_exec = nullptr;
+                exec = nullptr;
                 h->err = std::string("WS_FLAG_GRAPH: capture failed (") + hipGetErrorName(e) + "), using direct launches";
             }
         }
-        if (h->graph_exec) {
-            HIP_TRY(h, hipGraphLaunch(h->graph_exec, s));
+        if (exec) {
+            HIP_TRY(h, hipGraphLaunch(exec, s));
+            h->last_scan = sums ? 2 : 1;
+            h->tile_sums_valid = true;
             h->pred_stale = true;
             h->accel_stale = true;
             h->graph_steps++;
@@ -1158,6 +1186,7 @@
     const ws_status st = call.prepare(h, nullptr);
     if (st) return st;
     HIP_TRY(h, hipMemsetAsync(h->count, 0, (size_t)h->dev.ncells * 4, h->stream));
+    h->tile_sums_valid = false;
     wsk_edit_current(h->stream, h->dev, h->cur, h->cid_cur, h->count, call.args);
     HIP_TRY(h, hipGetLastError());
     h->pred_stale = true;
@@ -1799,6 +1828,39 @@
     return WS_OK;
 }
 
+ws_status ws_dev_scan_lookback(ws_handle *h, int on)
+{
+    if (!h) return WS_ERR_INVALID_ARG;
+    HIP_TRY(h, hipSetDevice(h->device));
+    h->scan_lookback_only = on != 0;
+    drop_graphs(h);
+    return WS_OK;
+}
+
+ws_status ws_dev_read_tile_sums(ws_handle *h, uint32_t *now, uint32_t *after_place, uint32_t *info)
+{
+    if (!h) return WS_ERR_INVALID_ARG;
+    WS_DEAD_CHECK(h);
+    HIP_TRY(h, hipSetDevice(h->device));
+    if (!h->tile_sum) return fail(h, WS_ERR_INVALID_ARG, "ws_dev_read_tile_sums: the handle has no tile table");
+    const ws_status st = dev_drain(h);
+    if (st) return st;
+    const size_t bytes = (size_t)h->tile_count * 4;
+    if (info) info[0] = h->tile_count, info[1] = h->tile_shift, info[2] = h->last_scan, info[3] = h->tile_sums_valid ? 1u : 0u;
+    if (now) HIP_TRY(h, copy_now(h, now, h->tile_sum, bytes, hipMemcpyDeviceToHost));
+    if (after_place) {
+        if (h->tile_snap.bytes < bytes) {
+            const ws_status sa = h->tile_snap.alloc(h, bytes, "tile table snapshot");
+            if (sa) return sa;
+            HIP_TRY(h, hipMemsetAsync(h->tile_snap.p, 0xFF, bytes, h->stream));
+            drop_graphs(h);
+        }
+        HIP_TRY(h, copy_now(h, after_place, h->tile_snap.p, bytes, hipMemcpyDeviceToHost));
+        HIP_TRY(h, hipMemsetAsync(h->tile_snap.p, 0xFF, bytes, h->stream));
+    }
+    return WS_OK;
+}
+
 }
 #endif
 
diff --git a/water-sandbox_amd/csrc/ws_internal.h b/water-sandbox_amd/csrc/ws_internal.h
--- a/water-sandbox_amd/csrc/ws_internal.h
+++ b/water-sandbox_amd/csrc/ws_internal.h
@@ -271,6 +271,12 @@
     uint32_t *start = nullptr;
     uint32_t *start_alloc = nullptr;
     uint32_t *bsum = nullptr;
+    uint32_t *tile_sum = nullptr;
+    uint32_t tile_count = 0, tile_shift = 0;
+    bool tile_sums_valid = false;
+    bool scan_lookback_only = false;
+    uint32_t last_scan = 0;
+    WsScratch<uint32_t> tile_snap;
     WsMask mask = {nullptr, 0};
     bool ieee = false;
     uint32_t *stats = nullptr;
@@ -321,7 +327,7 @@
     hipStream_t sched_stream = nullptr;
     hipEvent_t ev_sched_in = nullptr, ev_sched_out = nullptr;
 
-    hipGraphExec_t graph_exec = nullptr;
+    hipGraphExec_t graph_exec[2] = {nullptr, nullptr};
     bool graph_failed = false;
     uint64_t graph_steps = 0;
 
@@ -423,11 +429,20 @@
 
 void wsk_upload_positions(hipStream_t s, const float *xyz_dev, WsSoA cur, uint32_t n);
 void wsk_upload_particles(hipStream_t s, const ws_particle80 *in_dev, WsSoA cur, uint32_t n);
-void wsk_bin(hipStream_t s, const WsDev &d, WsSoA cur, uint32_t *cid, uint32_t *count);
-void wsk_place(hipStream_t s, const WsDev &d, const uint32_t *cid, const uint32_t *rank, const uint32_t *start, uint32_t *slot_tmp);
+struct WsTileSums {
+    uint32_t *sum = nullptr;
+    uint32_t shift = 0;
+};
+void wsk_bin(hipStream_t s, const WsDev &d, WsSoA cur, uint32_t *cid, uint32_t *count, WsTileSums ts = WsTileSums{});
+void wsk_place(hipStream_t s, const WsDev &d, const uint32_t *cid, const uint32_t *rank, const uint32_t *start, uint32_t *slot_tmp,
+               uint32_t *tile_sum = nullptr, uint32_t ntiles = 0);
 void wsk_scan(hipStream_t s, uint32_t *count, uint32_t *start_body, uint32_t *cursor, uint32_t *state, uint32_t nitems,
               bool zero_count, uint32_t base);
 uint32_t wsk_scan_state_words(uint32_t nitems);
+void wsk_scan_sums(hipStream_t s, uint32_t *count, uint32_t *start_body, const uint32_t *tile_sum, uint32_t nitems, uint32_t base);
+bool wsk_scan_sums_pays(uint32_t nitems);
+uint32_t wsk_scan_tiles(uint32_t nitems);
+uint32_t wsk_scan_tile_shift(uint32_t nitems);
 void wsk_scatter(hipStream_t s, const uint32_t *keys, uint32_t *cursor, uint32_t *slot_tmp, uint32_t n, const uint32_t *n_dev);
 void wsk_reorder(hipStream_t s, const WsDev &d, const uint32_t *slot_tmp, const uint32_t *cid_cur, const uint32_t *start, WsSoA cur,
                  WsSorted srt, uint32_t *cid_srt, WsXYZ sxyz, bool recompute_pred);
@@ -494,7 +509,8 @@
 uint32_t wsk_mask_words(void);
 void wsk_force(hipStream_t s, const WsDev &d, const uint32_t *start, const uint32_t *cid_srt, WsSorted srt, WsSoA out,
                float4 *accel, uint32_t *cid_out, uint32_t *count, const uint8_t *mult, bool alias, int variant, bool ieee,
-               WsMask mask, bool accel_only, const WsEventPair *ev = nullptr, WsSched sched = WsSched{});
+               WsMask mask, bool accel_only, const WsEventPair *ev = nullptr, WsSched sched = WsSched{},
+               WsTileSums ts = WsTileSums{});
 void wsk_gather_positions(hipStream_t s, WsSoA cur, float *out_xyz, uint32_t n);
 void wsk_gather_speeds(hipStream_t s, WsSoA cur, float *out, uint32_t n);
 void wsk_gather_velocities(hipStream_t s, WsSoA cur, float *out_xyz, uint32_t n);
diff --git a/water-sandbox_amd/csrc/ws_kernels.hip b/water-sandbox_amd/csrc/ws_kernels.hip
--- a/water-sandbox_amd/csrc/ws_kernels.hip
+++ b/water-sandbox_amd/csrc/ws_kernels.hip
@@ -155,7 +155,22 @@
 
 #define WS_DEAD 0xFFFFFFFFu
 
-__global__ void __launch_bounds__(WS_BLOCK) k_bin(WsDev d, WsSoA cur, uint32_t *__restrict__ cid, uint32_t *__restrict__ count)
+__device__ __forceinline__ void wave_tile_sum_add(const WsTileSums &ts, uint32_t cell)
+{
+    if (!ts.sum) return;
+    const uint32_t tile = cell >> ts.shift;
+    for (;;) {
+        const uint32_t t = (uint32_t)__builtin_amdgcn_readfirstlane((int)tile);
+        const unsigned long long same = __ballot(tile == t);
+        if (tile == t) {
+            if ((int)(threadIdx.x & 63u) == __builtin_ctzll(same)) atomicAdd(&ts.sum[t], (uint32_t)__builtin_popcountll(same));
+            break;
+        }
+    }
+}
+
+__global__ void __launch_bounds__(WS_BLOCK) k_bin(WsDev d, WsSoA cur, uint32_t *__restrict__ cid, uint32_t *__restrict__ count,
+                                                  WsTileSums ts)
 {
     const uint32_t i = blockIdx.x * WS_BLOCK + threadIdx.x;
     if (i >= ws_n(d)) return;
@@ -165,11 +180,12 @@
     cur.vel(i).w = __uint_as_float(c);
     const uint32_t r = atomicAdd(&count[c], 1u);
     if (cur.rank) cur.rank[i] = r;
-}
-
-void wsk_bin(hipStream_t s, const WsDev &d, WsSoA cur, uint32_t *cid, uint32_t *count)
-{
-    hipLaunchKernelGGL(k_bin, dim3(cdiv(d.n, WS_BLOCK)), dim3(WS_BLOCK), 0, s, d, cur, cid, count);
+    wave_tile_sum_add(ts, c);
+}
+
+void wsk_bin(hipStream_t s, const WsDev &d, WsSoA cur, uint32_t *cid, uint32_t *count, WsTileSums ts)
+{
+    hipLaunchKernelGGL(k_bin, dim3(cdiv(d.n, WS_BLOCK)), dim3(WS_BLOCK), 0, s, d, cur, cid, count, ts);
 }
 
 __device__ __forceinline__ uint32_t wave_incl_scan(uint32_t v)
@@ -203,24 +219,9 @@
     return base + (uint32_t)(lane - hl);
 }
 
-template <bool ZERO, int WS_SCAN_ITEMS>
-__global__ void __launch_bounds__(WS_BLOCK) k_scan(uint32_t *__restrict__ count, uint32_t nitems,
-                                                   uint32_t *__restrict__ state, uint32_t *__restrict__ start,
-                                                   uint32_t *__restrict__ cursor, uint32_t start_offset, uint32_t ntiles)
-{
-    __shared__ uint32_t s_tile, s_epoch, s_prefix;
-    if (threadIdx.x == 0) {
-        const unsigned long long ticket = atomicAdd(reinterpret_cast<unsigned long long *>(state), 1ull);
-        s_tile = (uint32_t)(ticket % ntiles);
-        s_epoch = (uint32_t)(ticket / ntiles) + 1u;
-    }
-    __syncthreads();
-    const uint32_t tile = s_tile, epoch = s_epoch;
-    constexpr int Q = WS_SCAN_ITEMS / 4;
-    constexpr uint32_t WS_SCAN_TILE = WS_BLOCK * WS_SCAN_ITEMS;
-    const uint32_t tbase = tile * WS_SCAN_TILE;
-    uint4 v[Q];
-    uint32_t excl[Q], total = 0;
+template <int Q>
+__device__ __forceinline__ void scan_tile_fetch(const uint32_t *__restrict__ count, uint32_t nitems, uint32_t tbase, uint4 (&v)[Q])
+{
 #pragma unroll
     for (int q = 0; q < Q; q++) {
         const uint32_t at = tbase + (q * WS_BLOCK + threadIdx.x) * 4u;
@@ -233,6 +234,12 @@
             v[q].w = 0u;
         }
     }
+}
+
+template <int Q>
+__device__ __forceinline__ uint32_t scan_tile_scan(const uint4 (&v)[Q], uint32_t (&excl)[Q])
+{
+    uint32_t total = 0;
     {
         __shared__ uint32_t wsum[Q][WS_BLOCK / 64];
         const int lane = threadIdx.x & 63, wave = threadIdx.x >> 6;
@@ -255,6 +262,56 @@
             total += tot;
         }
     }
+    return total;
+}
+
+template <bool ZERO, int Q>
+__device__ __forceinline__ void scan_tile_store(uint32_t *__restrict__ count, uint32_t nitems, uint32_t tbase, const uint4 (&v)[Q],
+                                                const uint32_t (&excl)[Q], uint32_t carry, uint32_t *__restrict__ start,
+                                                uint32_t *__restrict__ cursor)
+{
+#pragma unroll
+    for (int q = 0; q < Q; q++) {
+        const uint32_t at = tbase + (q * WS_BLOCK + threadIdx.x) * 4u;
+        uint4 r;
+        r.x = carry + excl[q];
+        r.y = r.x + v[q].x;
+        r.z = r.y + v[q].y;
+        r.w = r.z + v[q].z;
+        if (at + 4u <= nitems) {
+            *reinterpret_cast<uint4 *>(start + at) = r;
+            if (cursor) *reinterpret_cast<uint4 *>(cursor + at) = r;
+            if (ZERO) *reinterpret_cast<uint4 *>(count + at) = make_uint4(0u, 0u, 0u, 0u);
+        } else {
+            const uint32_t rr[3] = {r.x, r.y, r.z};
+            for (uint32_t k = 0; k < 3u && at + k < nitems; k++) {
+                start[at + k] = rr[k];
+                if (cursor) cursor[at + k] = rr[k];
+                if (ZERO) count[at + k] = 0u;
+            }
+        }
+    }
+}
+
+template <bool ZERO, int WS_SCAN_ITEMS>
+__global__ void __launch_bounds__(WS_BLOCK) k_scan(uint32_t *__restrict__ count, uint32_t nitems,
+                                                   uint32_t *__restrict__ state, uint32_t *__restrict__ start,
+                                                   uint32_t *__restrict__ cursor, uint32_t start_offset, uint32_t ntiles)
+{
+    __shared__ uint32_t s_tile, s_epoch, s_prefix;
+    if (threadIdx.x == 0) {
+        const unsigned long long ticket = atomicAdd(reinterpret_cast<unsigned long long *>(state), 1ull);
+        s_tile = (uint32_t)(ticket % ntiles);
+        s_epoch = (uint32_t)(ticket / ntiles) + 1u;
+    }
+    __syncthreads();
+    const uint32_t tile = s_tile, epoch = s_epoch;
+    constexpr int Q = WS_SCAN_ITEMS / 4;
+    const uint32_t tbase = tile * (WS_BLOCK * WS_SCAN_ITEMS);
+    uint4 v[Q];
+    uint32_t excl[Q];
+    scan_tile_fetch<Q>(count, nitems, tbase, v);
+    const uint32_t total = scan_tile_scan<Q>(v, excl);
     if (threadIdx.x < 64) {
         unsigned long long *desc = reinterpret_cast<unsigned long long *>(state + 2);
         const uint32_t e30 = epoch & 0x3FFFFFFFu;
@@ -291,28 +348,35 @@
         }
     }
     __syncthreads();
-    const uint32_t carry = s_prefix + start_offset;
+    scan_tile_store<ZERO, Q>(count, nitems, tbase, v, excl, s_prefix + start_offset, start, cursor);
+}
+
+template <int WS_SCAN_ITEMS>
+__global__ void __launch_bounds__(WS_BLOCK) k_scan_sums(uint32_t *__restrict__ count, uint32_t nitems,
+                                                        const uint32_t *__restrict__ tile_sum, uint32_t *__restrict__ start,
+                                                        uint32_t start_offset)
+{
+    __shared__ uint32_t s_prefix;
+    const uint32_t tile = blockIdx.x;
+    constexpr int Q = WS_SCAN_ITEMS / 4;
+    const uint32_t tbase = tile * (WS_BLOCK * WS_SCAN_ITEMS);
+    uint4 v[Q];
+    uint32_t excl[Q], before = 0;
+    scan_tile_fetch<Q>(count, nitems, tbase, v);
+    if (threadIdx.x < 64) {
+        for (uint32_t t0 = 0; t0 < tile; t0 += 64u) {
+            const uint32_t t = t0 + threadIdx.x;
+            before += t < tile ? tile_sum[t] : 0u;
+        }
+    }
+    scan_tile_scan<Q>(v, excl);
+    if (threadIdx.x < 64) {
 #pragma unroll
-    for (int q = 0; q < Q; q++) {
-        const uint32_t at = tbase + (q * WS_BLOCK + threadIdx.x) * 4u;
-        uint4 r;
-        r.x = carry + excl[q];
-        r.y = r.x + v[q].x;
-        r.z = r.y + v[q].y;
-        r.w = r.z + v[q].z;
-        if (at + 4u <= nitems) {
-            *reinterpret_cast<uint4 *>(start + at) = r;
-            if (cursor) *reinterpret_cast<uint4 *>(cursor + at) = r;
-            if (ZERO) *reinterpret_cast<uint4 *>(count + at) = make_uint4(0u, 0u, 0u, 0u);
-        } else {
-            const uint32_t rr[3] = {r.x, r.y, r.z};
-            for (uint32_t k = 0; k < 3u && at + k < nitems; k++) {
-                start[at + k] = rr[k];
-                if (cursor) cursor[at + k] = rr[k];
-                if (ZERO) count[at + k] = 0u;
-            }
-        }
-    }
+        for (int sh = 32; sh >= 1; sh >>= 1) before += __shfl_xor(before, sh, 64);
+        if (threadIdx.x == 0) s_prefix = before;
+    }
+    __syncthreads();
+    scan_tile_store<true, Q>(count, nitems, tbase, v, excl, s_prefix + start_offset, start, nullptr);
 }
 
 uint32_t wsk_scan_state_words(uint32_t nitems) { return 2u + 2u * cdiv(nitems, WS_SCAN_TILE_MIN); }
@@ -334,6 +398,21 @@
 #undef WS_SCAN_LAUNCH
 }
 
+#define WS_SCAN_SUMS_BELOW (1u << 23)
+bool wsk_scan_sums_pays(uint32_t nitems) { return nitems < WS_SCAN_SUMS_BELOW; }
+uint32_t wsk_scan_tile_shift(uint32_t nitems) { return nitems >= WS_SCAN_LARGE_FROM ? 14u : 13u; }
+static_assert(WS_BLOCK * WS_SCAN_ITEMS_LARGE == 1 << 14 && WS_BLOCK * WS_SCAN_ITEMS_SMALL == 1 << 13, "wsk_scan_tile_shift");
+uint32_t wsk_scan_tiles(uint32_t nitems) { return cdiv(nitems, 1u << wsk_scan_tile_shift(nitems)); }
+
+void wsk_scan_sums(hipStream_t s, uint32_t *count, uint32_t *start_body, const uint32_t *tile_sum, uint32_t nitems, uint32_t base)
+{
+    const uint32_t ntiles = wsk_scan_tiles(nitems);
+    if (nitems >= WS_SCAN_LARGE_FROM)
+        hipLaunchKernelGGL((k_scan_sums<WS_SCAN_ITEMS_LARGE>), dim3(ntiles), dim3(WS_BLOCK), 0, s, count, nitems, tile_sum, start_body, base);
+    else
+        hipLaunchKernelGGL((k_scan_sums<WS_SCAN_ITEMS_SMALL>), dim3(ntiles), dim3(WS_BLOCK), 0, s, count, nitems, tile_sum, start_body, base);
+}
+
 __global__ void __launch_bounds__(WS_BLOCK) k_scatter(const uint32_t *__restrict__ keys, uint32_t *__restrict__ cursor,
                                                       uint32_t *__restrict__ slot_tmp, uint32_t n,
                                                       const uint32_t *__restrict__ n_dev)
@@ -347,8 +426,11 @@
 
 __global__ void __launch_bounds__(WS_BLOCK) k_place(WsDev d, const uint32_t *__restrict__ cid,
                                                     const uint32_t *__restrict__ rank,
-                                                    const uint32_t *__restrict__ start, uint32_t *__restrict__ slot_tmp)
-{
+                                                    const uint32_t *__restrict__ start, uint32_t *__restrict__ slot_tmp,
+                                                    uint32_t *__restrict__ tile_sum, uint32_t ntiles)
+{
+    if (blockIdx.x == 0)
+        for (uint32_t t = threadIdx.x; t < ntiles; t += WS_BLOCK) tile_sum[t] = 0u;
     const uint32_t i = blockIdx.x * WS_BLOCK + threadIdx.x;
     if (i >= ws_n(d)) return;
     const uint32_t c = cid[i];
@@ -356,9 +438,11 @@
     slot_tmp[start[d.guard + c] + rank[i]] = i;
 }
 
-void wsk_place(hipStream_t s, const WsDev &d, const uint32_t *cid, const uint32_t *rank, const uint32_t *start, uint32_t *slot_tmp)
-{
-    hipLaunchKernelGGL(k_place, dim3(cdiv(d.n, WS_BLOCK)), dim3(WS_BLOCK), 0, s, d, cid, rank, start, slot_tmp);
+void wsk_place(hipStream_t s, const WsDev &d, const uint32_t *cid, const uint32_t *rank, const uint32_t *start, uint32_t *slot_tmp,
+               uint32_t *tile_sum, uint32_t ntiles)
+{
+    hipLaunchKernelGGL(k_place, dim3(cdiv(d.n, WS_BLOCK)), dim3(WS_BLOCK), 0, s, d, cid, rank, start, slot_tmp, tile_sum,
+                       tile_sum ? ntiles : 0u);
 }
 
 void wsk_scatter(hipStream_t s, const uint32_t *keys, uint32_t *cursor, uint32_t *slot_tmp, uint32_t n, const uint32_t *n_dev)
@@ -1070,7 +1154,7 @@
 __device__ __forceinline__ void force_integrate_bin(const WsDev &d, const ForceAcc &a, float rho_x, float4 vel, uint32_t i,
                                                     const float4 *__restrict__ pos, WsSoA out, float4 *__restrict__ accel,
                                                     uint32_t *__restrict__ cid_out, uint32_t *__restrict__ count,
-                                                    WsNewRecord &rec)
+                                                    const WsTileSums &ts, WsNewRecord &rec)
 {
     const float accx = a.pfx / rho_x + a.vfx * d.viscosity;
     const float accy = a.pfy / rho_x + a.vfy * d.viscosity;
@@ -1106,6 +1190,7 @@
     rec.have = 1;
     const uint32_t r = wave_run_atomic_inc(count, nc, stays);
     if (out.rank) out.rank[i] = r;
+    wave_tile_sum_add(ts, nc);
     if (!stays) migrate_out(d, *d.mig, i, make_float4(px, py, pz, p0.w), make_float4(vx, vy, vz, 0.f), make_float4(qx, qy, qz, 0.f));
 }
 
@@ -1180,7 +1265,8 @@
 __global__ void __launch_bounds__(WS_BLOCK) k_force_simple(WsDev d, const uint32_t *__restrict__ start,
                                                            const uint32_t *__restrict__ cid_srt, WsSorted srt, WsSoA out,
                                                            float4 *__restrict__ accel, uint32_t *__restrict__ cid_out,
-                                                           uint32_t *__restrict__ count, const uint8_t *__restrict__ mult)
+                                                           uint32_t *__restrict__ count, const uint8_t *__restrict__ mult,
+                                                           WsTileSums ts)
 {
     const WsSpan sp = ws_span(d, start);
     const uint32_t v = blockIdx.x * WS_BLOCK + threadIdx.x;
@@ -1195,7 +1281,7 @@
         const float near_pressure = d.near_pressure_scalar * vel.w;
         ForceAcc acc = {0.f, 0.f, 0.f, 0.f, 0.f, 0.f};
         force_sweep_simple<ALIAS, IEEE>(d, start, srt, mult, i, o, vel, (int)cid_srt[i], pressure, near_pressure, acc);
-        force_integrate_bin<ACCEL_ONLY>(d, acc, o.w, vel, i, srt.pos, out, accel, cid_out, count, rec);
+        force_integrate_bin<ACCEL_ONLY>(d, acc, o.w, vel, i, srt.pos, out, accel, cid_out, count, ts, rec);
     }
     if constexpr (!ACCEL_ONLY) store_records(d, out, i, rec);
 }
@@ -1402,7 +1488,7 @@
 template <bool IEEE, bool ACCEL_ONLY, bool CUT, int P>
 __device__ __forceinline__ void nf_tile(const WsDev &d, const uint32_t *__restrict__ start, const uint32_t *__restrict__ cid_srt,
                                         WsSorted srt, WsSoA out, float4 *__restrict__ accel, uint32_t *__restrict__ cid_out,
-                                        uint32_t *__restrict__ count, WsMask mask, uint32_t *t_end, uint32_t *t_delta,
+                                        uint32_t *__restrict__ count, const WsTileSums &ts, WsMask mask, uint32_t *t_end, uint32_t *t_delta,
                                         const uint32_t iv, const bool valid, const uint32_t tid, const uint32_t wordsync_max)
 {
     const uint32_t i = iv;
@@ -1526,7 +1612,7 @@
         force_sweep_simple<false, IEEE, CUT ? 1 : 0>(d, start, srt, nullptr, i, o, vel, c, pressure, near_pressure, acc);
     }
     WsNewRecord rec = {0.f, 0.f, 0.f, 0.f, 0.f, 0.f, 0.f, 0.f, 0};
-    if (valid) force_integrate_bin<ACCEL_ONLY>(d, acc, o.w, vel, i, srt.pos, out, accel, cid_out, count, rec);
+    if (valid) force_integrate_bin<ACCEL_ONLY>(d, acc, o.w, vel, i, srt.pos, out, accel, cid_out, count, ts, rec);
     if constexpr (!ACCEL_ONLY) store_records(d, out, i, rec);
 }
 
@@ -1534,7 +1620,7 @@
 __global__ void __launch_bounds__(P) k_force_listed(WsDev d, const uint32_t *__restrict__ start,
                                                        const uint32_t *__restrict__ cid_srt, WsSorted srt, WsSoA out,
                                                        float4 *__restrict__ accel, uint32_t *__restrict__ cid_out,
-                                                       uint32_t *__restrict__ count, WsMask mask, WsSched sched)
+                                                       uint32_t *__restrict__ count, WsMask mask, WsSched sched, WsTileSums ts)
 {
     __shared__ uint32_t t_end[10 * P];
     __shared__ uint32_t t_delta[9 * P];
@@ -1546,7 +1632,7 @@
         const uint32_t tile = sched.perm[s0 + j];
         const uint32_t v = tile * P + threadIdx.x;
         const bool valid = v < d.n;
-        nf_tile<IEEE, ACCEL_ONLY, CUT, P>(d, start, cid_srt, srt, out, accel, cid_out, count, mask, t_end, t_delta,
+        nf_tile<IEEE, ACCEL_ONLY, CUT, P>(d, start, cid_srt, srt, out, accel, cid_out, count, ts, mask, t_end, t_delta,
                                        d.base + (valid ? v : d.n - 1u), valid, threadIdx.x, (uint32_t)(IEEE ? NF_WORDSYNC_MAX_IEEE : NF_WORDSYNC_MAX));
         __syncthreads();
         if (threadIdx.x == 0) sched.cost[tile] = (uint32_t)min(wall_clock64() - t0, 0xFFFFFFull) + 1u;
@@ -1556,7 +1642,7 @@
         if (blockIdx.x >= ntiles) return;
         const uint32_t v = xcd_tile(blockIdx.x, ntiles) * P + threadIdx.x;
         const bool valid = v < sp.len;
-        nf_tile<IEEE, ACCEL_ONLY, CUT, P>(d, start, cid_srt, srt, out, accel, cid_out, count, mask, t_end, t_delta,
+        nf_tile<IEEE, ACCEL_ONLY, CUT, P>(d, start, cid_srt, srt, out, accel, cid_out, count, ts, mask, t_end, t_delta,
                                        span_at(sp, valid ? v : sp.len - 1u), valid, threadIdx.x,
                                        IEEE ? (uint32_t)NF_WORDSYNC_MAX_IEEE : ntiles >= (uint32_t)NF_WORDSYNC_BIG_TILES ? (uint32_t)NF_WORDSYNC_MAX_BIG
                                                                      : ntiles >= (uint32_t)NF_WORDSYNC_TINY_TILES ? (uint32_t)NF_WORDSYNC_MAX : (uint32_t)NF_WORDSYNC_MAX_TINY);
@@ -1594,34 +1680,35 @@
 
 template <bool IEEE, bool ACCEL_ONLY, int P>
 static void launch_force_listed(hipStream_t s, const WsDev &d, const uint32_t *start, const uint32_t *cid_srt, WsSorted srt, WsSoA out,
-                                float4 *accel, uint32_t *cid_out, uint32_t *count, WsMask mask, const WsEventPair *ev, WsSched sched)
+                                float4 *accel, uint32_t *cid_out, uint32_t *count, WsMask mask, const WsEventPair *ev, WsSched sched,
+                                WsTileSums ts)
 {
     if (d.dyn && d.range_sel == WS_RANGE_EARLY)
         WS_LAUNCH((k_force_listed<IEEE, ACCEL_ONLY, true, false, P>), dim3(cdiv(d.n, P)), dim3(P), s, ev, d, start, cid_srt, srt, out,
-                  accel, cid_out, count, mask, sched);
+                  accel, cid_out, count, mask, sched, ts);
     else if (sched.perm && !d.dyn)
         WS_LAUNCH((k_force_listed<IEEE, ACCEL_ONLY, false, true, P>), dim3(wsk_sched_grid(cdiv(d.n, P))), dim3(P), s, ev, d, start, cid_srt, srt, out,
-                  accel, cid_out, count, mask, sched);
+                  accel, cid_out, count, mask, sched, ts);
     else
         WS_LAUNCH((k_force_listed<IEEE, ACCEL_ONLY, false, false, P>), dim3(cdiv(d.n, P)), dim3(P), s, ev, d, start, cid_srt, srt, out,
-                  accel, cid_out, count, mask, sched);
+                  accel, cid_out, count, mask, sched, ts);
 }
 
 template <bool IEEE, bool ACCEL_ONLY>
 static void launch_force(hipStream_t s, const WsDev &d, const uint32_t *start, const uint32_t *cid_srt, WsSorted srt,
                          WsSoA out, float4 *accel, uint32_t *cid_out, uint32_t *count, const uint8_t *mult, bool alias,
-                         int variant, WsMask mask, const WsEventPair *ev, WsSched sched)
+                         int variant, WsMask mask, const WsEventPair *ev, WsSched sched, WsTileSums ts)
 {
     if (alias)
         WS_LAUNCH((k_force_simple<true, IEEE, ACCEL_ONLY>), dim3(cdiv(d.n, WS_BLOCK)), dim3(WS_BLOCK), s, ev, d, start, cid_srt,
-                  srt, out, accel, cid_out, count, mult);
+                  srt, out, accel, cid_out, count, mult, ts);
     else if (variant == WS_VARIANT_SIMPLE)
         WS_LAUNCH((k_force_simple<false, IEEE, ACCEL_ONLY>), dim3(cdiv(d.n, WS_BLOCK)), dim3(WS_BLOCK), s, ev, d, start, cid_srt,
-                  srt, out, accel, cid_out, count, mult);
+                  srt, out, accel, cid_out, count, mult, ts);
     else if (wsk_force_tile(d.n) == (uint32_t)NF_P_SMALL)
-        launch_force_listed<IEEE, ACCEL_ONLY, NF_P_SMALL>(s, d, start, cid_srt, srt, out, accel, cid_out, count, mask, ev, sched);
+        launch_force_listed<IEEE, ACCEL_ONLY, NF_P_SMALL>(s, d, start, cid_srt, srt, out, accel, cid_out, count, mask, ev, sched, ts);
     else
-        launch_force_listed<IEEE, ACCEL_ONLY, NF_P>(s, d, start, cid_srt, srt, out, accel, cid_out, count, mask, ev, sched);
+        launch_force_listed<IEEE, ACCEL_ONLY, NF_P>(s, d, start, cid_srt, srt, out, accel, cid_out, count, mask, ev, sched, ts);
 }
 
 void wsk_density(hipStream_t s, const WsDev &d, const uint32_t *start, const uint32_t *cid_srt, WsSorted srt,
@@ -1634,14 +1721,14 @@
 
 void wsk_force(hipStream_t s, const WsDev &d, const uint32_t *start, const uint32_t *cid_srt, WsSorted srt, WsSoA out,
                float4 *accel, uint32_t *cid_out, uint32_t *count, const uint8_t *mult, bool alias, int variant, bool ieee,
-               WsMask mask, bool accel_only, const WsEventPair *ev, WsSched sched)
+               WsMask mask, bool accel_only, const WsEventPair *ev, WsSched sched, WsTileSums ts)
 {
     if (accel_only) {
-        if (ieee) launch_force<true, true>(s, d, start, cid_srt, srt, out, accel, cid_out, count, mult, alias, variant, mask, ev, sched);
-        else launch_force<false, true>(s, d, start, cid_srt, srt, out, accel, cid_out, count, mult, alias, variant, mask, ev, sched);
+        if (ieee) launch_force<true, true>(s, d, start, cid_srt, srt, out, accel, cid_out, count, mult, alias, variant, mask, ev, sched, ts);
+        else launch_force<false, true>(s, d, start, cid_srt, srt, out, accel, cid_out, count, mult, alias, variant, mask, ev, sched, ts);
     } else {
-        if (ieee) launch_force<true, false>(s, d, start, cid_srt, srt, out, accel, cid_out, count, mult, alias, variant, mask, ev, sched);
-        else launch_force<false, false>(s, d, start, cid_srt, srt, out, accel, cid_out, count, mult, alias, variant, mask, ev, sched);
+        if (ieee) launch_force<true, false>(s, d, start, cid_srt, srt, out, accel, cid_out, count, mult, alias, variant, mask, ev, sched, ts);
+        else launch_force<false, false>(s, d, start, cid_srt, srt, out, accel, cid_out, count, mult, alias, variant, mask, ev, sched, ts);
     }
 }
 
```

New measurement: 792.8 (median of 2 runs). No clear change (-0.0%).
